# abstract-liu/LORB_SLAM

Measured on AMD Instinct MI355X. Metric: ORB matches/sec + local-BA iterations/sec (50 KF, 10k pts) at 1/2/4/8 MI355X, higher is better.
Workload: dtype f64+u8; 1 GPU; c4_local_mapping_step_chained; windows_per_gpu=1, kf=50, fixed_kf=5, points=10679, observations=75130, new_kf_keypoints=2000, match=2000x~10679 bf crossCheck, parallelism=independent windows x1

## Files before the change

### lorb_slam_amd/csrc/lorb_ba.hip

```cpp
#ifndef LORB_NO_CONTRACT
#pragma clang fp contract(fast)
#endif
#include "lorb_ba_math.h"
#include "lorb_internal.h"
#include "lorb_ba_dev.h"
#include "lorb_ba_plan.h"

#include <algorithm>
#include <cmath>
#include <type_traits>

namespace {

using namespace lorb::ba;
using lorb::residual;
using lorb::residual_jac;
using lorb::residual_jac_s;
using lorb::residual_s;

__device__ __forceinline__ void init_run(const BaDev& d, int W, int ctot, int n_pt, int nf, const LMOpt& o, const int i,
                                         const int stride) {
  if (i < W) {
    WinState s;
    s.radius = o.init_radius; s.decrease_factor = 2.0; s.cost = 0.0; s.x_norm = 0.0; s.gmax = 0.0;
    s.initial_cost = 0.0; s.iter = 0; s.n_success = 0; s.n_invalid = 0;
    s.done = d.win[i].n_obs_all == 0 ? 1 : 0;
    s.relin = 1; s.cur = 0; s.last_successful = 1; s.term = 0; s.chol_fail = 0; s.pad = 0;
    d.st[i] = s;
    d.ls_fail[i] = 0;
    if (d.sharded) d.wfail_part[i] = 0.0;
  }
  if (i < ctot) {
    double x[6];
#pragma unroll
    for (int k = 0; k < 6; ++k) { x[k] = d.x_init_pose[6 * i + k]; d.x_pose[0][6 * i + k] = x[k]; }
    d.rot_lin[i] = lorb::rot_jet(x);
  }
  if (i < nf) {
    double x[6];
#pragma unroll
    for (int k = 0; k < 6; ++k) x[k] = d.fixed_pose[6 * i + k];
    d.rot_fix[i] = lorb::rot_jet(x);
    d.rotv_fix[i] = lorb::rot_val(x);
  }
  for (int k = i; k < 3 * n_pt; k += stride) d.x_pt[0][k] = d.x_init_pt[k];
}
__global__ __launch_bounds__(256) void k_ba_init(BaDev d, int W, int ctot, int n_pt, int nf, LMOpt o) {
  init_run(d, W, ctot, n_pt, nf, o, blockIdx.x * blockDim.x + threadIdx.x, gridDim.x * blockDim.x);
}


constexpr int kGW = kGB / 64;
static_assert(kGW >= 1 && kGW <= 16 && kGB % 64 == 0, "point groups of 64..1024 observations, whole waves");
template <bool M1>
__device__ __forceinline__ void block_red3(double& a, double& b, double& c, double (*red)[kGW]) {
  a = wave_sum(a); b = M1 ? wave_max(b) : wave_sum(b); c = wave_sum(c);
  if (kGW == 1) return;
  __syncthreads();
  if ((threadIdx.x & 63) == 0) {
    const int w = threadIdx.x >> 6;
    red[0][w] = a; red[1][w] = b; red[2][w] = c;
  }
  __syncthreads();
  a = red[0][0]; b = red[1][0]; c = red[2][0];
#pragma unroll
  for (int k = 1; k < kGW; ++k) { a += red[0][k]; b = M1 ? fmax(b, red[1][k]) : b + red[1][k]; c += red[2][k]; }
}

__device__ __forceinline__ bool prep_point(const double (&Eu)[6], const double (&bu)[3], const double (&sp)[3],
                                           double rad, const LMOpt& o, double (&Ei)[6], double (&b)[3]) {
  double E[6];
#pragma unroll
  for (int k = 0; k < 3; ++k) b[k] = bu[k] * sp[k];
  E[0] = Eu[0] * sp[0] * sp[0]; E[1] = Eu[1] * sp[0] * sp[1]; E[2] = Eu[2] * sp[0] * sp[2];
  E[3] = Eu[3] * sp[1] * sp[1]; E[4] = Eu[4] * sp[1] * sp[2]; E[5] = Eu[5] * sp[2] * sp[2];
  E[0] += fmin(fmax(E[0], o.min_diag), o.max_diag) / rad;
  E[3] += fmin(fmax(E[3], o.min_diag), o.max_diag) / rad;
  E[5] += fmin(fmax(E[5], o.min_diag), o.max_diag) / rad;
  if (!inv3(E, Ei)) {
#pragma unroll
    for (int k = 0; k < 6; ++k) Ei[k] = 0.0;
    return false;
  }
  return true;
}
__device__ __forceinline__ void prep_fail(const BaDev& d, int win, int fold) {
  if (fold) d.ls_fail[win] = 1;
  else if (d.sharded) d.wfail_part[win] = 1.0;
  else d.st[win].chol_fail = 1;
}

template <int PH>
__global__ __launch_bounds__(64) void k_ba_win_reduce(BaDev d) {
  const int w = blockIdx.x;
  if (d.st[w].done) return;
  const BaWin& W = d.win[w];
  const int lane = threadIdx.x;
  double a = 0.0, b = 0.0, c = 0.0;
  if (PH == 0) group_partials<0, 1, 2, true>(d.part, W.pblk_base, W.n_pblk, lane, a, c, b);
  else group_partials<3, 4, 5, false>(d.part, W.pblk_base, W.n_pblk, lane, a, b, c);
  a = wave_sum(a); b = wave_sum(b);
  c = PH == 0 ? wave_max(c) : wave_sum(c);
  if (lane == 0) {
    if (PH == 0) { d.wlin_part[2 * w] = a; d.wlin_part[2 * w + 1] = b; d.wmax_part[w] = c; }
    else { d.wstep_part[3 * w] = a; d.wstep_part[3 * w + 1] = b; d.wstep_part[3 * w + 2] = c; }
  }
}

template <bool SH>
__device__ __forceinline__ void lm_begin_run(const BaDev& d, const LMOpt& o, const int w) {
  const WinState* Sp = d.st + w;
  const WinState S = *Sp;
  const BaWin W = d.win[w];
  if (S.done) return;
  (void)lm_head<SH>(d, o, w, threadIdx.x, S, W);
}
template <bool SH>
__global__ __launch_bounds__(64) void k_ba_lm_begin(BaDev d, LMOpt o) {
  lm_begin_run<SH>(d, o, blockIdx.x);
}

__device__ __forceinline__ lorb_lm_iteration lm_rec(const WinState& S, int outcome, double mcc, double ncost,
                                                    double step_norm) {
  lorb_lm_iteration r;
  r.iteration = S.iter; r.outcome = outcome;
  r.cost = S.cost; r.model_cost_change = mcc; r.new_cost = ncost; r.radius = S.radius; r.step_norm = step_norm;
  return r;
}
__device__ __forceinline__ void lm_record(const BaDev& d, int w, const lorb_lm_iteration& r) {
  if (r.iteration < 1 || r.iteration > LORB_LM_TRACE_CAP) return;
  d.trace[(size_t)w * LORB_LM_TRACE_CAP + r.iteration - 1] = r;
}

__device__ __forceinline__ WinState state_copy(const WinState& s) {
  WinState r;
  r.radius = s.radius; r.decrease_factor = s.decrease_factor; r.cost = s.cost; r.x_norm = s.x_norm; r.gmax = s.gmax;
  r.initial_cost = s.initial_cost; r.iter = s.iter; r.n_success = s.n_success; r.n_invalid = s.n_invalid;
  r.done = s.done; r.relin = s.relin; r.cur = s.cur; r.last_successful = s.last_successful; r.term = s.term;
  r.chol_fail = s.chol_fail; r.pad = s.pad;
  return r;
}

__device__ __forceinline__ int lm_decide(const LMOpt& o, WinState& S, bool valid, double mccs, double ncost,
                                         double sn2, lorb_lm_iteration& rec) {
  const double model_cost_change = -mccs;
  valid = valid && isfinite(model_cost_change) && isfinite(sn2) && model_cost_change > 0.0;
  if (!valid) {
    rec = lm_rec(S, LORB_LM_STEP_INVALID, model_cost_change, ncost, sqrt(sn2));
    if (++S.n_invalid >= o.max_invalid) {
      S.done = 1; S.term = LORB_TERM_FAILURE;
    } else {
      S.radius = S.radius / S.decrease_factor;
      S.decrease_factor *= 2.0;
      S.last_successful = 0;
      if (S.iter >= o.max_iter) { S.done = 1; S.term = LORB_TERM_NO_CONVERGENCE; }
    }
    return 0;
  }
  S.n_invalid = 0;
  const double new_cost = isfinite(ncost) ? ncost : 1.7976931348623157e308;
  const double step_norm = sqrt(sn2);
  if (step_norm <= o.ptol * (S.x_norm + o.ptol)) {
    rec = lm_rec(S, LORB_LM_STEP_PARAM_TOL, model_cost_change, new_cost, step_norm);
    S.done = 1; S.term = LORB_TERM_PARAMETER_TOL; return 0;
  }
  const double cost_change = S.cost - new_cost;
  if (fabs(cost_change) <= o.ftol * S.cost) {
    rec = lm_rec(S, LORB_LM_STEP_FUNC_TOL, model_cost_change, new_cost, step_norm);
    S.done = 1; S.term = LORB_TERM_FUNCTION_TOL; return 0;
  }
  const double rel = cost_change / model_cost_change;
  rec = lm_rec(S, rel > o.min_rel ? LORB_LM_STEP_ACCEPTED : LORB_LM_STEP_REJECTED, model_cost_change, new_cost,
               step_norm);
  if (rel > o.min_rel) {
    S.cur ^= 1;
    S.relin = 1;
    S.cost = new_cost;
    S.n_success++;
    const double tt = 2.0 * rel - 1.0;
    S.radius = S.radius / fmax(1.0 / 3.0, 1.0 - tt * tt * tt);
    S.radius = fmin(o.max_radius, S.radius);
    S.decrease_factor = 2.0;
  } else {
    S.last_successful = 0;
    S.radius = S.radius / S.decrease_factor;
    S.decrease_factor *= 2.0;
  }
  if (S.iter >= o.max_iter) { S.done = 1; S.term = LORB_TERM_NO_CONVERGENCE; }
  return rel > o.min_rel;
}

template <bool SH>
__device__ __forceinline__ void lm_end_eval(const BaDev& d, const LMOpt& o, int w, int lane, WinState& S,
                                            const BaWin& W, lorb_lm_iteration& rec) {
  bool valid = !S.chol_fail;
  double mccs = 0.0, ncost = 0.0, sn2 = 0.0;
  if (valid) {
    const int cur = S.cur;
    const int c0 = W.pose_base + lane;
    const bool has0 = lane < W.n_poses;
// ... 935 lines not shown
      df = 2.0;
    } else {
      last_successful = 0;
      radius /= df;
      df *= 2.0;
    }
  }
#pragma unroll
  for (int k = 0; k < 6; ++k)
    if (t == k) pose_out[k] = xs[k];
  if (t == 0) {
    lorb_ba_summary sm;
    sm.iterations = iter; sm.successful_steps = n_success; sm.termination = term; sm.pad_ = 0;
    sm.initial_cost = initial_cost; sm.final_cost = cost;
    *sum = sm;
  }
}
__global__ __launch_bounds__(kPoThreads) void k_ba_pose_only(PoOff aoff, const int32_t* __restrict__ res_off,
                                                             const float* __restrict__ intr,
                                                             const float* __restrict__ pose_init,
                                                             const float* __restrict__ pts3d,
                                                             const float* __restrict__ obs2d, LMOpt o,
                                                             double* __restrict__ pose_out,
                                                             lorb_ba_summary* __restrict__ sums) {
  const int f = blockIdx.x;
  const int r0 = aoff.n ? aoff.off[f] : res_off[f], r1 = aoff.n ? aoff.off[f + 1] : res_off[f + 1];
  const float* P = pts3d + 3 * (size_t)r0;
  const float* U = obs2d + 2 * (size_t)r0;
  po_run(r1 - r0, intr[4 * f], intr[4 * f + 1], intr[4 * f + 2], intr[4 * f + 3], pose_init + 6 * f, o,
         [&](int r, double (&X)[3], double (&uv)[2]) {
#pragma unroll
           for (int k = 0; k < 3; ++k) X[k] = P[3 * r + k];
           uv[0] = U[2 * r]; uv[1] = U[2 * r + 1];
         },
         pose_out + 6 * f, sums + f);
}

struct TailSlots {
  int nk;
  const int* code;
  bool keep;
  const uint8_t* slot_state;
  const float *slot_pos, *pt_pos, *x, *y;
  float* list;
  int* copy_to;
  int* assign_out;
};
__device__ __forceinline__ void tail_run(const TailSlots& s, bool solve, double fx, double fyv, double cx, double cy,
                                         const float* pose_init, const LMOpt& o, int* __restrict__ n_res,
                                         double* __restrict__ pose_out, lorb_ba_summary* __restrict__ sum) {
  __shared__ int s_slot[kPoRegRes];
  __shared__ int wsum[kPoW];
  const int t = threadIdx.x;
  int nres = 0;
  for (int c0 = 0; c0 < s.nk; c0 += kPoThreads) {
    const int j = c0 + t;
    int cd = LORB_ASSIGN_NULL;
    bool has = false;
    if (j < s.nk) {
      cd = s.code[j];
      has = cd >= 0 || (s.keep && cd == LORB_ASSIGN_UNCHANGED && s.slot_state && s.slot_state[j] != LORB_SLOT_EMPTY);
      if (s.copy_to) s.copy_to[j] = cd;
      if (s.assign_out) s.assign_out[j] = cd;
    }
    int tot;
    const int r = nres + lorb::block_excl_scan<kPoThreads>(has ? 1 : 0, wsum, &tot);
    if (has) {
      if (r < kPoRegRes) {
        s_slot[r] = j;
      } else {
        const float* X = cd >= 0 ? s.pt_pos + 3 * (size_t)cd : s.slot_pos + 3 * (size_t)j;
        float* L = s.list + 5 * (size_t)r;
        L[0] = X[0]; L[1] = X[1]; L[2] = X[2]; L[3] = s.x[j]; L[4] = s.y[j];
      }
    }
    nres += tot;
  }
  __syncthreads();
  if (t == 0) *n_res = nres;
  po_run(solve ? nres : 0, fx, fyv, cx, cy, pose_init, o,
         [&](int r, double (&X)[3], double (&uv)[2]) {
           if (r < kPoRegRes) {
             const int j = s_slot[r], cd = s.code[j];
             const float* Xp = cd >= 0 ? s.pt_pos + 3 * (size_t)cd : s.slot_pos + 3 * (size_t)j;
#pragma unroll
             for (int k = 0; k < 3; ++k) X[k] = Xp[k];
             uv[0] = s.x[j]; uv[1] = s.y[j];
           } else {
             const float* L = s.list + 5 * (size_t)r;
#pragma unroll
             for (int k = 0; k < 3; ++k) X[k] = L[k];
             uv[0] = L[3]; uv[1] = L[4];
           }
         },
         pose_out, sum);
}

__global__ __launch_bounds__(kPoThreads) void k_track_tail(lorb::TrackTail a, LMOpt o) {
  const int nm1 = *a.nm1;
  const bool retry = nm1 <= a.min_matches;
  const int nm2 = retry ? *a.nm2 : -1;
  const int pass = !retry ? 1 : (nm2 > a.min_matches ? 2 : 0);
  if (threadIdx.x == 0) { a.rec->pass = pass; a.rec->nmatches_first = nm1; a.rec->nmatches_retry = nm2; }
  const TailSlots s = {a.nk, retry ? a.assign2 : a.assign, !retry, a.slot_state, a.slot_pos, a.last_pos, a.x, a.y,
                       a.list, retry ? a.assign : nullptr, a.assign_out};
  tail_run(s, pass != 0, a.fx, a.fy_eff, a.cx, a.cy, a.pose_init, o, &a.rec->n_residuals, a.rec->pose, &a.rec->summary);
}

__global__ __launch_bounds__(kPoThreads) void k_local_tail(lorb::LocalTail a, LMOpt o) {
  __shared__ int wcnt[kPoW];
  const int nm = *a.nm;
  int c = 0;
  for (int m = threadIdx.x; m < a.np; m += kPoThreads) c += a.in_view[m] != 0;
  int n_in_view;
  lorb::block_excl_scan<kPoThreads>(c, wcnt, &n_in_view);
  const bool ok = nm > a.min_matches;
  if (threadIdx.x == 0) { a.rec->ok = ok; a.rec->nmatches = nm; a.rec->n_in_view = n_in_view; }
  const TailSlots s = {a.nk, a.assign, true, a.slot_state, a.slot_pos, a.pt_pos, a.x, a.y, a.list, nullptr, a.assign_out};
  tail_run(s, ok, a.fx, a.fy_eff, a.cx, a.cy, a.pose_init, o, &a.rec->n_residuals, a.rec->pose, &a.rec->summary);
}

LMOpt to_dev_opt(const lorb_lm_options* o) {
  LMOpt d;
  d.max_iter = o->max_num_iterations; d.max_invalid = o->max_num_consecutive_invalid_steps;
  d.jacobi = o->jacobi_scaling; d.ftol = o->function_tolerance; d.gtol = o->gradient_tolerance;
  d.ptol = o->parameter_tolerance; d.init_radius = o->initial_trust_region_radius;
  d.max_radius = o->max_trust_region_radius; d.min_radius = o->min_trust_region_radius;
  d.min_rel = o->min_relative_decrease; d.min_diag = o->min_lm_diagonal; d.max_diag = o->max_lm_diagonal;
  return d;
}
bool same_opt(const LMOpt& a, const LMOpt& b) {
  return a.max_iter == b.max_iter && a.max_invalid == b.max_invalid && a.jacobi == b.jacobi && a.ftol == b.ftol &&
         a.gtol == b.gtol && a.ptol == b.ptol && a.init_radius == b.init_radius && a.max_radius == b.max_radius &&
         a.min_radius == b.min_radius && a.min_rel == b.min_rel && a.min_diag == b.min_diag && a.max_diag == b.max_diag;
}

bool no_graph() { static const bool v = env_flag("LORB_NO_GRAPH"); return v; }
bool no_fuse() { static const bool v = env_flag("LORB_NO_FUSE"); return v; }

int chol_kind_of(const lorb_ba_plan* P) {
  static const bool force_old = [] { const char* e = getenv("LORB_CHOL"); return e && e[0] == 'o'; }();
  static const bool no_2s = [] { const char* e = getenv("LORB_CHOL"); return e && e[0] == 'w'; }();
  if (!P->Ctot) return -1;
  const bool chol_w = !force_old && P->max_bw <= 48 && sizeof(double) * (size_t)P->max_env_w <= (size_t)kLdsBudget;
  const bool chol_2s = chol_w && !no_2s && P->min_n16 >= 128 && P->min_bw >= 15;
  return chol_2s ? 2 : chol_w ? 1 : 0;
}

size_t x2_count(const lorb_ba_plan* P) {
  return P->devb ? P->x2_off + (size_t)P->env_total : (size_t)P->env_total + P->n_total + P->W;
}

int red_threads(const lorb_ba_plan* P) {
  const double W = std::max(P->W, 1), cams = std::max((double)P->Ctot / W, 1.0);
  const double cand = (double)P->n_pblk / W * ((P->max_bw + 1) / 6.0) / cams;
  if (P->grid_bp <= 256 || cand >= 128.0) return 1024;
  return P->grid_bp <= 1024 ? 512 : 256;
}
template <int MODE>
void launch_red(const lorb_ba_plan* P, hipStream_t s, const BaDev& d, const LMOpt& o) {
  const int rt = red_threads(P);
  if (rt == 1024) hipLaunchKernelGGL((k_ba_red<MODE, 1024>), dim3(P->grid_bp), dim3(1024), 0, s, d, o);
  else if (rt == 512) hipLaunchKernelGGL((k_ba_red<MODE, 512>), dim3(P->grid_bp), dim3(512), 0, s, d, o);
  else hipLaunchKernelGGL((k_ba_red<MODE, 256>), dim3(P->grid_bp), dim3(256), 0, s, d, o);
}

void launch_ls(const lorb_ba_plan* P, hipStream_t s, const BaDev& d, const LMOpt& o) {
  lorb::KernelTimer kt(P->ctx, LORB_K_BA_LINEARIZE);
  if (P->has_super) {
    if (P->grid_sg) hipLaunchKernelGGL(k_ba_ls_sup, dim3(P->grid_sg), dim3(kLsThreads), 0, s, d, o);
  } else if (P->grid_pblk) {
    hipLaunchKernelGGL(k_ba_ls, dim3(P->grid_pblk), dim3(kLsThreads), 0, s, d, o);
  }
}

constexpr int kFoldMaxGroups = 512;
bool fold_of(const lorb_ba_plan* P) {
  if (env_flag("LORB_NO_FOLD") || no_fuse() || P->comm || P->has_super || chol_kind_of(P) != 2) return false;
  for (const BaWin& w : P->hwin)
    if (w.n_poses > 0 && w.n_pblk == 0) return false;
  return P->grid_pblk > 0 && P->grid_pblk <= kFoldMaxGroups;
}

lorb_ba_plan::GraphKey graph_key(const lorb_ba_plan* P) {
  lorb_ba_plan::GraphKey k;
  k.kind = chol_kind_of(P);
  k.lds = k.kind >= 1 ? P->max_env_w : P->max_env + 1000000 * P->max_bw;
  k.memset_env = sizeof(double) * (size_t)P->max_env > (size_t)kLdsBudget;
  k.env_total = k.memset_env ? P->env_total : 0;
  k.grid_pblk = P->grid_pblk; k.grid_bp = P->grid_bp; k.pt_launch = P->pt_launch;
  k.x2_n = P->comm ? (int)x2_count(P) : 0;
  k.red_wide = red_threads(P);
  k.sup = P->has_super ? 1 : 0;
  k.grid_sg = P->grid_sg;
  k.fold = P->fold ? 1 : 0;
  return k;
}

int enqueue_linearize(lorb_ba_plan* P, const LMOpt& o) {
  hipStream_t s = P->ctx->stream;
  const BaDev& d = P->dev;
  launch_ls(P, s, d, o);
  if (P->grid_bp) {
    lorb::KernelTimer kt(P->ctx, LORB_K_BA_SCHUR);
    launch_red<0>(P, s, d, o);
  }
  if (P->comm) {
    hipLaunchKernelGGL(k_ba_win_reduce<0>, dim3(P->W), dim3(64), 0, s, d);
    {
      lorb::KernelTimer kt(P->ctx, LORB_K_ALLREDUCE);
      LORB_TRY(lorb::comm_allreduce(P->comm, d.U_part, d.U, (size_t)P->Ctot * 27 + 2 * P->W, LORB_OP_SUM));
      LORB_TRY(lorb::comm_allreduce(P->comm, d.wmax_part, d.wmax, (size_t)P->W, LORB_OP_MAX));
    }
    hipLaunchKernelGGL(k_ba_lm_begin<true>, dim3(P->W), dim3(64), 0, s, d, o);
  } else {
    hipLaunchKernelGGL(k_ba_lm_begin<false>, dim3(P->W), dim3(64), 0, s, d, o);
  }
  return LORB_OK;
}

int enqueue_iteration(lorb_ba_plan* P, const LMOpt& o, bool first, bool last) {
  lorb_ctx* ctx = P->ctx;
  hipStream_t s = ctx->stream;
  const bool fused = !first && chol_kind_of(P) == 2 && !no_fuse();
  const bool fold_in = P->fold && fused, fold_out = P->fold && !last;
  BaDev d = P->dev;
  d.fold = fold_in ? (P->W == 1 ? 2 : 1) : 0;
  if (fused) {
    launch_ls(P, s, d, o);
  } else {
    LORB_TRY(enqueue_linearize(P, o));
  }
  const bool chol_in_lds = sizeof(double) * (size_t)P->max_env <= (size_t)kLdsBudget;
  if (P->env_total && !chol_in_lds && !P->comm) LORB_HIP(ctx, hipMemsetAsync(d.env, 0, sizeof(double) * P->env_total, s));
  if (P->grid_bp) {
    lorb::KernelTimer kt(ctx, LORB_K_BA_SCHUR);
    if (fused) launch_red<2>(P, s, d, o);
    else launch_red<1>(P, s, d, o);
  }
  if (P->comm && fused) {
    hipLaunchKernelGGL(k_ba_win_reduce<0>, dim3(P->W), dim3(64), 0, s, d);
    lorb::KernelTimer kt(ctx, LORB_K_ALLREDUCE);
    LORB_TRY(lorb::comm_allreduce(P->comm, d.U_part, d.U, P->fx_n, LORB_OP_SUM));
    LORB_TRY(lorb::comm_allreduce(P->comm, d.wmax_part, d.wmax, (size_t)P->W, LORB_OP_MAX));
  } else if (P->comm) {
    lorb::KernelTimer kt(ctx, LORB_K_ALLREDUCE);
    LORB_TRY(lorb::comm_allreduce(P->comm, P->x2_send, P->x2_recv, x2_count(P), LORB_OP_SUM));
  }
  const int kind = chol_kind_of(P);
  P->chol_kind = kind;
  if (kind >= 0) {
    lorb::KernelTimer kt(ctx, LORB_K_BA_CHOLESKY);
    launch_chol(kind, CholShape{P->W, P->max_env, P->max_env_w, P->max_bw}, s, d, o, fused);
  }
  if (P->grid_pblk) hipLaunchKernelGGL(k_ba_bs2, dim3(P->grid_pblk), dim3(kGB), 0, s, d);
  if (P->comm) {
    hipLaunchKernelGGL(k_ba_win_reduce<1>, dim3(P->W), dim3(64), 0, s, d);
    {
      lorb::KernelTimer kt(ctx, LORB_K_ALLREDUCE);
      LORB_TRY(lorb::comm_allreduce(P->comm, d.wstep_part, d.wstep, 3 * (size_t)P->W, LORB_OP_SUM));
    }
    hipLaunchKernelGGL(k_ba_lm_end<true>, dim3(P->W), dim3(64), 0, s, d, o);
  } else if (!fold_out) {
    hipLaunchKernelGGL(k_ba_lm_end<false>, dim3(P->W), dim3(64), 0, s, d, o);
  }
  LORB_CHECK_LAUNCH(ctx);
  return LORB_OK;
}

int enqueue_solve(lorb_ba_plan* P, const LMOpt& o) {
  lorb_ctx* ctx = P->ctx;
  {
    const int n = std::max(std::max(std::max(P->W, P->Ctot), P->NF), std::min(3 * P->pt_launch, 256 * 1024));
    hipLaunchKernelGGL(k_ba_init, dim3(lorb::ceil_div(std::max(n, 1), 256)), dim3(256), 0, ctx->stream, P->dev, P->W,
                       P->Ctot, P->pt_launch, P->NF, o);
  }
  LORB_CHECK_LAUNCH(ctx);
  if (o.max_iter <= 0) return enqueue_linearize(P, o);
  for (int it = 0; it < o.max_iter; ++it) LORB_TRY(enqueue_iteration(P, o, it == 0, it + 1 == o.max_iter));
  return LORB_OK;
}

int plan_solve(lorb_ba_plan* P, const lorb_lm_options* opt) {
  lorb_ctx* ctx = P->ctx;
  LMOpt o = to_dev_opt(opt);
  P->fold = fold_of(P);
  const bool timing = ctx->ktime || no_graph() || (P->comm && !P->comm->rccl);
  if (timing) return enqueue_solve(P, o);
  const lorb_ba_plan::GraphKey key = graph_key(P);
  const bool same = key == P->gkey && same_opt(P->graph_opt, o);
  return P->cache.replay_or_capture(ctx, same, [&] { return enqueue_solve(P, o); },
                                    [&] { P->gkey = key; P->graph_opt = o; });
}

int plan_read(lorb_ba_plan* P, double* const* pose_out, double* const* point_out,
              lorb_ba_summary* sums) {
  lorb_ctx* ctx = P->ctx;
  std::vector<WinState> st(P->W);
  std::vector<std::vector<double>> hp(P->W);
  LORB_HIP(ctx, hipMemcpyAsync(st.data(), P->d_state, sizeof(WinState) * P->W, hipMemcpyDeviceToHost, ctx->stream));
  LORB_HIP(ctx, hipStreamSynchronize(ctx->stream));
  for (int w = 0; w < P->W; ++w) {
    const BaWin& bw = P->hwin[w];
    const int cur = st[w].cur;
    if (pose_out && pose_out[w] && bw.n_poses) {
      hp[w].resize(6 * (size_t)bw.n_poses);
      LORB_HIP(ctx, hipMemcpyAsync(hp[w].data(), P->dev.x_pose[cur] + 6 * bw.pose_base, sizeof(double) * 6 * bw.n_poses, hipMemcpyDeviceToHost, ctx->stream));
    }
    if (point_out && point_out[w] && bw.n_points)
      LORB_HIP(ctx, hipMemcpyAsync(point_out[w], P->dev.x_pt[cur] + 3 * bw.point_base, sizeof(double) * 3 * bw.n_points, hipMemcpyDeviceToHost, ctx->stream));
    if (sums) {
      lorb_ba_summary s{};
      s.iterations = st[w].iter; s.successful_steps = st[w].n_success; s.termination = st[w].term;
      s.initial_cost = st[w].initial_cost; s.final_cost = st[w].cost;
      if (bw.n_obs_all == 0) { s.iterations = 0; s.termination = LORB_TERM_FUNCTION_TOL; }
      sums[w] = s;
    }
  }
  LORB_HIP(ctx, hipStreamSynchronize(ctx->stream));
  for (int w = 0; w < P->W; ++w) {
    if (hp[w].empty()) continue;
    const std::vector<int>& map = P->cam_map[w];
    for (int c = 0; c < P->hwin[w].n_poses; ++c)
      for (int q = 0; q < 6; ++q)
        pose_out[w][6 * (size_t)c + q] = hp[w][6 * (size_t)(map.empty() ? c : map[c]) + q];
  }
  return LORB_OK;
}

}

struct lorb_ba_group {
  lorb_ctx* ctx = nullptr;
  std::vector<lorb_ba_plan*> plans;
  GraphCache cache{"group graph"};
  LMOpt graph_opt{};
  std::vector<unsigned> gens;
  std::vector<lorb_ba_plan::GraphKey> keys;
  int n_fused = 0;
};

namespace {

bool group_fused(const lorb_ba_group* G) {
  if (no_fuse() || G->plans.size() > (size_t)kGrpMax) return false;
  for (const lorb_ba_plan* P : G->plans)
    if (P->W == 0 || P->comm || P->has_super || chol_kind_of(P) != 2) return false;
  return true;
}

template <typename F>
GrpGrid grp_grid(const lorb_ba_group* G, F f) {
  GrpGrid g{};
  for (size_t k = 0; k < G->plans.size(); ++k) g.pre[k + 1] = g.pre[k] + f(G->plans[k]);
  for (size_t k = G->plans.size() + 1; k <= (size_t)kGrpMax; ++k) g.pre[k] = g.pre[G->plans.size()];
  return g;
}

template <int MODE>
void launch_red_g(const lorb_ba_group* G, hipStream_t s, const BaGrp& bg, const LMOpt& o) {
  const GrpGrid gg = grp_grid(G, [](const lorb_ba_plan* P) { return P->grid_bp; });
  const int n = (int)G->plans.size(), nb = gg.pre[n];
  if (nb == 0) return;
  bool wide = nb <= 256;
  for (const lorb_ba_plan* P : G->plans) wide = wide || (red_threads(P) == 1024 && P->grid_bp > 256);
  const int rt = wide ? 1024 : nb <= 1024 ? 512 : 256;
  if (rt == 1024) hipLaunchKernelGGL((k_ba_red_g<MODE, 1024>), dim3(nb), dim3(1024), 0, s, bg, gg, o);
  else if (rt == 512) hipLaunchKernelGGL((k_ba_red_g<MODE, 512>), dim3(nb), dim3(512), 0, s, bg, gg, o);
  else hipLaunchKernelGGL((k_ba_red_g<MODE, 256>), dim3(nb), dim3(256), 0, s, bg, gg, o);
}

int enqueue_group_solve(lorb_ba_group* G, const LMOpt& o) {
  lorb_ctx* ctx = G->ctx;
  hipStream_t s = ctx->stream;
  const int n = (int)G->plans.size();
  BaGrp bg{};
  bg.n = n;
  for (int k = 0; k < n; ++k) bg.d[k] = G->plans[k]->dev;
  {
    GrpInit a{};
    for (int k = 0; k < n; ++k) {
      const lorb_ba_plan* P = G->plans[k];
      a.W[k] = P->W; a.ctot[k] = P->Ctot; a.n_pt[k] = P->pt_launch; a.nf[k] = P->NF;
    }
    const GrpGrid gg = grp_grid(G, [](const lorb_ba_plan* P) {
      const int m = std::max(std::max(std::max(P->W, P->Ctot), P->NF), std::min(3 * P->pt_launch, 256 * 1024));
      return lorb::ceil_div(std::max(m, 1), 256);
    });
    hipLaunchKernelGGL(k_ba_init_g, dim3(gg.pre[n]), dim3(256), 0, s, bg, gg, a, o);
  }
  const GrpGrid g_pb = grp_grid(G, [](const lorb_ba_plan* P) { return P->grid_pblk; });
  const GrpGrid g_w = grp_grid(G, [](const lorb_ba_plan* P) { return P->W; });
  size_t lds = 0;
  for (const lorb_ba_plan* P : G->plans) lds = std::max(lds, sizeof(double) * (size_t)P->max_env_w);
  const bool fold = G->plans[0]->fold;
  bool one_win = true;
  for (const lorb_ba_plan* P : G->plans) one_win = one_win && P->W == 1;
  BaGrp bgf = bg;
  for (int k = 0; k < n; ++k) bgf.d[k].fold = one_win ? 2 : 1;
  auto linearise = [&](bool fold_in) {
    lorb::KernelTimer kt(ctx, LORB_K_BA_LINEARIZE);
    if (g_pb.pre[n]) hipLaunchKernelGGL(k_ba_ls_g, dim3(g_pb.pre[n]), dim3(kLsThreads), 0, s, fold_in ? bgf : bg, g_pb, o);
  };
  if (o.max_iter <= 0) {
    linearise(false);
    launch_red_g<0>(G, s, bg, o);
    hipLaunchKernelGGL(k_ba_lm_begin_g, dim3(g_w.pre[n]), dim3(64), 0, s, bg, g_w, o);
    LORB_CHECK_LAUNCH(ctx);
    return LORB_OK;
  }
  for (int it = 0; it < o.max_iter; ++it) {
    const bool first = it == 0;
    const bool fold_in = fold && !first, fold_out = fold && it + 1 < o.max_iter;
    const BaGrp& bi = fold_in ? bgf : bg;
    linearise(fold_in);
    if (first) {
      {
        lorb::KernelTimer kt(ctx, LORB_K_BA_SCHUR);
        launch_red_g<0>(G, s, bg, o);
      }
      hipLaunchKernelGGL(k_ba_lm_begin_g, dim3(g_w.pre[n]), dim3(64), 0, s, bg, g_w, o);
    }
    for (const lorb_ba_plan* P : G->plans)
      if (P->env_total && sizeof(double) * (size_t)P->max_env > (size_t)kLdsBudget)
        LORB_HIP(ctx, hipMemsetAsync(P->dev.env, 0, sizeof(double) * P->env_total, s));
    {
      lorb::KernelTimer kt(ctx, LORB_K_BA_SCHUR);
      if (first) launch_red_g<1>(G, s, bg, o);
      else launch_red_g<2>(G, s, bi, o);
    }
    {
      lorb::KernelTimer kt(ctx, LORB_K_BA_CHOLESKY);
      launch_chol_2s_g(s, bi, g_w, o, !first, lds);
    }
    if (g_pb.pre[n]) hipLaunchKernelGGL(k_ba_bs2_g, dim3(g_pb.pre[n]), dim3(kGB), 0, s, bg, g_pb);
    if (!fold_out) hipLaunchKernelGGL(k_ba_lm_end_g, dim3(g_w.pre[n]), dim3(64), 0, s, bg, g_w, o);
  }
  for (lorb_ba_plan* P : G->plans) P->chol_kind = 2;
  LORB_CHECK_LAUNCH(ctx);
  return LORB_OK;
}

int group_solve(lorb_ba_group* G, const lorb_lm_options* opt) {
  lorb_ctx* ctx = G->ctx;
  if (!group_fused(G)) {
    for (lorb_ba_plan* P : G->plans)
      if (P->W > 0) LORB_TRY(plan_solve(P, opt));
    return LORB_OK;
  }
  const LMOpt o = to_dev_opt(opt);
  bool fold = true;
  int groups = 0;
  for (const lorb_ba_plan* P : G->plans) { fold = fold && fold_of(P); groups += P->grid_pblk; }
  fold = fold && groups <= kFoldMaxGroups;
  for (lorb_ba_plan* P : G->plans) P->fold = fold;
  if (no_graph() || ctx->ktime) {
    LORB_TRY(enqueue_group_solve(G, o));
    G->n_fused++;
    return LORB_OK;
  }
  bool same = same_opt(G->graph_opt, o) && G->gens.size() == G->plans.size();
  for (size_t k = 0; k < G->plans.size() && same; ++k)
    same = G->gens[k] == G->plans[k]->gen && G->keys[k] == graph_key(G->plans[k]);
  LORB_TRY(G->cache.replay_or_capture(ctx, same, [&] { return enqueue_group_solve(G, o); }, [&] {
    G->graph_opt = o;
    G->gens.clear(); G->keys.clear();
    for (const lorb_ba_plan* P : G->plans) { G->gens.push_back(P->gen); G->keys.push_back(graph_key(P)); }
  }));
  G->n_fused++;
  return LORB_OK;
}

}

namespace lorb {
int launch_local_tail(lorb_ctx* ctx, const LocalTail& t, const lorb_lm_options* opt) {
  hipLaunchKernelGGL(k_local_tail, dim3(1), dim3(kPoThreads), 0, ctx->stream, t, to_dev_opt(opt));
  LORB_CHECK_LAUNCH(ctx);
  return LORB_OK;
}
int launch_track_tail(lorb_ctx* ctx, const TrackTail& t, const lorb_lm_options* opt) {
  hipLaunchKernelGGL(k_track_tail, dim3(1), dim3(kPoThreads), 0, ctx->stream, t, to_dev_opt(opt));
// ... 187 lines not shown
```

### lorb_slam_amd/csrc/lorb_ba_build.hip

```cpp
#ifndef LORB_NO_CONTRACT
#pragma clang fp contract(fast)
#endif
#include "lorb_ba_math.h"
#include "lorb_internal.h"
#include "lorb_ba_dev.h"
#include "lorb_ba_plan.h"

#include <algorithm>
#include <chrono>
#include <cmath>
#include <map>

struct lorb_ba_devbuild {
  int K_cap = 0, P_cap = 0, C = 0, F = 0, Wd = 0;
  int* key_out = nullptr; int* val_out = nullptr;
  int* scr = nullptr; size_t scr_bytes = 0;
  int* pt_cnt = nullptr;
  int* hdr = nullptr;
  int* cov = nullptr;
  int* cam_cnt = nullptr;
  unsigned long long* bits = nullptr;
  int* perm = nullptr;
  int pblk_cap = 0, part_cap = 0, gspan_cap = 0, sgrp_cap = 0;
  size_t gpart_cap = 0;
  int* pinned = nullptr; size_t pinned_n = 0;
  bool dirty = true;
  bool sorted_hint = false;
  std::vector<double> h_red;
  unsigned char* up_dev = nullptr; unsigned char* up_host = nullptr; int up_bp_cap = 0;
  const unsigned char* up_host_dev = nullptr;
  size_t off_live = 0, off_perm = 0, off_gcam = 0, off_bp = 0, up_bytes = 0;
  std::vector<char> last_adj;
  std::vector<int> h_copy;
  std::vector<int> last_map;
  hipEvent_t rb_ev = nullptr;
  bool rb_pending = false, rb_sorted = false, rb_fuse = false;
  ~lorb_ba_devbuild() {
    if (rb_ev) (void)hipEventDestroy(rb_ev);
    if (pinned) (void)hipHostFree(pinned);
    if (up_host) (void)hipHostFree(up_host);
  }
};

namespace {

using namespace lorb::ba;

void print_diagnostics(const lorb_ba_plan& p) {
  if (p.hp_n)
    fprintf(stderr, "lorb_ba_plan: host phase %.2f us per device build (%d builds): checks %.2f order %.2f blocks %.2f "
            "buffers %.2f staging %.2f launch %.2f\n", p.hp_us / p.hp_n, p.hp_n, p.hp_sec[0] / p.hp_n, p.hp_sec[1] / p.hp_n,
            p.hp_sec[2] / p.hp_n, p.hp_sec[3] / p.hp_n, p.hp_sec[4] / p.hp_n, p.hp_sec[5] / p.hp_n);
  if (p.dev.gspan && p.n_pblk > 0 && getenv("LORB_PM_SPANS")) {
    std::vector<int2> gs(p.n_pblk);
    if (hipStreamSynchronize(p.ctx->stream) == hipSuccess &&
        hipMemcpy(gs.data(), p.dev.gspan, sizeof(int2) * p.n_pblk, hipMemcpyDeviceToHost) == hipSuccess) {
      std::vector<int> sp;
      for (const int2& g : gs) if (g.y > 0) sp.push_back(g.y);
      std::sort(sp.begin(), sp.end());
      if (!sp.empty())
        fprintf(stderr, "lorb_ba_plan: %d point groups (%zu live), %d observations; camera span p50 %d p90 %d max %d\n",
                p.n_pblk, sp.size(), p.K, sp[sp.size() / 2], sp[sp.size() * 9 / 10], sp.back());
    }
  }
#ifdef LORB_LS_STAMPS
  if (p.dev.dbg && p.n_pblk > 0 && getenv("LORB_LS_PRINT")) {
    std::vector<unsigned long long> st((size_t)p.n_pblk * 8);
    if (hipStreamSynchronize(p.ctx->stream) == hipSuccess &&
        hipMemcpy(st.data(), p.dev.dbg, sizeof(unsigned long long) * st.size(), hipMemcpyDeviceToHost) == hipSuccess) {
      fprintf(stderr, "lorb_ba_plan: k_ba_ls phase cycles (median, p90):");
      for (int k = 0; k < 5; ++k) {
        std::vector<long long> v;
        for (int g = 0; g < p.n_pblk; ++g)
          if (st[8 * g]) v.push_back((long long)(st[8 * g + k + 1] - st[8 * g + k]));
        std::sort(v.begin(), v.end());
        if (!v.empty()) fprintf(stderr, " %c %lld %lld", "ABCDE"[k], v[v.size() / 2], v[v.size() * 9 / 10]);
      }
      fprintf(stderr, "\n");
      std::map<unsigned long long, std::vector<int>> by_cu;
      unsigned long long r0 = ~0ull, r1 = 0;
      std::vector<long long> dur;
      for (int g = 0; g < p.n_pblk; ++g) {
        if (!st[8 * g]) continue;
        const unsigned long long a = st[8 * g + 7] >> 20, b = a + (st[8 * g + 7] & 0xfffff);
        r0 = std::min(r0, a); r1 = std::max(r1, b);
        dur.push_back((long long)(b - a));
        by_cu[st[8 * g + 6] & 0xff00ffull].push_back(g);
      }
      std::sort(dur.begin(), dur.end());
      int shared = 0;
      long long pair_max = 0;
      for (auto& c : by_cu) {
        if (c.second.size() < 2) continue;
        ++shared;
        unsigned long long a = ~0ull, b = 0;
        for (int g : c.second) { a = std::min(a, st[8 * g + 7] >> 20); b = std::max(b, (st[8 * g + 7] >> 20) + (st[8 * g + 7] & 0xfffff)); }
        pair_max = std::max(pair_max, (long long)(b - a));
      }
      if (!dur.empty())
        fprintf(stderr, "lorb_ba_plan: k_ba_ls real time (us): first start -> last end %.2f; group p50 %.2f p90 %.2f max %.2f; "
                "%zu CUs, %d with > 1 group (their span max %.2f)\n", (r1 - r0) * 0.01, dur[dur.size() / 2] * 0.01,
                dur[dur.size() * 9 / 10] * 0.01, dur.back() * 0.01, by_cu.size(), shared, pair_max * 0.01);
      std::vector<PBlk> pb(p.n_pblk);
      std::vector<int2> gs(p.n_pblk);
      if (hipMemcpy(pb.data(), p.dev.pblk, sizeof(PBlk) * p.n_pblk, hipMemcpyDeviceToHost) == hipSuccess &&
          hipMemcpy(gs.data(), p.dev.gspan, sizeof(int2) * p.n_pblk, hipMemcpyDeviceToHost) == hipSuccess) {
        std::vector<int> ord;
        for (int g = 0; g < p.n_pblk; ++g) if (st[8 * g]) ord.push_back(g);
        std::sort(ord.begin(), ord.end(), [&](int a, int b) { return (st[8 * a + 7] & 0xfffff) > (st[8 * b + 7] & 0xfffff); });
        for (size_t i = 0; i < ord.size() && i < 6; ++i) {
          const int g = ord[i];
          fprintf(stderr, "  group %d: %.2f us, points %d obs %d span %d, phases", g, (st[8 * g + 7] & 0xfffff) * 0.01,
                  pb[g].cnt, pb[g].no, gs[g].y);
          for (int k = 0; k < 5; ++k) fprintf(stderr, " %lld", (long long)(st[8 * g + k + 1] - st[8 * g + k]));
          fprintf(stderr, "\n");
        }
      }
    }
  }
#endif
}

template <typename T>
int dalloc(lorb_ba_plan* P, size_t n, T** out) {
  void* p = nullptr;
  LORB_HIP(P->ctx, hipMalloc(&p, std::max<size_t>(n, 1) * sizeof(T)));
  P->allocs.push_back(p);
  *out = static_cast<T*>(p);
  return LORB_OK;
}
template <typename T>
int dupload(lorb_ba_plan* P, const std::vector<T>& v, T** out) {
  LORB_TRY(dalloc(P, v.size(), out));
  if (!v.empty())
    LORB_HIP(P->ctx, hipMemcpyAsync(*out, v.data(), v.size() * sizeof(T), hipMemcpyHostToDevice, P->ctx->stream));
  return LORB_OK;
}
template <typename T>
int dalloc(lorb_ba_plan* P, size_t n, const T** out) { return dalloc(P, n, const_cast<T**>(out)); }
template <typename T>
int dupload(lorb_ba_plan* P, const std::vector<T>& v, const T** out) { return dupload(P, v, const_cast<T**>(out)); }
int dfree(lorb_ba_plan* P, const void* ptr) {
  LORB_HIP(P->ctx, hipStreamSynchronize(P->ctx->stream));
  LORB_HIP(P->ctx, hipFree(const_cast<void*>(ptr)));
  auto it = std::find(P->allocs.begin(), P->allocs.end(), ptr);
  if (it != P->allocs.end()) P->allocs.erase(it);
  return LORB_OK;
}

int camera_band(int C, const std::vector<char>& adj, const std::vector<int>& pos) {
  int b = 0;
  for (int c = 0; c < C; ++c) {
    int lo = pos[c];
    for (int n = 0; n < C; ++n)
      if (adj[(size_t)c * C + n]) lo = std::min(lo, pos[n]);
    b = std::max(b, pos[c] - lo);
  }
  return b;
}

std::vector<int> camera_order(int C, const std::vector<char>& adj) {
  std::vector<int> id(C), deg(C, 0);
  for (int c = 0; c < C; ++c) {
    id[c] = c;
    for (int n = 0; n < C; ++n) deg[c] += (n != c) && adj[(size_t)c * C + n];
  }
  static const bool off = env_flag("LORB_NO_RCM");
  if (off || C < 3) return id;
  std::vector<int> order;
  std::vector<char> seen(C, 0);
  order.reserve(C);
  while ((int)order.size() < C) {
    int s = -1;
    for (int c = 0; c < C; ++c)
      if (!seen[c] && (s < 0 || deg[c] < deg[s])) s = c;
    size_t head = order.size();
    order.push_back(s);
    seen[s] = 1;
    while (head < order.size()) {
      const int u = order[head++];
      std::vector<int> nb;
      for (int n = 0; n < C; ++n)
        if (n != u && adj[(size_t)u * C + n] && !seen[n]) nb.push_back(n);
      std::sort(nb.begin(), nb.end(), [&](int a, int b) { return deg[a] != deg[b] ? deg[a] < deg[b] : a < b; });
      for (int n : nb) { seen[n] = 1; order.push_back(n); }
    }
  }
  std::reverse(order.begin(), order.end());
  std::vector<int> pos(C);
  for (int i = 0; i < C; ++i) pos[order[i]] = i;
  return camera_band(C, adj, pos) < camera_band(C, adj, id) ? pos : id;
}

constexpr int kPmSpan = 128;
constexpr size_t kPartBudgetBytes = (size_t)16 << 30;
void pm_layout(BaWin& bw, int span_max, long long& total) {
  bw.bwc = bw.n > 0 ? std::max(bw.bw - 5, 0) / 6 : 0;
  span_max = std::max(std::min(span_max, bw.n_poses), 0);
  bw.part_cam = 36 * pm_nslots(span_max, bw.bwc);
  bw.part_stride = bw.part_cam + 18 * span_max;
  bw.part_base = total;
  total += (long long)bw.n_sg * bw.part_stride;
}
int sg_factor(int n_pblk) {
  const char* e = getenv("LORB_SG_F");
  if (e && atoi(e) >= 1) return n_pblk > 1 ? atoi(e) : 1;
  return n_pblk > 512 ? (n_pblk + 479) / 480 : 1;
}
int part_budget_check(lorb_ctx* ctx, long long total) {
  if ((size_t)std::max(total, 1ll) * sizeof(double) > kPartBudgetBytes)
    return lorb::set_error(ctx, LORB_E_NOMEM, "point-group partials need %.1f GB (> %.0f GB budget)",
                           (double)total * sizeof(double) / 1e9, (double)kPartBudgetBytes / 1e9);
  return LORB_OK;
}

int band_of(const std::vector<int>& fc) {
  int bw = 0;
  for (int c = 0; c < (int)fc.size(); ++c) bw = std::max(bw, 6 * c + 5 - 6 * fc[c]);
  return bw;
}

int alloc_exchange(lorb_ba_plan* P, size_t C, size_t W, size_t solve_n, double** sol, double** sol_part) {
  BaDev& d = P->dev;
  const lorb_comm* comm = P->comm;
  const size_t lin_pad = (C * 27 + 2 * W + 31) & ~(size_t)31;
  P->fx_n = lin_pad + solve_n;
  double *lin, *mx, *stp;
  LORB_TRY(dalloc(P, P->fx_n, &lin)); LORB_TRY(dalloc(P, W, &mx)); LORB_TRY(dalloc(P, 3 * W, &stp));
  double *linp = lin, *mxp = mx, *stpp = stp;
  if (comm && comm->nranks > 1) {
    LORB_TRY(dalloc(P, P->fx_n, &linp)); LORB_TRY(dalloc(P, W, &mxp)); LORB_TRY(dalloc(P, 3 * W, &stpp));
    LORB_HIP(P->ctx, hipMemsetAsync(linp, 0, sizeof(double) * P->fx_n, P->ctx->stream));
  }
  d.U = lin; d.V = lin + C * 21; d.wlin = lin + C * 27; d.wmax = mx; d.wstep = stp;
  d.U_part = linp; d.V_part = linp + C * 21; d.wlin_part = linp + C * 27; d.wmax_part = mxp; d.wstep_part = stpp;
  *sol = lin + lin_pad; *sol_part = linp + lin_pad;
  P->x2_send = *sol_part; P->x2_recv = *sol;
  d.sharded = comm ? 1 : 0;
  d.rank0 = comm ? (comm->rank == 0) : 1;
  return LORB_OK;
}

std::vector<std::vector<int>> point_cameras(const lorb_ba_window& in) {
  std::vector<std::vector<int>> pf(std::max(in.n_points, 0));
  for (int k = 0; k < in.n_obs; ++k) {
    const int p = in.obs_point[k], f = in.obs_frame[k];
    if (p >= 0 && p < in.n_points && f >= 0 && f < in.n_poses) pf[p].push_back(f);
  }
  return pf;
}

int build_plan(lorb_ctx* ctx, int nw, const lorb_ba_window* win_in, lorb_ba_plan* P) {
  P->cam_map.assign(nw, {});
  std::vector<lorb_ba_window> wins(win_in, win_in + nw);
  std::vector<std::vector<int>> frame_buf(nw);
  std::vector<std::vector<float>> pose_buf(nw);
  for (int w = 0; w < nw; ++w) {
    const lorb_ba_window& in = win_in[w];
    const int C = std::max(in.n_poses, 0);
    std::vector<char> adj((size_t)C * C, 0);
    for (auto& v : point_cameras(in))
      for (int a : v)
        for (int b : v) adj[(size_t)a * C + b] = 1;
    if (P->comm && C > 0) {
      std::vector<double> h(adj.begin(), adj.end());
      LORB_TRY(lorb::comm_allreduce_host(P->comm, h.data(), h.size(), LORB_OP_MAX));
      for (size_t i = 0; i < h.size(); ++i) adj[i] = h[i] > 0.0;
    }
    std::vector<int> map = camera_order(C, adj);
    bool ident = true;
    for (int c = 0; c < C; ++c) ident &= map[c] == c;
    P->cam_map[w] = map;
    if (ident) continue;
    frame_buf[w].assign(in.obs_frame, in.obs_frame + std::max(in.n_obs, 0));
    for (int& f : frame_buf[w])
      if (f >= 0 && f < C) f = map[f];
    pose_buf[w].resize(6 * (size_t)C);
    for (int c = 0; c < C; ++c)
      for (int q = 0; q < 6; ++q) pose_buf[w][6 * (size_t)map[c] + q] = in.pose_init[6 * (size_t)c + q];
    wins[w].obs_frame = frame_buf[w].data();
    wins[w].pose_init = pose_buf[w].data();
  }
  const lorb_ba_window* win = wins.data();
  P->ctx = ctx;
  P->W = nw;
  lorb_comm* comm = P->comm;
  std::vector<std::vector<int>> g_fc(nw);
  std::vector<std::vector<int>> g_cam_obs(nw);
  std::vector<int> g_obs(nw, 0);
  if (comm) {
    size_t nfc = 0;
    for (int w = 0; w < nw; ++w) nfc += (size_t)std::max(win[w].n_poses, 0);
    std::vector<double> hmin(nfc), hsum(nfc + nw);
    size_t o = 0;
    for (int w = 0; w < nw; ++w) {
      const lorb_ba_window& in = win[w];
      std::vector<int> fc(std::max(in.n_poses, 0)), cobs(std::max(in.n_poses, 0), 0);
      for (int c = 0; c < in.n_poses; ++c) fc[c] = c;
      for (auto& v : point_cameras(in))
        for (int a : v) {
          cobs[a]++;
          for (int b : v) fc[a] = std::min(fc[a], b);
        }
      for (int c = 0; c < in.n_poses; ++c) { hmin[o + c] = fc[c]; hsum[o + c] = cobs[c]; }
      hsum[nfc + w] = in.n_obs;
      o += in.n_poses;
    }
    LORB_TRY(lorb::comm_allreduce_host(comm, hmin.data(), hmin.size(), LORB_OP_MIN));
    LORB_TRY(lorb::comm_allreduce_host(comm, hsum.data(), hsum.size(), LORB_OP_SUM));
    o = 0;
    for (int w = 0; w < nw; ++w) {
      g_fc[w].resize(win[w].n_poses); g_cam_obs[w].resize(win[w].n_poses);
      for (int c = 0; c < win[w].n_poses; ++c) { g_fc[w][c] = (int)hmin[o + c]; g_cam_obs[w][c] = (int)hsum[o + c]; }
      g_obs[w] = (int)hsum[nfc + w];
      o += win[w].n_poses;
    }
  }
  std::vector<int> cam_active;
  std::vector<int> pt_obs_off(1, 0), obs_cam, obs_fix, obs_pt;
  std::vector<double2> obs_uv;
  std::vector<double> fixed, xpose, xpt;
  std::vector<PBlk> pblk;
  std::vector<int2> gcam;
  std::vector<int4> sgrp;
  std::vector<BlockPair> bps;
  int pose_base = 0, point_base = 0, fix_base = 0, env_base = 0, row_base = 0, n_pairs = 0;
  long long part_total = 0;
  for (int w = 0; w < nw; ++w) {
    const lorb_ba_window& in = win[w];
    if (in.n_poses < 0 || in.n_points < 0 || in.n_obs < 0 || in.n_fixed < 0)
      return lorb::set_error(ctx, LORB_E_INVALID, "window %d: negative sizes", w);
    BaWin bw{};
    bw.pose_base = pose_base; bw.n_poses = in.n_poses;
    bw.point_base = point_base; bw.n_points = in.n_points;
    bw.fx = in.fx; bw.fy = in.fy; bw.cx = in.cx; bw.cy = in.cy;
    bw.obs_base = (int)obs_cam.size(); bw.n_obs = in.n_obs;
    bw.n_obs_all = comm ? g_obs[w] : in.n_obs;
    std::vector<int> cnt(in.n_points + 1, 0);
    for (int k = 0; k < in.n_obs; ++k) {
      const int p = in.obs_point[k], f = in.obs_frame[k];
      if (p < 0 || p >= in.n_points) return lorb::set_error(ctx, LORB_E_INVALID, "window %d obs %d: bad point %d", w, k, p);
      if (f >= in.n_poses || f < -in.n_fixed) return lorb::set_error(ctx, LORB_E_INVALID, "window %d obs %d: bad frame %d", w, k, f);
      cnt[p + 1]++;
    }
    for (int p = 0; p < in.n_points; ++p) cnt[p + 1] += cnt[p];
    std::vector<int> order(in.n_obs), fill(in.n_points, 0);
    for (int k = 0; k < in.n_obs; ++k) { const int p = in.obs_point[k]; order[cnt[p] + fill[p]++] = k; }
    const int ob0 = (int)obs_cam.size();
    for (int p = 0; p < in.n_points; ++p) pt_obs_off.push_back(ob0 + cnt[p + 1]);
    for (int e = 0; e < in.n_obs; ++e) {
      const int k = order[e], f = in.obs_frame[k];
      obs_cam.push_back(f >= 0 ? pose_base + f : -1);
      obs_pt.push_back(point_base + in.obs_point[k]);
      obs_fix.push_back(f >= 0 ? -1 : fix_base + (-1 - f));
      obs_uv.push_back(make_double2(in.obs_uv[2 * k], in.obs_uv[2 * k + 1]));
    }
    for (int i = 0; i < 6 * in.n_fixed; ++i) fixed.push_back(in.fixed_pose[i]);
    for (int i = 0; i < 6 * in.n_poses; ++i) xpose.push_back(in.pose_init[i]);
    for (int i = 0; i < 3 * in.n_points; ++i) xpt.push_back(in.point_init[i]);
    {
      std::vector<int> n_cam(in.n_poses, 0);
// ... 234 lines not shown
        constexpr int kR = 16;
        int fr[kR];
#pragma unroll
        for (int k = 0; k < kR; ++k) fr[k] = k < cnt ? of[i + k] : -1 - k;
#pragma unroll
        for (int a = 1; a < kR; ++a)
#pragma unroll
          for (int b = 0; b < a; ++b)
            if (fr[a] >= 0 && fr[a] == fr[b]) err |= 4;
        for (int a = kR; a < cnt; ++a) {
          const int fa = of[i + a];
          if (fa < 0) continue;
          for (int b = 0; b < a; ++b)
            if (of[i + b] == fa) err |= 4;
        }
        if (FUSE && q >= 0 && q < n_pt) {
#pragma unroll
          for (int a = 0; a < kR; ++a) {
            if (fr[a] < 0 || fr[a] >= C) continue;
            atomicAdd(&s_cam[fr[a]], 1);
#pragma unroll
            for (int b = 0; b < a; ++b)
              if (fr[b] >= 0 && fr[b] < C && fr[b] != fr[a])
                atomicAdd(&s_cov[max(fr[a], fr[b]) * C + min(fr[a], fr[b])], 1);
          }
          for (int a = kR; a < cnt; ++a) {
            const int fa = of[i + a];
            if (fa < 0 || fa >= C) continue;
            atomicAdd(&s_cam[fa], 1);
            for (int b = 0; b < a; ++b) {
              const int fb = of[i + b];
              if (fb >= 0 && fb < C && fb != fa) atomicAdd(&s_cov[max(fa, fb) * C + min(fa, fb)], 1);
            }
          }
        }
      }
    }
  }
#pragma unroll
  for (int o = 32; o > 0; o >>= 1) cnt = max(cnt, __shfl_xor(cnt, o, 64));
  if (lane == 0 && cnt) atomicMax(&s_cnt, cnt);
  if (err) atomicOr(&s_err, err);
  __syncthreads();
  for (int k = t; k < C * kDbWords; k += 256) {
    const unsigned long long v = s_bits[k];
    const int wd = w0 + k % kDbWords;
    if (v && wd < Wd)
      __hip_atomic_fetch_or(&bits[(size_t)(k / kDbWords) * Wd + wd], v, __ATOMIC_RELAXED, __HIP_MEMORY_SCOPE_AGENT);
  }
  if (FUSE) {
    for (int k = t; k < C * C + C; k += 256) {
      const int v = s_cov[k];
      if (v) __hip_atomic_fetch_add(k < C * C ? &cov[k] : &cam_cnt[k - C * C], v, __ATOMIC_RELAXED, __HIP_MEMORY_SCOPE_AGENT);
    }
  }
  if (t == 0) {
    if (s_cnt > __hip_atomic_load(&hdr[1], __ATOMIC_RELAXED, __HIP_MEMORY_SCOPE_AGENT)) atomicMax(&hdr[1], s_cnt);
    if (s_err) atomicOr(&hdr[2], s_err);
  }
}

__global__ __launch_bounds__(1024) void k_db_scan1(const int* __restrict__ in, int* __restrict__ out, int n,
                                                   const int* __restrict__ n_dev, int* __restrict__ hdr) {
  __shared__ int wsum[16];
  __shared__ int s_tile[lorb::kScanTileLds];
  if (n_dev) n = min(n, *n_dev + 1);
  int mx = 0;
  const int tot = lorb::wg_excl_scan(in, out, n, s_tile, wsum, &mx);
  if (hdr) {
#pragma unroll
    for (int o = 32; o > 0; o >>= 1) mx = max(mx, __shfl_xor(mx, o, 64));
    if ((threadIdx.x & 63) == 0 && mx) atomicMax(&hdr[1], mx);
    if (threadIdx.x == 0) hdr[0] = tot;
  }
}

__global__ __launch_bounds__(256) void k_db_scatter(lorb_ba_window_dev w, int C, int F,
                                                    const int* __restrict__ pt_off, int* __restrict__ pt_cnt,
                                                    int* __restrict__ val) {
  const int k = blockIdx.x * 256 + threadIdx.x;
  const int n_obs = min(*w.d_n_obs, w.max_obs), n_pt = min(*w.d_n_points, w.max_points);
  if (k >= n_obs) return;
  const int q = w.d_obs_point[k], f = w.d_obs_frame[k];
  if (f < -F || f >= C || q < 0 || q >= n_pt) return;
  val[pt_off[q] + atomicSub(&pt_cnt[q], 1) - 1] = k;
}

__global__ __launch_bounds__(256) void k_db_segsort(lorb_ba_window_dev w, const int* __restrict__ pt_off,
                                                    int* __restrict__ val, int* __restrict__ key) {
  const int p = blockIdx.x * 256 + threadIdx.x;
  if (p >= min(*w.d_n_points, w.max_points)) return;
  const int a0 = pt_off[p], a1 = pt_off[p + 1], m = a1 - a0;
  if (m <= 16) {
    int v[16];
#pragma unroll
    for (int i = 0; i < 16; ++i) v[i] = i < m ? val[a0 + i] : 0x7fffffff;
#pragma unroll
    for (int r = 0; r < 16; ++r)
#pragma unroll
      for (int i = r & 1; i + 1 < 16; i += 2) {
        const int lo = min(v[i], v[i + 1]), hi = max(v[i], v[i + 1]);
        v[i] = lo; v[i + 1] = hi;
      }
#pragma unroll
    for (int i = 0; i < 16; ++i)
      if (i < m) { val[a0 + i] = v[i]; key[a0 + i] = p; }
  } else {
    for (int i = a0 + 1; i < a1; ++i) {
      const int x = val[i];
      int j = i - 1;
      while (j >= a0 && val[j] > x) { val[j + 1] = val[j]; --j; }
      val[j + 1] = x;
    }
    for (int i = a0; i < a1; ++i) key[i] = p;
  }
}

__global__ __launch_bounds__(256) void k_db_cov(int C, int Wd, const unsigned long long* __restrict__ bits,
                                                int* __restrict__ cov, int* __restrict__ cam_cnt) {
  const int pr = blockIdx.x * 4 + (threadIdx.x >> 6), lane = threadIdx.x & 63;
  if (pr >= C * (C + 1) / 2) return;
  int a = 0, r = pr;
  while (r >= C - a) { r -= C - a; ++a; }
  const int b = a + r;
  const unsigned long long* x = bits + (size_t)a * Wd;
  const unsigned long long* y = bits + (size_t)b * Wd;
  int c = 0;
  for (int i = lane; i < Wd; i += 64) c += __popcll(x[i] & y[i]);
#pragma unroll
  for (int o = 32; o > 0; o >>= 1) c += __shfl_xor(c, o, 64);
  if (lane == 0) {
    if (a == b) {
      cam_cnt[a] = c;
      cov[a * C + a] = 0;
    } else {
      cov[a * C + b] = c;
      cov[b * C + a] = c;
    }
  }
}

struct DbFused {
  int C, F, P, G, S, env_n, bits_n;
  int sorted;
  unsigned long long* bits;
  int* hdr;
  int* cov;
  int cov_n;
  const int* up_src;
  int* up_dst;
  int up_words;
  int sgf = 1, nsg = 0;
  int4* sgrp = nullptr;
};
struct DbCams {
  int perm[kPmSpan], gcam[kPmSpan];
};
__device__ __forceinline__ void group_bounds(const int* __restrict__ off, int P, long long b0, long long b1, int lane,
                                             int& s0, int& s1) {
  const int half = lane >> 5, j = lane & 31;
  const long long bound = half ? b1 : b0;
  int lo = 0, hi = P;
  while (__ballot(hi > lo)) {
    const int n = hi - lo;
    bool pr = false;
    if (n > 0) {
      const int q = lo + (int)(((long long)n * (j + 1)) / 33);
      pr = (long long)off[q] + q >= bound;
    }
    const unsigned long long bal = __ballot(pr);
    const unsigned msk = half ? (unsigned)(bal >> 32) : (unsigned)bal;
    if (n > 0) {
      if (msk) {
        const int f = __builtin_ctz(msk);
        hi = lo + (int)(((long long)n * (f + 1)) / 33);
        if (f > 0) lo = lo + (int)(((long long)n * f) / 33) + 1;
      } else {
        lo = lo + (int)(((long long)n * 32) / 33) + 1;
      }
    }
  }
  s0 = __shfl(lo, 0, 64);
  s1 = __shfl(lo, 32, 64);
}
__global__ __launch_bounds__(256) void k_db_gather(lorb_ba_window_dev w, BaDev d, int K, const int* __restrict__ key,
                                                   const int* __restrict__ val, DbFused f, DbCams cams) {
  const int gt = blockIdx.x * 256 + threadIdx.x, gs = gridDim.x * 256;
  for (int i = gt; i < f.up_words; i += gs) f.up_dst[i] = f.up_src[i];
  const int* __restrict__ perm = cams.perm;
  const int* __restrict__ gcam = cams.gcam;
  {
    const int m = max(max(6 * f.C, 6 * f.F), 3 * f.P);
    for (int i = gt; i < m; i += gs) {
      if (i < 6 * f.C) {
        const int c = i / 6, q = i - 6 * c;
        d.x_init_pose[6 * perm[c] + q] = (double)w.d_pose_init[i];
        if (q == 0) const_cast<int*>(d.cam_active)[perm[c]] = gcam[c] > 0;
      }
      if (i < 6 * f.F) const_cast<double*>(d.fixed_pose)[i] = (double)w.d_fixed_pose[i];
      if (i < 3 * f.P) d.x_init_pt[i] = (double)w.d_point_init[i];
    }
  }
  for (int g = gt >> 6; g < f.G; g += gs >> 6) {
    int s0, s1;
    group_bounds(d.pt_obs_off, f.P, (long long)g * f.S, (long long)(g + 1) * f.S, threadIdx.x & 63, s0, s1);
    if ((threadIdx.x & 63) == 0) {
      PBlk b;
      b.win = 0; b.p0 = s0; b.cnt = s1 - s0; b.o0 = d.pt_obs_off[s0]; b.no = d.pt_obs_off[s1] - d.pt_obs_off[s0];
      const_cast<PBlk*>(d.pblk)[g] = b;
    }
  }
  for (int i = gt; i < f.nsg; i += gs) f.sgrp[i] = make_int4(0, i * f.sgf, min(f.sgf, f.G - i * f.sgf), 0);
  for (int i = gt; i < f.env_n; i += gs) d.env_part[i] = 0.0;
  for (int i = gt; i < f.bits_n; i += gs) f.bits[i] = 0ull;
  for (int i = gt; i < f.cov_n; i += gs) f.cov[i] = 0;
  if (gt == 0) { f.hdr[1] = 0; f.hdr[2] = 0; }
  for (int e = gt; e < K; e += gs) {
    const int k = f.sorted ? e : val[e];
    const int fr = w.d_obs_frame[k];
    const_cast<int*>(d.obs_pt)[e] = f.sorted ? w.d_obs_point[e] : key[e];
    const_cast<int*>(d.obs_cam)[e] = fr >= 0 ? perm[fr] : -1;
    const_cast<int*>(d.obs_fix)[e] = fr >= 0 ? -1 : -1 - fr;
    const_cast<double2*>(d.obs_uv)[e] = make_double2(w.d_obs_uv[2 * k], w.d_obs_uv[2 * k + 1]);
  }
}

__global__ __launch_bounds__(256) void k_db_result(BaDev d, int C, int P, const int* __restrict__ perm,
                                                   float* __restrict__ pose_out, float* __restrict__ pt_out,
                                                   float* __restrict__ ring, int R, int t0) {
  const int i = blockIdx.x * 256 + threadIdx.x;
  const int cur = d.st[0].cur;
  if ((pose_out || ring) && i < 6 * C) {
    const int c = i / 6, q = i - 6 * c;
    const float v = (float)d.x_pose[cur][6 * perm[c] + q];
    if (pose_out) pose_out[i] = v;
    if (ring) {
      const int r = (t0 + c) % R;
      ring[6 * (r < 0 ? r + R : r) + q] = v;
    }
  }
  if (pt_out)
    for (int k = i; k < 3 * P; k += gridDim.x * 256) pt_out[k] = (float)d.x_pt[cur][k];
}

__global__ __launch_bounds__(256) void k_db_result64(BaDev d, int C, int P, const int* __restrict__ perm,
                                                     double* __restrict__ out) {
  const int i = blockIdx.x * 256 + threadIdx.x;
  const WinState& st = d.st[0];
  const int cur = st.cur;
  if (i < 6 * C) {
    const int c = i / 6, q = i - 6 * c;
    out[i] = d.x_pose[cur][6 * perm[c] + q];
  }
  for (int k = i; k < 3 * P; k += gridDim.x * 256) out[6 * C + k] = d.x_pt[cur][k];
  if (i == 0) {
    double* s = out + 6 * C + 3 * P;
    s[0] = st.iter; s[1] = st.n_success; s[2] = st.term; s[3] = st.initial_cost; s[4] = st.cost;
  }
}

template <typename T, typename Cap>
int grow(lorb_ba_plan* P, T** ptr, Cap* cap, size_t need) {
  if (*ptr && (size_t)*cap >= need) return LORB_OK;
  if (*ptr) LORB_TRY(dfree(P, *ptr));
  const size_t n = std::max<size_t>(need + need / 4, 16);
  LORB_TRY(dalloc(P, n, ptr));
  *cap = (Cap)n;
  P->cache.invalidate();
  P->gen++;
  return LORB_OK;
}

int dev_alloc(lorb_ctx* ctx, const lorb_ba_window_dev* w, lorb_ba_plan* P) {
  lorb_ba_devbuild& b = *P->devb;
  b.K_cap = w->max_obs; b.P_cap = w->max_points; b.C = w->n_poses; b.F = w->n_fixed;
  b.Wd = (std::max(b.P_cap, 1) + 63) / 64;
  const size_t K = (size_t)std::max(b.K_cap, 1), Pn = (size_t)std::max(b.P_cap, 1), C = (size_t)std::max(b.C, 1);
  BaDev& d = P->dev;
  if (b.C > kPmSpan)
    return lorb::set_error(ctx, LORB_E_UNSUPPORTED, "device-built plans hold windows of <= %d cameras (%d)", kPmSpan, b.C);
  LORB_TRY(dalloc(P, K, &b.key_out)); LORB_TRY(dalloc(P, K, &b.val_out));
  {
    const size_t ints = ((Pn + 1 + 8 + C * C + C) + 1) & ~(size_t)1;
    b.scr_bytes = sizeof(int) * ints + sizeof(unsigned long long) * C * (size_t)b.Wd;
    unsigned char* m;
    LORB_TRY(dalloc(P, b.scr_bytes, &m));
    b.scr = reinterpret_cast<int*>(m);
    b.pt_cnt = b.scr; b.hdr = b.pt_cnt + Pn + 1; b.cov = b.hdr + 8; b.cam_cnt = b.cov + C * C;
    b.bits = reinterpret_cast<unsigned long long*>(b.scr + ints);
  }
  LORB_TRY(dalloc(P, K, &d.obs_pt)); LORB_TRY(dalloc(P, K, &d.obs_cam)); LORB_TRY(dalloc(P, K, &d.obs_fix));
  LORB_TRY(dalloc(P, K, &d.obs_uv)); LORB_TRY(dalloc(P, C, &d.cam_active));
  LORB_TRY(dalloc(P, Pn + 1, &d.pt_obs_off)); LORB_TRY(dalloc(P, (size_t)std::max(b.F, 1) * 6, &d.fixed_pose));
  LORB_TRY(dalloc(P, C * 6, &d.x_init_pose)); LORB_TRY(dalloc(P, Pn * 3, &d.x_init_pt));
  LORB_TRY(dalloc(P, C * 6, &d.x_pose[0])); LORB_TRY(dalloc(P, C * 6, &d.x_pose[1]));
  LORB_TRY(dalloc(P, Pn * 3, &d.x_pt[0])); LORB_TRY(dalloc(P, Pn * 3, &d.x_pt[1]));
  LORB_TRY(dalloc(P, C * 6, &d.scale_pose)); LORB_TRY(dalloc(P, Pn * 3, &d.scale_pt));
  LORB_TRY(dalloc(P, Pn * 3, &d.etb)); LORB_TRY(dalloc(P, Pn * 6, &d.pinv));
  const size_t n = 6 * C;
  P->x2_off = (n + 1 + 31) & ~(size_t)31;
  double *sol, *solp;
  LORB_TRY(alloc_exchange(P, C, 1, P->x2_off + n * n, &sol, &solp));
  d.rhs = sol; d.wfail = sol + n; d.env = sol + P->x2_off;
  d.rhs_part = solp; d.wfail_part = solp + n; d.env_part = solp + P->x2_off;
  LORB_TRY(dalloc(P, 2 * C, &d.rot_lin)); d.rot_stride = (int)C; LORB_TRY(dalloc(P, C, &d.rot_cand));
  LORB_TRY(dalloc(P, (size_t)std::max(b.F, 1), &d.rot_fix)); LORB_TRY(dalloc(P, (size_t)std::max(b.F, 1), &d.rotv_fix));
  LORB_TRY(dalloc(P, n, &d.ycam));
  LORB_TRY(dalloc(P, dbg_words(1, K + Pn + 1), &d.dbg));
  LORB_TRY(dalloc(P, ((size_t)n / 16 + 2) * 1024, &d.kco));
  LORB_TRY(dalloc(P, (size_t)1, &P->d_state)); d.st = P->d_state;
  LORB_TRY(dalloc(P, (size_t)1, &d.st2)); LORB_TRY(dalloc(P, (size_t)1, &d.ls_fail));
  LORB_TRY(dalloc(P, (size_t)LORB_LM_TRACE_CAP, &d.trace));
  P->W = 1;
  P->hwin.assign(1, BaWin{});
  P->pt_launch = b.P_cap;
  return LORB_OK;
}

int up_alloc(lorb_ba_plan* P, int bp_need) {
  lorb_ba_devbuild& b = *P->devb;
  if (b.up_dev && b.up_bp_cap >= bp_need) return LORB_OK;
  lorb_ctx* ctx = P->ctx;
  const int cap = std::max(bp_need + bp_need / 4, 16);
  auto al = [](size_t x) { return (x + 255) & ~(size_t)255; };
  const size_t C = (size_t)std::max(b.C, 1);
  b.off_live = al(sizeof(BaWin));
  b.off_perm = b.off_live + 256;
  b.off_gcam = b.off_perm + al(4 * C);
  b.off_bp = b.off_gcam + al(4 * C);
  b.up_bytes = b.off_bp + sizeof(BlockPair) * (size_t)cap;
  if (b.up_dev) {
    LORB_TRY(dfree(P, b.up_dev));
    (void)hipHostFree(b.up_host);
    b.up_host = nullptr;
  }
  LORB_TRY(dalloc(P, b.up_bytes, &b.up_dev));
  LORB_HIP(ctx, hipHostMalloc(reinterpret_cast<void**>(&b.up_host), b.up_bytes));
  LORB_HIP(ctx, hipHostGetDevicePointer((void**)&b.up_host_dev, b.up_host, 0));
  b.up_bp_cap = cap;
  BaDev& d = P->dev;
  d.win = reinterpret_cast<const BaWin*>(b.up_dev);
  d.live = reinterpret_cast<const int*>(b.up_dev + b.off_live);
  b.perm = reinterpret_cast<int*>(b.up_dev + b.off_perm);
  d.bp = reinterpret_cast<const BlockPair*>(b.up_dev + b.off_bp);
  P->grid_bp = cap;
  P->cache.invalidate();
  P->gen++;
  return LORB_OK;
}

int db_phase1_issue(lorb_ctx* ctx, const lorb_ba_window_dev* w, lorb_ba_plan* P, bool sorted) {
  lorb_ba_devbuild& b = *P->devb;
  hipStream_t s = ctx->stream;
  BaDev& d = P->dev;
  const int C = b.C, F = b.F, Kc = w->max_obs;
  const size_t nrb = 8 + (size_t)C + (size_t)C * C;
  const int nb_obs = lorb::ceil_div(std::max(Kc, 1), 256), nb_pt = lorb::ceil_div(std::max(b.P_cap, 1), 256);
  if (b.pinned_n < nrb) {
    if (b.pinned) (void)hipHostFree(b.pinned);
    b.pinned = nullptr; b.pinned_n = 0;
    LORB_HIP(ctx, hipHostMalloc(reinterpret_cast<void**>(&b.pinned), sizeof(int) * nrb));
    b.pinned_n = nrb;
  }
  if (!b.rb_ev) LORB_HIP(ctx, hipEventCreateWithFlags(&b.rb_ev, hipEventDisableTiming));
  if (b.dirty) LORB_HIP(ctx, hipMemsetAsync(b.scr, 0, b.scr_bytes, s));
  b.dirty = true;
  const bool fuse = sorted && C > 0 && sizeof(int) * ((size_t)C * C + C) <= (size_t)kDbFuseLds;
  if (sorted) {
    const size_t lds = sizeof(unsigned long long) * kDbWords * std::max(C, 1) +
                       (fuse ? sizeof(int) * ((size_t)C * C + C) : 0);
    hipLaunchKernelGGL(fuse ? k_db_sorted<true> : k_db_sorted<false>, dim3(lorb::ceil_div(Kc + 1, 256)), dim3(256), lds, s,
                       *w, C, F, b.Wd, const_cast<int*>(d.pt_obs_off), b.hdr, b.bits, b.cov, b.cam_cnt);
  } else {
    hipLaunchKernelGGL(k_db_keys, dim3(nb_obs), dim3(256), 0, s, *w, C, F, b.Wd, b.pt_cnt, b.hdr, b.bits);
    hipLaunchKernelGGL(k_db_scan1, dim3(1), dim3(1024), 0, s, b.pt_cnt, const_cast<int*>(d.pt_obs_off), b.P_cap + 1,
                       w->d_n_points, b.hdr);
    if (Kc > 0) {
      hipLaunchKernelGGL(k_db_scatter, dim3(nb_obs), dim3(256), 0, s, *w, C, F, d.pt_obs_off, b.pt_cnt, b.val_out);
      hipLaunchKernelGGL(k_db_segsort, dim3(nb_pt), dim3(256), 0, s, *w, d.pt_obs_off, b.val_out, b.key_out);
    }
  }
  if (C > 0 && !fuse)
    hipLaunchKernelGGL(k_db_cov, dim3(lorb::ceil_div(C * (C + 1) / 2, 4)), dim3(256), 0, s, C, b.Wd, b.bits, b.cov,
                       b.cam_cnt);
  LORB_CHECK_LAUNCH(ctx);
  LORB_HIP(ctx, hipMemcpyAsync(b.pinned, b.hdr, sizeof(int) * nrb, hipMemcpyDeviceToHost, s));
  LORB_HIP(ctx, hipEventRecord(b.rb_ev, s));
  b.rb_sorted = sorted;
  b.rb_fuse = fuse;
  b.rb_pending = true;
  return LORB_OK;
}

int db_phase1_wait(lorb_ctx* ctx, const lorb_ba_window_dev* w, lorb_ba_plan* P) {
  lorb_ba_devbuild& b = *P->devb;
  for (;;) {
    b.rb_pending = false;
    LORB_HIP(ctx, lorb::spin_wait(b.rb_ev));
    if (!(b.rb_sorted && (b.pinned[2] & 16))) return LORB_OK;
    b.sorted_hint = false;
    LORB_TRY(db_phase1_issue(ctx, w, P, false));
  }
}

int dev_build_issue(lorb_ctx* ctx, const lorb_ba_window_dev* w, lorb_ba_plan* P, int* lerr_out) {
  lorb_ba_devbuild& b = *P->devb;
  const bool shape_ok = w->n_poses == b.C && w->n_fixed == b.F && w->max_obs <= b.K_cap && w->max_points <= b.P_cap;
  *lerr_out = shape_ok ? 0 : 32;
  if (!shape_ok && !P->comm)
    return lorb::set_error(ctx, LORB_E_INVALID, "window shape differs from the plan's (cameras %d/%d, fixed %d/%d)",
                           w->n_poses, b.C, w->n_fixed, b.F);
  if (!shape_ok) return LORB_OK;
  const int rc = db_phase1_issue(ctx, w, P, b.sorted_hint);
  if (rc != LORB_OK && P->comm) { *lerr_out |= 64; return LORB_OK; }
  return rc;
}

struct HostPhase {
  using Clock = std::chrono::steady_clock;
  lorb_ba_plan* P;
  const bool on;
  const Clock::time_point t0 = Clock::now();
  Clock::time_point last = t0;
  void mark(int k) {
    if (!on) return;
    const auto now = Clock::now();
    P->hp_sec[k] += std::chrono::duration<double, std::micro>(now - last).count();
    if (k == 5) { P->hp_us += std::chrono::duration<double, std::micro>(now - t0).count(); P->hp_n++; }
    last = now;
  }
};

struct DbBuild {
  int K, maxk, Pn, K_all;
  const int *cov, *cam_cnt;
  const int *gcov, *gcam;
  std::vector<int> g_int;
  std::vector<BlockPair> bps;
  int n_pairs = 0, bw = 0;
  int S, G, SF, NSG;
  long long part_total;
};

int db_land(lorb_ctx* ctx, const lorb_ba_window_dev* w, lorb_ba_plan* P, int lerr, int phase_rc, DbBuild& r) {
  lorb_ba_devbuild& b = *P->devb;
  const bool shape_ok = !(lerr & 32), fuse = b.rb_fuse;
  const int C = b.C;
  const size_t nrb = 8 + (size_t)C + (size_t)C * C;
  if (phase_rc != LORB_OK) {
    if (!P->comm) return phase_rc;
    lerr |= 64;
  }
  b.h_copy.resize(nrb);
  if (lerr) std::fill(b.h_copy.begin(), b.h_copy.end(), 0);
  else std::memcpy(b.h_copy.data(), b.pinned, sizeof(int) * nrb);
  int* H = b.h_copy.data();
  if (fuse)
    for (int i = 0; i < C; ++i)
      for (int j = i + 1; j < C; ++j) H[8 + (size_t)i * C + j] = H[8 + (size_t)j * C + i];
  r.K = r.K_all = H[0]; r.maxk = H[1]; r.Pn = H[3];
  r.cov = r.gcov = H + 8;
  r.cam_cnt = r.gcam = r.cov + (size_t)C * C;
  const int err = H[2], Pn = r.Pn;
  int gerr = err, gmaxk = r.maxk;
  if (P->comm) {
    const size_t m = (size_t)C * C + C;
    b.h_red.assign(m + 9, 0.0);
    for (size_t i = 0; i < m; ++i) b.h_red[i] = (double)r.cov[i];
    b.h_red[m] = r.K;
    b.h_red[m + 1] = (Pn < 0 || Pn > b.P_cap) ? 1.0 : 0.0;
    for (int q = 0; q < 7; ++q) b.h_red[m + 2 + q] = ((err | lerr) >> q) & 1;
    LORB_TRY(lorb::comm_allreduce_host(P->comm, b.h_red.data(), b.h_red.size(), LORB_OP_SUM));
    double mk = r.maxk;
    LORB_TRY(lorb::comm_allreduce_host(P->comm, &mk, 1, LORB_OP_MAX));
    r.g_int.resize(m);
    for (size_t i = 0; i < m; ++i) r.g_int[i] = (int)b.h_red[i];
    r.gcov = r.g_int.data();
    r.gcam = r.g_int.data() + (size_t)C * C;
    r.K_all = (int)b.h_red[m];
    gerr = b.h_red[m + 1] > 0.0 ? 16 : 0;
    for (int q = 0; q < 7; ++q) gerr |= b.h_red[m + 2 + q] > 0.0 ? 1 << q : 0;
    gmaxk = (int)mk;
  }
  if (gerr & 32)
    return lorb::set_error(ctx, LORB_E_INVALID, "window shape differs from the plan's on %s (cameras %d/%d, fixed %d/%d)",
                           shape_ok ? "another rank" : "this rank", w->n_poses, b.C, w->n_fixed, b.F);
  if (gerr & 64)
    return phase_rc != LORB_OK ? phase_rc
                               : lorb::set_error(ctx, LORB_E_DEVICE, "device plan build failed on another rank");
  if (gerr & 8) return lorb::set_error(ctx, LORB_E_INVALID, "live point / observation count outside [0, capacity] (%d / %d)",
                                       b.P_cap, b.K_cap);
  if (gerr & 1) return lorb::set_error(ctx, LORB_E_INVALID, "observation with a point index outside [0, n_points)");
  if (gerr & 2) return lorb::set_error(ctx, LORB_E_INVALID, "observation with a frame index >= n_poses");
  if (gerr & 4) return lorb::set_error(ctx, LORB_E_INVALID, "a point observed twice by one camera");
  if ((gerr & 16) || Pn < 0 || Pn > b.P_cap) return lorb::set_error(ctx, LORB_E_INVALID, "n_points %d outside [0, %d]", Pn, b.P_cap);
  if (kGB - gmaxk < 1)
    return lorb::set_error(ctx, LORB_E_UNSUPPORTED, "a point with %d observations (device plans hold <= %d)", gmaxk, kGB - 1);
  return LORB_OK;
}

void db_camera_order(lorb_ba_devbuild& b, const DbBuild& r) {
  const int C = b.C;
  bool same_adj = b.last_adj.size() == (size_t)C * C;
  for (int i = 0; i < C && same_adj; ++i) {
    const int* row = r.gcov + (size_t)i * C;
    const char* last = b.last_adj.data() + (size_t)i * C;
    for (int j = 0; j < C; ++j)
      if (last[j] != (char)((i == j && r.gcam[i] > 0) || row[j] > 0)) { same_adj = false; break; }
  }
  if (!same_adj) {
    std::vector<char> adj((size_t)C * C, 0);
    for (int i = 0; i < C; ++i)
      for (int j = 0; j < C; ++j) adj[(size_t)i * C + j] = (i == j && r.gcam[i] > 0) || r.gcov[(size_t)i * C + j] > 0;
    b.last_map = camera_order(C, adj);
    b.last_adj.swap(adj);
  }
}

void db_blocks(const lorb_ba_devbuild& b, DbBuild& r) {
  const int C = b.C;
  std::vector<int> inv(C), fc(C);
  for (int c = 0; c < C; ++c) inv[b.last_map[c]] = c;
  for (int ch = 0; ch < C; ++ch) {
    fc[ch] = ch;
    for (int cl = 0; cl <= ch; ++cl) {
      const int cnt = ch == cl ? r.cam_cnt[inv[ch]] : r.cov[(size_t)inv[ch] * C + inv[cl]];
      if (ch != cl && r.gcov[(size_t)inv[ch] * C + inv[cl]] > 0) fc[ch] = std::min(fc[ch], cl);
      if (ch != cl && cnt == 0) continue;
      r.bps.push_back(BlockPair{0, ch, cl, r.n_pairs, cnt});
      r.n_pairs += cnt;
    }
  }
  r.bw = band_of(fc);
}

int db_layout(lorb_ctx* ctx, const lorb_ba_window_dev* w, lorb_ba_plan* P, DbBuild& r) {
  const int C = P->devb->C, n = 6 * C, K = r.K, Pn = r.Pn, bwid = r.bw;
  const int S = r.S = kGB - (r.maxk + 1) + 1;
  const int G = r.G = Pn > 0 ? (K + Pn - 1) / S + 1 : 0;
  BaWin bw{};
  bw.pose_base = 0; bw.n_poses = C; bw.point_base = 0; bw.n_points = Pn; bw.pblk_base = 0; bw.n_pblk = G;
  bw.env_base = 0; bw.env_size = n * (bwid + 1); bw.n = n; bw.row_base = 0; bw.bw = bwid;
  bw.obs_base = 0; bw.n_obs = K; bw.n_obs_all = r.K_all;
  bw.fx = w->fx; bw.fy = w->fy; bw.cx = w->cx; bw.cy = w->cy;
  const int SF = r.SF = sg_factor(G), NSG = r.NSG = G > 0 ? (G + SF - 1) / SF : 0;
  bw.sg_base = 0; bw.n_sg = NSG;
  r.part_total = 0;
  pm_layout(bw, C, r.part_total);
  LORB_TRY(part_budget_check(ctx, r.part_total));
  P->hwin[0] = bw;
  P->Ctot = C; P->Ptot = Pn; P->K = K; P->NF = P->devb->F; P->n_pblk = G; P->n_bp = (int)r.bps.size(); P->n_pairs = r.n_pairs;
  P->env_total = bw.env_size; P->n_total = n;
  P->max_env = bw.env_size + 2 * n; P->max_bw = bwid;
  P->min_bw = n > 0 ? bwid : (1 << 30);
  const int n16 = (n + 15) & ~15;
  P->max_env_w = chol_lds_words(n16, bwid);
  if (bwid <= 48 && sizeof(double) * (size_t)chol_lds_words(n16, 48) <= (size_t)kLdsBudget)
    P->max_env_w = chol_lds_words(n16, 48);
  P->min_n16 = n16 > 0 ? n16 : (1 << 30);
  return LORB_OK;
}

int db_buffers(lorb_ba_plan* P, const DbBuild& r) {
  lorb_ba_devbuild& b = *P->devb;
  BaDev& d = P->dev;
  LORB_TRY(grow(P, &d.pblk, &b.pblk_cap, (size_t)std::max(r.G, 1)));
  LORB_TRY(grow(P, &d.part, &b.part_cap, (size_t)b.pblk_cap * 8));
  P->grid_pblk = b.pblk_cap;
  LORB_TRY(grow(P, &d.gpart, &b.gpart_cap, (size_t)std::max(r.part_total, 1ll)));
  LORB_TRY(grow(P, &d.gspan, &b.gspan_cap, (size_t)b.pblk_cap));
  LORB_TRY(grow(P, &d.sgrp, &b.sgrp_cap, (size_t)b.pblk_cap));
  P->has_super = r.SF > 1;
  P->grid_sg = b.pblk_cap;
  return up_alloc(P, (int)r.bps.size());
}

void db_stage_and_gather(lorb_ctx* ctx, const lorb_ba_window_dev* w, lorb_ba_plan* P, const DbBuild& r, HostPhase& hp) {
  lorb_ba_devbuild& b = *P->devb;
  const std::vector<int>& map = b.last_map;
  const std::vector<BlockPair>& bps = r.bps;
  const int C = b.C;
  unsigned char* h = b.up_host;
  memcpy(h, &P->hwin[0], sizeof(BaWin));
  const int live[3] = {r.G, (int)bps.size(), r.NSG};
  memcpy(h + b.off_live, live, sizeof(live));
  memcpy(h + b.off_perm, map.data(), sizeof(int) * C);
  memcpy(h + b.off_gcam, r.gcam, sizeof(int) * C);
  if (!bps.empty()) memcpy(h + b.off_bp, bps.data(), sizeof(BlockPair) * bps.size());
  const int up_words = (int)((b.off_bp + sizeof(BlockPair) * bps.size() + 3) / 4);
  hp.mark(4);
  DbFused f{C, b.F, r.Pn, r.G, r.S, P->env_total, C * b.Wd, b.rb_sorted ? 1 : 0, b.bits, b.hdr, b.cov, C * C + C,
            reinterpret_cast<const int*>(b.up_host_dev), reinterpret_cast<int*>(b.up_dev), up_words};
  f.sgf = r.SF; f.nsg = r.NSG; f.sgrp = const_cast<int4*>(P->dev.sgrp);
  DbCams cams;
  for (int c = 0; c < C; ++c) { cams.perm[c] = map[c]; cams.gcam[c] = r.gcam[c]; }
  const int NB = lorb::ceil_div(r.K, 256);
  hipLaunchKernelGGL(k_db_gather, dim3(std::max(NB, 1)), dim3(256), 0, ctx->stream, *w, P->dev, r.K, b.key_out, b.val_out,
                     f, cams);
  b.dirty = false;
  hp.mark(5);
}

int dev_build_finish(lorb_ctx* ctx, const lorb_ba_window_dev* w, lorb_ba_plan* P, int lerr) {
  lorb_ba_devbuild& b = *P->devb;
  const int phase_rc = (lerr || !b.rb_pending) ? LORB_OK : db_phase1_wait(ctx, w, P);
  static const bool hp_log = env_flag("LORB_HOST_PHASE");
  HostPhase hp{P, hp_log};
  DbBuild r;
  LORB_TRY(db_land(ctx, w, P, lerr, phase_rc, r));
  hp.mark(0);
  db_camera_order(b, r);
  hp.mark(1);
  P->cam_map.assign(1, b.last_map);
  db_blocks(b, r);
  LORB_TRY(db_layout(ctx, w, P, r));
  hp.mark(2);
  LORB_TRY(db_buffers(P, r));
  hp.mark(3);
  db_stage_and_gather(ctx, w, P, r, hp);
  LORB_CHECK_LAUNCH(ctx);
  return LORB_OK;
}

int dev_build(lorb_ctx* ctx, const lorb_ba_window_dev* w, lorb_ba_plan* P) {
  int lerr = 0;
  LORB_TRY(dev_build_issue(ctx, w, P, &lerr));
  return dev_build_finish(ctx, w, P, lerr);
}

int create_host_plan(lorb_ctx* ctx, lorb_comm* comm, int32_t n_windows, const lorb_ba_window* windows, lorb_ba_plan** out) {
  if (!ctx || !out || n_windows < 0 || (n_windows > 0 && !windows)) return LORB_E_INVALID;
  if (comm && comm->ctx != ctx) return lorb::set_error(ctx, LORB_E_INVALID, "communicator belongs to another context");
  *out = nullptr;
  lorb_ba_plan* P = new (std::nothrow) lorb_ba_plan();
  if (!P) return LORB_E_NOMEM;
  P->comm = comm;
  const int rc = build_plan(ctx, n_windows, windows, P);
  if (rc != LORB_OK) { delete P; return rc; }
  *out = P;
  return LORB_OK;
}
bool window_dev_ok(const lorb_ba_window_dev* w) {
  return w->n_poses >= 0 && w->n_fixed >= 0 && w->max_points >= 0 && w->max_obs >= 0 && w->d_n_points && w->d_n_obs &&
         (w->n_poses == 0 || w->d_pose_init) && (w->n_fixed == 0 || w->d_fixed_pose) &&
         (w->max_points == 0 || w->d_point_init) &&
         (w->max_obs == 0 || (w->d_obs_point && w->d_obs_frame && w->d_obs_uv));
}
int create_dev_plan(lorb_ctx* ctx, lorb_comm* comm, const lorb_ba_window_dev* win, lorb_ba_plan** out) {
  if (!ctx || !win || !out) return LORB_E_INVALID;
  if (comm && comm->ctx != ctx) return lorb::set_error(ctx, LORB_E_INVALID, "communicator belongs to another context");
  if (!window_dev_ok(win)) return LORB_E_INVALID;
  *out = nullptr;
  lorb_ba_plan* P = new (std::nothrow) lorb_ba_plan();
  if (!P) return LORB_E_NOMEM;
  P->ctx = ctx;
  P->comm = comm;
  P->devb = new (std::nothrow) lorb_ba_devbuild();
  if (P->devb) P->devb->sorted_hint = true;
  int rc = P->devb ? dev_alloc(ctx, win, P) : LORB_E_NOMEM;
  if (rc == LORB_OK) rc = dev_build(ctx, win, P);
  if (rc != LORB_OK) { delete P; return rc; }
  *out = P;
  return LORB_OK;
}

}

lorb_ba_plan::~lorb_ba_plan() {
  print_diagnostics(*this);
  delete devb;
  for (void* p : allocs) (void)hipFree(p);
}

namespace lorb {
int ba_plan_update_dev_issue(lorb_ba_plan* P, const lorb_ba_window_dev* w) {
  if (!P || !w || !P->devb || P->comm) return LORB_E_INVALID;
  int lerr = 0;
  return dev_build_issue(P->ctx, w, P, &lerr);
}
int ba_plan_update_dev_finish(lorb_ba_plan* P, const lorb_ba_window_dev* w) {
  if (!P || !w || !P->devb || P->comm) return LORB_E_INVALID;
  return dev_build_finish(P->ctx, w, P, 0);
}
void ba_plan_sorted_hint(lorb_ba_plan* P, bool sorted) {
  if (P && P->devb) P->devb->sorted_hint = sorted;
}
const int* ba_plan_point_offsets(const lorb_ba_plan* P) { return P && P->devb ? P->dev.pt_obs_off : nullptr; }
void ba_plan_window_counts(const lorb_ba_plan* P, int* n_points, int* n_obs) {
  *n_points = P->Ptot;
  *n_obs = P->K;
}

static dim3 result_grid(const lorb_ba_plan* P) {
  return dim3(lorb::ceil_div(std::max(std::max(6 * P->Ctot, 1), std::min(3 * P->Ptot, 256 * 1024)), 256));
}
int ba_plan_result_ring_dev(lorb_ba_plan* P, float* ring, int R, int t0, float* d_point_out) {
  if (!P || !P->devb || !ring || R < 1) return LORB_E_INVALID;
  hipLaunchKernelGGL(k_db_result, result_grid(P), dim3(256), 0, P->ctx->stream, P->dev, P->Ctot, P->Ptot,
                     P->devb->perm, (float*)nullptr, d_point_out, ring, R, t0);
  LORB_CHECK_LAUNCH(P->ctx);
  return LORB_OK;
}

int ba_plan_result64_dev(lorb_ba_plan* P, double* d_out) {
  if (!P || !P->devb || !d_out) return LORB_E_INVALID;
  hipLaunchKernelGGL(k_db_result64, result_grid(P), dim3(256), 0, P->ctx->stream, P->dev, P->Ctot, P->Ptot, P->devb->perm,
                     d_out);
  LORB_CHECK_LAUNCH(P->ctx);
  return LORB_OK;
}

}

extern "C" {

int lorb_ba_plan_create(lorb_ctx* ctx, int32_t n_windows, const lorb_ba_window* windows, lorb_ba_plan** out) {
  return create_host_plan(ctx, nullptr, n_windows, windows, out);
}

int lorb_ba_plan_create_sharded(lorb_ctx* ctx, lorb_comm* comm, int32_t n_windows, const lorb_ba_window* shards,
                                lorb_ba_plan** out) {
  if (!comm) return LORB_E_INVALID;
  return create_host_plan(ctx, comm, n_windows, shards, out);
}

int lorb_ba_plan_create_dev(lorb_ctx* ctx, const lorb_ba_window_dev* win, lorb_ba_plan** out) {
  return create_dev_plan(ctx, nullptr, win, out);
}

int lorb_ba_plan_create_sharded_dev(lorb_ctx* ctx, lorb_comm* comm, const lorb_ba_window_dev* shard,
                                    lorb_ba_plan** out) {
  if (!comm) return LORB_E_INVALID;
  return create_dev_plan(ctx, comm, shard, out);
}

int lorb_ba_plan_update_dev(lorb_ba_plan* plan, const lorb_ba_window_dev* win) {
  if (!plan || !win) return LORB_E_INVALID;
  if (!plan->devb) return lorb::set_error(plan->ctx, LORB_E_INVALID, "not a device-built plan");
  return dev_build(plan->ctx, win, plan);
}

int lorb_ba_plan_result_dev(lorb_ba_plan* plan, float* d_pose_out, float* d_point_out) {
  if (!plan) return LORB_E_INVALID;
  if (!plan->devb) return lorb::set_error(plan->ctx, LORB_E_INVALID, "not a device-built plan");
  const int C = plan->Ctot, Pn = plan->Ptot;
  const int m = std::max(6 * C, std::min(3 * Pn, 256 * 1024));
  if (m > 0)
    hipLaunchKernelGGL(k_db_result, dim3(lorb::ceil_div(m, 256)), dim3(256), 0, plan->ctx->stream, plan->dev, C, Pn,
                       plan->devb->perm, d_pose_out, d_point_out, (float*)nullptr, 1, 0);
  LORB_CHECK_LAUNCH(plan->ctx);
  return LORB_OK;
}

int lorb_ba_plan_destroy(lorb_ba_plan* plan) {
  if (!plan) return LORB_OK;
  if (plan->ctx) (void)hipStreamSynchronize(plan->ctx->stream);
  delete plan;
  return LORB_OK;
}

}
```

### lorb_slam_amd/csrc/lorb_ba_dev.h

```cpp
#pragma once
#include "lorb_ba_math.h"
#include "lorb_internal.h"

namespace lorb {
namespace ba {

constexpr int kGB = 256;

struct BaWin {
  int pose_base, n_poses, point_base, n_points;
  int pblk_base, n_pblk;
  int env_base, env_size, n, row_base, bw;
  int obs_base, n_obs;
  int n_obs_all;
  int part_stride, part_cam, bwc, pad_;
  int sg_base, n_sg;
  long long part_base;
  double fx, fy, cx, cy;
};
struct PBlk { int win, p0, cnt, o0, no; };
struct BlockPair { int win, ch, cl, off, cnt; };
struct WinState {
  double radius, decrease_factor, cost, x_norm, gmax, initial_cost;
  int iter, n_success, n_invalid, done, relin, cur, last_successful, term, chol_fail, pad;
// ... 154 lines not shown
  double* x_pt[2];
  double* scale_pose;
  double* scale_pt;
  double* etb;
  double* pinv;
  double* U;
  double* V;
  double* env;
  double* rhs;
  double *U_part, *V_part, *wlin, *wlin_part, *wmax, *wmax_part;
  double *env_part, *rhs_part, *wfail, *wfail_part, *wstep, *wstep_part;
  const int* cam_active;
  int sharded, rank0;
  double* ycam;
  double* part;
  unsigned long long* dbg;
  double* kco;
  WinState* st;
  WinState* st2;
  int* ls_fail;
  int fold;
  int rot_stride;
  double* gpart;
  int2* gspan;
  const int4* sgrp;
  lorb_lm_iteration* trace;
  const int* live;
};

__device__ __forceinline__ int u21(int a, int b) {
  if (a > b) { const int t = a; a = b; b = t; }
  return a * 6 - (a * (a - 1)) / 2 + (b - a);
}

__device__ __forceinline__ int rot_off(const BaDev& d, int k) { return k ? d.rot_stride : 0; }

__device__ __forceinline__ double readlane_d(double v, int l) {
  const unsigned long long u = __double_as_longlong(v);
  const int lo = __builtin_amdgcn_readlane((int)(u & 0xffffffffu), l);
  const int hi = __builtin_amdgcn_readlane((int)(u >> 32), l);
  return __longlong_as_double(((unsigned long long)(unsigned)hi << 32) | (unsigned)lo);
}

__device__ __forceinline__ double& band(double* A, int bw, int i, int j) {
  return A[(size_t)i * (bw + 1) + (j - i + bw)];
}
__host__ __device__ __forceinline__ int pm_slot(int a, int dd, int bwc) {
  return a <= bwc ? a * (a + 1) / 2 + dd : (bwc + 1) * (bwc + 2) / 2 + (a - bwc - 1) * (bwc + 1) + dd;
}
__host__ __device__ __forceinline__ int pm_nslots(int span, int bwc) {
  return span <= 0 ? 0 : pm_slot(span - 1, span - 1 < bwc ? span - 1 : bwc, bwc) + 1;
}

#ifndef LORB_RSQ_STEPS
#define LORB_RSQ_STEPS 2
#endif
__device__ __forceinline__ double rsqrt_refined(double a) {
  double y = __builtin_amdgcn_rsq(a);
#pragma unroll
  for (int s = 0; s < LORB_RSQ_STEPS; ++s) {
    const double e = fma(-a * y, y, 1.0);
    y = fma(0.5 * y, e, y);
  }
  return y;
}

template <int F0, int F1, int F2, bool M1>
__device__ __forceinline__ void group_partials(const double* __restrict__ part, int base, int n, int lane,
                                               double& a, double& b, double& c) {
  constexpr int kPU = 8;
  for (int b0 = lane; b0 < n; b0 += 64 * kPU) {
    double v0[kPU], v1[kPU], v2[kPU];
#pragma unroll
    for (int u = 0; u < kPU; ++u) {
      const int g = b0 + 64 * u;
      const double* P = part + 8 * (base + (g < n ? g : 0));
      v0[u] = P[F0]; v1[u] = P[F1]; v2[u] = P[F2];
    }
#pragma unroll
    for (int u = 0; u < kPU; ++u)
      if (b0 + 64 * u < n) {
        a += v0[u];
        b = M1 ? fmax(b, v1[u]) : b + v1[u];
        c += v2[u];
      }
  }
}

template <bool SH>
__device__ __forceinline__ WinState lm_head(const BaDev& d, const LMOpt& o, int w, int lane, WinState S, const BaWin& W) {
  if (S.relin) {
    double cost = 0.0, gm = 0.0, xn2 = 0.0;
    if (!SH) group_partials<0, 1, 2, true>(d.part, W.pblk_base, W.n_pblk, lane, cost, gm, xn2);
    const int cur = S.cur;
    for (int c = W.pose_base + lane; c < W.pose_base + W.n_poses; c += 64) {
      if (S.iter == 0) {
        const int dg[6] = {0, 6, 11, 15, 18, 20};
        for (int k = 0; k < 6; ++k) d.scale_pose[6 * c + k] = 1.0 / (1.0 + sqrt(d.U[21 * c + dg[k]]));
      }
      if (!d.cam_active[c]) continue;
      for (int k = 0; k < 6; ++k) {
        const double x = d.x_pose[cur][6 * c + k];
        gm = fmax(gm, fabs(x - (x + -d.V[6 * c + k])));
        xn2 += x * x;
      }
    }
    cost = wave_sum(cost); gm = wave_max(gm); xn2 = wave_sum(xn2);
    if (SH) { cost += d.wlin[2 * w]; xn2 += d.wlin[2 * w + 1]; gm = fmax(gm, d.wmax[w]); }
    S.cost = cost;
    S.gmax = gm;
    S.x_norm = sqrt(xn2);
    if (S.iter == 0) S.initial_cost = cost;
    S.last_successful = 1;
    S.relin = 0;
  }
  if (lane == 0) {
    if (S.iter >= o.max_iter) { S.done = 1; S.term = LORB_TERM_NO_CONVERGENCE; }
    else if (S.last_successful && S.gmax <= o.gtol) { S.done = 1; S.term = LORB_TERM_GRADIENT_TOL; }
    else if (S.radius <= o.min_radius) { S.done = 1; S.term = LORB_TERM_MIN_RADIUS; }
    else S.iter++;
    d.st[w] = S;
  }
  return S;
}

__host__ __device__ constexpr int chol2s_words(int n16, int bw) {
  return n16 * (bw + 1) + (n16 + 48) + 2 * 64 * 18 + 48 + 2 * 64 * 17 + 2;
}
constexpr int chol_lds_words(int n16, int bw) {
  const int w1 = n16 * (bw + 1) + 2 * n16 + 64 * 18, w2 = (n16 + 48) * (bw + 2) + 2 * 64 * 18 + 48;
  const int w3 = chol2s_words(n16, bw);
  return w1 > w2 ? (w1 > w3 ? w1 : w3) : (w2 > w3 ? w2 : w3);
}

constexpr int kGrpMax = 4;
struct BaGrp {
  BaDev d[kGrpMax];
  int n;
};
struct GrpGrid {
  int pre[kGrpMax + 1];
};
struct GrpInit {
  int W[kGrpMax], ctot[kGrpMax], n_pt[kGrpMax], nf[kGrpMax];
};
__device__ __forceinline__ int grp_member(const GrpGrid& G, int n, unsigned b, unsigned& lb) {
  int k = 0;
#pragma unroll
  for (int i = 1; i < kGrpMax; ++i) k += (i < n && (int)b >= G.pre[i]) ? 1 : 0;
  lb = b - (unsigned)G.pre[k];
  return k;
}


constexpr int kLdsBudget = 160 * 1024 - 2048;
struct CholShape { int W, max_env, max_env_w, max_bw; };
void launch_chol(int kind, const CholShape& sh, hipStream_t s, const BaDev& d, const LMOpt& o, bool head);
void launch_chol_2s_g(hipStream_t s, const BaGrp& g, const GrpGrid& G, const LMOpt& o, bool head, size_t lds);

}
}
```

### lorb_slam_amd/csrc/lorb_ba_plan.h

```cpp
#pragma once
#include "lorb_ba_dev.h"

#include <algorithm>
#include <cstring>
#include <vector>

namespace lorb::ba {

inline bool env_flag(const char* name) { const char* e = getenv(name); return e && e[0] == '1'; }

inline size_t dbg_words(size_t windows, size_t stamp_slots) {
#ifdef LORB_CHOL_TRACE
  return windows * 512;
#elif defined(LORB_LS_STAMPS)
  return stamp_slots * 8;
#else
  return windows * 8;
#endif
}

struct GraphCache {
  const char* what;
  hipGraph_t graph = nullptr;
  hipGraphExec_t exec = nullptr;
  bool valid = false;
  int captures = 0;
  int kernel_nodes = 0;
  explicit GraphCache(const char* what_) : what(what_) {}
  GraphCache(const GraphCache&) = delete;
  GraphCache& operator=(const GraphCache&) = delete;
  ~GraphCache() { destroy(); }
  void invalidate() { valid = false; }
  template <typename F, typename R>
  int replay_or_capture(lorb_ctx* ctx, bool same, F enqueue, R remember) {
    if (!valid || !same) {
      destroy();
      LORB_HIP(ctx, hipStreamBeginCapture(ctx->stream, hipStreamCaptureModeThreadLocal));
      const int rc = enqueue();
      hipGraph_t g = nullptr;
      const hipError_t e = hipStreamEndCapture(ctx->stream, &g);
      if (rc != LORB_OK) { if (g) (void)hipGraphDestroy(g); return rc; }
      if (e != hipSuccess) return lorb::set_error(ctx, LORB_E_DEVICE, "%s capture failed: %s", what, hipGetErrorString(e));
      graph = g;
      LORB_HIP(ctx, hipGraphInstantiate(&exec, graph, nullptr, nullptr, 0));
      {
        size_t nn = 0;
        LORB_HIP(ctx, hipGraphGetNodes(graph, nullptr, &nn));
        std::vector<hipGraphNode_t> nodes(nn);
        if (nn) LORB_HIP(ctx, hipGraphGetNodes(graph, nodes.data(), &nn));
        kernel_nodes = 0;
        for (size_t i = 0; i < nn; ++i) {
          hipGraphNodeType ty;
          LORB_HIP(ctx, hipGraphNodeGetType(nodes[i], &ty));
          kernel_nodes += ty == hipGraphNodeTypeKernel;
        }
      }
      remember();
      valid = true;
      captures++;
    }
    LORB_HIP(ctx, hipGraphLaunch(exec, ctx->stream));
    return LORB_OK;
  }

 private:
  void destroy() {
    if (exec) { (void)hipGraphExecDestroy(exec); exec = nullptr; }
    if (graph) { (void)hipGraphDestroy(graph); graph = nullptr; }
    valid = false;
  }
};

}

struct lorb_ba_devbuild;

struct lorb_ba_plan {
  lorb_ctx* ctx = nullptr;
  int W = 0, Ctot = 0, Ptot = 0, K = 0, NF = 0, n_pblk = 0, n_bp = 0, n_pairs = 0;
  int env_total = 0, n_total = 0, max_env = 0, max_bw = 0, max_env_w = 0, min_n16 = 1 << 30;
  int min_bw = 1 << 30;
  double hp_us = 0.0, hp_sec[6] = {};
  int hp_n = 0;
  std::vector<lorb::ba::BaWin> hwin;
  std::vector<void*> allocs;
  lorb::ba::BaDev dev{};
  lorb::ba::WinState* d_state = nullptr;
  lorb::ba::GraphCache cache{"graph"};
  lorb::ba::LMOpt graph_opt{};
  unsigned gen = 0;
  struct GraphKey {
    int kind = -1, lds = 0, memset_env = 0, env_total = 0, grid_pblk = 0, grid_bp = 0, pt_launch = 0, x2_n = 0;
    int red_wide = 0, sup = 0, grid_sg = 0;
    int fold = 0;
    bool operator==(const GraphKey& o) const { return memcmp(this, &o, sizeof(GraphKey)) == 0; }
  } gkey;
  int grid_pblk = 0, grid_bp = 0;
  int grid_sg = 0;
  bool has_super = false;
  bool fold = false;
  int pt_launch = 0;
  int* live = nullptr;
  lorb_comm* comm = nullptr;
  double *x2_send = nullptr, *x2_recv = nullptr;
  size_t fx_n = 0;
  size_t x2_off = 0;
  std::vector<std::vector<int>> cam_map;
  int chol_kind = -1;
  lorb_ba_devbuild* devb = nullptr;
  ~lorb_ba_plan();
};
```

### lorb_slam_amd/csrc/lorb_internal.h

```cpp
#pragma once

#include <hip/hip_runtime.h>

#include <cstdarg>
#include <cstdint>
#include <cstdio>
#include <cstring>
#include <new>
#include <string>
#include <vector>

#include "../../include/lorb_c.h"

struct lorb_ctx {
  int device = 0;
  hipStream_t stream = nullptr;
  std::string err;
  hipEvent_t ev[64] = {};
  static constexpr int kScratch = 128;
  void* scratch[kScratch] = {};
  size_t scratch_sz[kScratch] = {};
  std::vector<unsigned char> up_mirror[kScratch];
  bool ktime = false;
  std::vector<hipEvent_t> kev_pool;
  std::vector<std::pair<hipEvent_t, hipEvent_t>> kev[LORB_K_COUNT];
  size_t tkey_ready = 0;
  void* tkey_buf = nullptr;
  void* done_buf = nullptr;
  void* pinned = nullptr;
  size_t pinned_sz = 0;
  hipEvent_t spin_ev = nullptr;
  lorb_ba_solver* solver = nullptr;
  void* io_in = nullptr;
  void* io_in_dev = nullptr;
  size_t io_in_sz = 0;
  void* io_out = nullptr;
  void* io_out_dev = nullptr;
  size_t io_out_sz = 0;
  bool io_pending = false;
  void* zero_ss = nullptr;
  size_t zero_ss_sz = 0;
};

namespace lorb {
inline hipError_t spin_wait(hipEvent_t ev) {
  hipError_t e;
  while ((e = hipEventQuery(ev)) == hipErrorNotReady) {
  }
  return e;
}
inline hipError_t spin_sync(lorb_ctx* ctx) {
  hipError_t e = hipEventRecord(ctx->spin_ev, ctx->stream);
  if (e != hipSuccess) return e;
  return spin_wait(ctx->spin_ev);
}
}

struct lorb_comm {
  lorb_ctx* ctx = nullptr;
  int nranks = 1, rank = 0;
  bool rccl = false;
  void* nccl = nullptr;
  lorb_host_allreduce_fn fn = nullptr;
  void* user = nullptr;
  double* pinned = nullptr;
  size_t pinned_n = 0;
  double* dbuf = nullptr;
  size_t dbuf_n = 0;
};

namespace lorb {

int set_error(lorb_ctx* ctx, int code, const char* fmt, ...);
int comm_allreduce(lorb_comm* comm, const double* d_send, double* d_recv, size_t n, int op);
int comm_allreduce_host(lorb_comm* comm, double* h_buf, size_t n, int op);

#define LORB_HIP(ctx, call)                                                              \
  do {                                                                                   \
    hipError_t e_ = (call);                                                              \
    if (e_ != hipSuccess)                                                                \
      return ::lorb::set_error((ctx), LORB_E_DEVICE, "%s failed: %s (%s:%d)", #call,    \
                               hipGetErrorString(e_), __FILE__, __LINE__);               \
  } while (0)

#define LORB_CHECK_LAUNCH(ctx) LORB_HIP(ctx, hipGetLastError())

#define LORB_TRY(expr)          \
  do {                          \
    int rc_ = (expr);           \
    if (rc_ != LORB_OK) return rc_; \
  } while (0)

int ba_plan_result64_dev(lorb_ba_plan* P, double* d_out);
int ba_plan_result_ring_dev(lorb_ba_plan* P, float* ring, int R, int t0, float* d_point_out);
void ba_plan_sorted_hint(lorb_ba_plan* P, bool sorted);
int ba_plan_update_dev_issue(lorb_ba_plan* P, const lorb_ba_window_dev* w);
int ba_plan_update_dev_finish(lorb_ba_plan* P, const lorb_ba_window_dev* w);
void ba_plan_window_counts(const lorb_ba_plan* P, int* n_points, int* n_obs);
const int* ba_plan_point_offsets(const lorb_ba_plan* P);

int match1_keys_dev(lorb_ctx* ctx, const uint8_t* d_q, int nq, const uint8_t* d_t, int nt,
                    unsigned long long** qkey_out, hipStream_t stream = nullptr);
int match1_keys_into(lorb_ctx* ctx, const uint8_t* d_q, int nq, const uint8_t* d_t, int nt,
                     unsigned long long* qkey, uint32_t* tkey, hipStream_t st);

int scratch(lorb_ctx* ctx, int slot, size_t bytes, void** out);
template <typename T>
int scratch_t(lorb_ctx* ctx, int slot, size_t count, T** out) {
  void* p = nullptr;
  int rc = scratch(ctx, slot, count * sizeof(T) + 16, &p);
  *out = static_cast<T*>(p);
  return rc;
}

int upload(lorb_ctx* ctx, int slot, const void* host, size_t bytes, void** dev);
template <typename T>
int upload_t(lorb_ctx* ctx, int slot, const T* host, size_t count, T** dev) {
  void* p = nullptr;
  if (host == nullptr || count == 0) { *dev = nullptr; return scratch(ctx, slot, 16, &p) == LORB_OK ? (*dev = nullptr, LORB_OK) : LORB_E_DEVICE; }
  int rc = upload(ctx, slot, host, count * sizeof(T), &p);
  *dev = static_cast<T*>(p);
  return rc;
}

class InPack {
 public:
  explicit InPack(lorb_ctx* c) : ctx(c) {}
  int add(const void* host, size_t bytes) {
    parts.push_back({host, bytes, total});
    total += (bytes + 255) & ~size_t(255);
    return (int)parts.size() - 1;
  }
  template <typename T>
  int add_t(const T* host, size_t count) { return add(host, host ? count * sizeof(T) : 0); }
  int commit(bool mapped = false);
  template <typename T>
  T* dev(int i) const { return parts[i].bytes ? reinterpret_cast<T*>(static_cast<unsigned char*>(base) + parts[i].off) : nullptr; }

 private:
  struct Part { const void* host; size_t bytes, off; };
  lorb_ctx* ctx;
  std::vector<Part> parts;
  size_t total = 0;
  void* base = nullptr;
};
class OutPack {
 public:
  explicit OutPack(lorb_ctx* c) : ctx(c) {}
  int add(size_t bytes) {
    parts.push_back({bytes, total});
    total += (bytes + 255) & ~size_t(255);
    return (int)parts.size() - 1;
  }
  int alloc(bool direct = false);
  int fetch();
  template <typename T>
  T* dev(int i) const { return reinterpret_cast<T*>(static_cast<unsigned char*>(dbase) + parts[i].off); }
  template <typename T>
  const T* host(int i) const { return reinterpret_cast<const T*>(static_cast<const unsigned char*>(hbase) + parts[i].off); }

 private:
  struct Part { size_t bytes, off; };
  lorb_ctx* ctx;
  std::vector<Part> parts;
  size_t total = 0;
  void* dbase = nullptr;
  void* hbase = nullptr;
  bool direct = false;
};

struct KernelTimer {
  lorb_ctx* ctx; int k; hipEvent_t b = nullptr, e = nullptr;
  KernelTimer(lorb_ctx* c, int kid);
  ~KernelTimer();
};

inline unsigned ceil_div(size_t a, size_t b) { return static_cast<unsigned>((a + b - 1) / b); }

__device__ __forceinline__ int block_excl_scan_1024(int v, int* wsum, int* total) {
  const int lane = threadIdx.x & 63, wv = threadIdx.x >> 6;
  int incl = v;
#pragma unroll
  for (int o = 1; o < 64; o <<= 1) {
    const int u = __shfl_up(incl, o, 64);
    if (lane >= o) incl += u;
  }
  if (lane == 63) wsum[wv] = incl;
  __syncthreads();
  int pre = 0, tot = 0;
#pragma unroll
  for (int w = 0; w < 16; ++w) {
    const int s = wsum[w];
    pre += w < wv ? s : 0;
    tot += s;
  }
  __syncthreads();
  *total = tot;
  return pre + incl - v;
}

template <int NT>
__device__ __forceinline__ int block_excl_scan(int v, int* wsum, int* total) {
  const int lane = threadIdx.x & 63, wv = threadIdx.x >> 6;
  int incl = v;
#pragma unroll
  for (int o = 1; o < 64; o <<= 1) {
    const int u = __shfl_up(incl, o, 64);
    if (lane >= o) incl += u;
  }
  if (lane == 63) wsum[wv] = incl;
  __syncthreads();
  int pre = 0, tot = 0;
#pragma unroll
  for (int w = 0; w < NT / 64; ++w) {
    const int s = wsum[w];
    pre += w < wv ? s : 0;
    tot += s;
  }
  __syncthreads();
  *total = tot;
  return pre + incl - v;
}

constexpr int kScanTile = 16384, kScanTileLds = kScanTile + kScanTile / 16;
__device__ __forceinline__ int wg_scan_tile(const int* __restrict__ in, int* __restrict__ out, int n, int carry,
                                            int* s_tile, int* wsum, int* mx = nullptr) {
  const int t = threadIdx.x;
  auto pad = [](int i) { return i + (i >> 4); };
#pragma unroll
  for (int u = 0; u < 4; ++u) {
    const int i = 4 * (t + 1024 * u);
    int4 v = make_int4(0, 0, 0, 0);
    if (i + 3 < n && ((reinterpret_cast<size_t>(in) & 15) == 0)) {
      v = *reinterpret_cast<const int4*>(in + i);
    } else {
      v.x = i < n ? in[i] : 0; v.y = i + 1 < n ? in[i + 1] : 0;
      v.z = i + 2 < n ? in[i + 2] : 0; v.w = i + 3 < n ? in[i + 3] : 0;
    }
    s_tile[pad(i)] = v.x; s_tile[pad(i + 1)] = v.y; s_tile[pad(i + 2)] = v.z; s_tile[pad(i + 3)] = v.w;
  }
  __syncthreads();
  int v[16], loc = 0, m = 0;
#pragma unroll
  for (int u = 0; u < 16; ++u) {
    v[u] = s_tile[17 * t + u];
    m = max(m, v[u]);
    loc += v[u];
// ... 236 lines not shown
```

### lorb_slam_amd/csrc/lorb_map.hip

```cpp
#include <algorithm>
#include <chrono>
#include <cstdlib>

#include "lorb_internal.h"

namespace {

struct MapDev {
  float* pos; uint8_t* desc; int* obs_pt; int* obs_kf; float* obs_uv;
  float* pos2; uint8_t* desc2; int* obs_pt2; int* obs_kf2; float* obs_uv2;
  int* obs_frame;
  int* cnt;
  int* flag_pt; int* newid; int* flag_obs; int* newpos;
  int* flag_new; int* newnew;
  int* tile_tot;
  float* ring;
  float* pose_init; float* fixed;
  int P_cap, K_cap, W, F, R;
};

struct Pose6 { float v[6]; };

__device__ __forceinline__ int ring_slot(int kf, int R) { const int r = kf % R; return r < 0 ? r + R : r; }

// ... 101 lines not shown
    if (nw) {
      p = pn++;
      float X[3];
      lorb::unproject_point(fx, fy, cx, cy, Twc, xq, yq, z, X);
      m.pos[3 * p + 0] = X[0]; m.pos[3 * p + 1] = X[1]; m.pos[3 * p + 2] = X[2];
      uint4* dd = reinterpret_cast<uint4*>(m.desc + 32 * (size_t)p);
      if constexpr (RM > 0) { dd[0] = d0[u]; dd[1] = d1[u]; }
      else {
        const uint4* sd = reinterpret_cast<const uint4*>(kdesc + 32 * (size_t)q);
        dd[0] = sd[0]; dd[1] = sd[1];
      }
    }
    const int k = ko++;
    m.obs_pt[k] = p;
    m.flag_new[p] = 1;
    m.obs_kf[k] = kf;
    m.obs_uv[2 * k + 0] = xq;
    m.obs_uv[2 * k + 1] = yq;
  }
  if (t == 0) {
    m.cnt[0] = P0 + tot.v[1]; m.cnt[1] = K0 + tot.v[0];
    m.cnt[3] = tot.v[1]; m.cnt[4] = tot.v[0]; m.cnt[5] = tot.v[2];
  }
}

__global__ __launch_bounds__(256) void k_map_cull(MapDev m, int Kb, int K0, int t0) {
  const int k = blockIdx.x * 256 + threadIdx.x, lane = threadIdx.x & 63;
  const int kc = min(m.cnt[1], Kb), k0 = min(K0, kc);
  const bool old = k < k0;
  int p = -1, kfv = 0, pprev = -1;
  if (k < kc) { p = m.obs_pt[k]; kfv = m.obs_kf[k]; }
  if (old && k > 0) pprev = m.obs_pt[k - 1];
  const bool start = old && (k == 0 || pprev != p);
  const unsigned long long B = __ballot(start || !old), Wb = __ballot(old && kfv >= t0);
  if (k > Kb) return;
  if (k >= kc) { m.flag_obs[k] = 0; return; }
  if (!old) {
    m.flag_obs[k] = kfv >= t0 - m.F;
    if (kfv >= t0) m.flag_pt[p] = 1;
    return;
  }
  const unsigned long long upto = lane == 63 ? ~0ull : (2ull << lane) - 1;
  const unsigned long long below = B & upto, above = B & ~upto;
  const int s0 = below ? 63 - __builtin_clzll(below) : 0;
  const int e0 = above ? __builtin_ctzll(above) : 64;
  const unsigned long long run = (e0 == 64 ? ~0ull : (1ull << e0) - 1) & ~((1ull << s0) - 1);
  bool keep = (Wb & run) != 0 || m.flag_new[p] != 0;
  const int wbase = k - lane;
  if (!below)
    for (int j = wbase - 1; !keep && j >= 0 && m.obs_pt[j] == p; --j) keep = m.obs_kf[j] >= t0;
  if (!above)
    for (int j = wbase + 64; !keep && j < k0 && m.obs_pt[j] == p; ++j) keep = m.obs_kf[j] >= t0;
  m.flag_obs[k] = keep && kfv >= t0 - m.F;
  if (start && keep) m.flag_pt[p] = 1;
}

__device__ __forceinline__ int tile_base(const int* tot, int tile) {
  int s = 0;
  for (int k = 0; k < tile; ++k) s += tot[k];
  return s;
}
__device__ __forceinline__ int new_id(const MapDev& m, int i) {
  return m.newid[i] + tile_base(m.tile_tot, i / lorb::kScanTile);
}
__device__ __forceinline__ int new_pos(const MapDev& m, int ntP, int i) {
  return m.newpos[i] + tile_base(m.tile_tot + 2 * ntP, i / lorb::kScanTile);
}
__device__ __forceinline__ int new_before(const MapDev& m, int ntP, int p) {
  return m.newnew[p] + tile_base(m.tile_tot + ntP, p / lorb::kScanTile);
}

__global__ __launch_bounds__(256) void k_map_compact(MapDev m, int Pb, int Kb, int K0, int P0, int t0, int ntP,
                                                     const int* __restrict__ pt_off) {
  const int i = blockIdx.x * 256 + threadIdx.x;
  if (blockIdx.x == 0) {
    if (i == 0) { m.cnt[0] = new_id(m, Pb); m.cnt[1] = new_pos(m, ntP, Kb); }
    for (int j = i; j < 6 * m.W; j += 256) m.pose_init[j] = m.ring[6 * ring_slot(t0 + j / 6, m.R) + j % 6];
    for (int j = i; j < 6 * m.F; j += 256) m.fixed[j] = m.ring[6 * ring_slot(t0 - 1 - j / 6, m.R) + j % 6];
  }
  const int fp = i < Pb ? m.flag_pt[i] : 0;
  if (i < Pb && m.flag_new[i]) m.flag_new[i] = 0;
  if (fp) {
    m.flag_pt[i] = 0;
    const int d = new_id(m, i);
    m.pos2[3 * d + 0] = m.pos[3 * i + 0];
    m.pos2[3 * d + 1] = m.pos[3 * i + 1];
    m.pos2[3 * d + 2] = m.pos[3 * i + 2];
    const uint4* s = reinterpret_cast<const uint4*>(m.desc + 32 * (size_t)i);
    uint4* o = reinterpret_cast<uint4*>(m.desc2 + 32 * (size_t)d);
    o[0] = s[0]; o[1] = s[1];
  }
  if (i < Kb && m.flag_obs[i]) {
    const int p = m.obs_pt[i], kf = m.obs_kf[i];
    int d;
    if (i < K0) {
      d = new_pos(m, ntP, i) + new_before(m, ntP, p);
    } else {
      int lo = 0, hi = K0;
      if (pt_off) {
        lo = pt_off[min(p + 1, P0)];
      } else {
        while (lo < hi) {
          const int mid = (lo + hi) >> 1;
          if (m.obs_pt[mid] <= p) lo = mid + 1; else hi = mid;
        }
      }
      d = new_pos(m, ntP, lo) + new_before(m, ntP, p);
    }
    m.obs_pt2[d] = new_id(m, p);
    m.obs_kf2[d] = kf;
    m.obs_uv2[2 * d + 0] = m.obs_uv[2 * i + 0];
    m.obs_uv2[2 * d + 1] = m.obs_uv[2 * i + 1];
    m.obs_frame[d] = kf >= t0 ? kf - t0 : -1 - (t0 - 1 - kf);
  }
}

__global__ __launch_bounds__(1024) void k_map_scans(MapDev m, int Pb, int Kb, int ntP) {
  __shared__ int wsum[16];
  __shared__ int s_tile[lorb::kScanTileLds];
  const int seg = (int)blockIdx.x < ntP ? 0 : (int)blockIdx.x < 2 * ntP ? 1 : 2;
  const int tile = blockIdx.x - seg * ntP;
  const int n = seg < 2 ? Pb + 1 : Kb + 1, base = tile * lorb::kScanTile;
  const int* in = seg == 0 ? m.flag_pt : seg == 1 ? m.flag_new : m.flag_obs;
  int* out = seg == 0 ? m.newid : seg == 1 ? m.newnew : m.newpos;
  const int tot = lorb::wg_scan_tile(in + base, out + base, min(n - base, lorb::kScanTile), 0, s_tile, wsum);
  if (threadIdx.x == 0) m.tile_tot[blockIdx.x] = tot;
}

}

struct lorb_map {
  lorb_ctx* ctx = nullptr;
  MapDev m{};
  int t0 = 0;
  int h_P = 0, h_K = 0;
  int n_cap = 0, last_n = 0;
  float fx = 0, fy = 0, cx = 0, cy = 0;
  bool prof = false;
  double prof_ms[8] = {};
  int prof_n = 0;
  std::chrono::steady_clock::time_point prof_clk{};
  int* mt = nullptr;
  unsigned long long* qkey = nullptr;
  uint32_t* tkey = nullptr;
  int* pinned = nullptr;
  lorb_ba_plan* plan = nullptr;
  bool plan_ok = false;
  bool broken = false;
  bool overlap = false;
  hipStream_t side = nullptr;
  hipEvent_t ev_built = nullptr, ev_app = nullptr;
  bool built = false;
  int n_overlapped = 0;
  std::vector<void*> allocs;
  ~lorb_map() {
    if (prof && prof_n)
      fprintf(stderr, "lorb_map profile over %d steps (ms/step): match %.3f unproject %.3f append %.3f slide %.3f "
              "plan %.3f solve %.3f writeback %.3f\n", prof_n, prof_ms[0] / prof_n, prof_ms[1] / prof_n,
              prof_ms[2] / prof_n, prof_ms[3] / prof_n, prof_ms[4] / prof_n, prof_ms[5] / prof_n, prof_ms[6] / prof_n);
    if (side) (void)hipStreamSynchronize(side);
    if (plan) (void)lorb_ba_plan_destroy(plan);
    if (pinned) (void)hipHostFree(pinned);
    if (ev_built) (void)hipEventDestroy(ev_built);
    if (ev_app) (void)hipEventDestroy(ev_app);
    if (side) (void)hipStreamDestroy(side);
    for (void* p : allocs) (void)hipFree(p);
  }
};

namespace {

template <typename T>
int malloc_n(lorb_map* M, size_t n, T** out) {
  void* p = nullptr;
  LORB_HIP(M->ctx, hipMalloc(&p, std::max<size_t>(n, 1) * sizeof(T)));
  M->allocs.push_back(p);
  *out = static_cast<T*>(p);
  return LORB_OK;
}

int map_alloc(lorb_map* M, const lorb_map_init* in) {
  MapDev& m = M->m;
  m.P_cap = in->max_points; m.K_cap = in->max_obs; m.W = in->n_window; m.F = in->n_fixed;
  m.R = in->n_window + in->n_fixed + 1;
  const size_t P = (size_t)m.P_cap, K = (size_t)m.K_cap;
  LORB_TRY(malloc_n(M, 3 * P, &m.pos)); LORB_TRY(malloc_n(M, 3 * P, &m.pos2));
  LORB_TRY(malloc_n(M, 32 * P, &m.desc)); LORB_TRY(malloc_n(M, 32 * P, &m.desc2));
  LORB_TRY(malloc_n(M, K, &m.obs_pt)); LORB_TRY(malloc_n(M, K, &m.obs_pt2));
  LORB_TRY(malloc_n(M, K, &m.obs_kf)); LORB_TRY(malloc_n(M, K, &m.obs_kf2));
  LORB_TRY(malloc_n(M, 2 * K, &m.obs_uv)); LORB_TRY(malloc_n(M, 2 * K, &m.obs_uv2));
  LORB_TRY(malloc_n(M, K, &m.obs_frame));
  LORB_TRY(malloc_n(M, (size_t)8, &m.cnt));
  LORB_TRY(malloc_n(M, P + 1, &m.flag_pt)); LORB_TRY(malloc_n(M, P + 1, &m.newid));
  LORB_HIP(M->ctx, hipMemsetAsync(m.flag_pt, 0, sizeof(int) * ((size_t)P + 1), M->ctx->stream));
  LORB_TRY(malloc_n(M, P + 1, &m.flag_new)); LORB_TRY(malloc_n(M, P + 1, &m.newnew));
  LORB_HIP(M->ctx, hipMemsetAsync(m.flag_new, 0, sizeof(int) * ((size_t)P + 1), M->ctx->stream));
  LORB_TRY(malloc_n(M, K + 1, &m.flag_obs)); LORB_TRY(malloc_n(M, K + 1, &m.newpos));
  LORB_TRY(malloc_n(M, 2 * (P + 1) / lorb::kScanTile + (K + 1) / lorb::kScanTile + 4, &m.tile_tot));
  LORB_TRY(malloc_n(M, 6 * (size_t)m.R, &m.ring));
  LORB_TRY(malloc_n(M, 6 * (size_t)m.W, &m.pose_init));
  LORB_TRY(malloc_n(M, 6 * (size_t)std::max(m.F, 1), &m.fixed));
  const size_t n = (size_t)std::max(in->max_keypoints, 1);
  M->n_cap = (int)n;
  LORB_TRY(malloc_n(M, n, &M->mt));
  LORB_TRY(malloc_n(M, n, &M->qkey));
  LORB_TRY(malloc_n(M, P, &M->tkey));
  LORB_HIP(M->ctx, hipMemsetAsync(M->tkey, 0xff, sizeof(uint32_t) * std::max<size_t>(P, 1), M->ctx->stream));
  LORB_HIP(M->ctx, hipHostMalloc(reinterpret_cast<void**>(&M->pinned), sizeof(int) * 8));
  return LORB_OK;
}

lorb_ba_window_dev window_of(const lorb_map* M) {
  const MapDev& m = M->m;
  lorb_ba_window_dev w{};
  w.n_poses = m.W; w.n_fixed = m.F; w.max_points = m.P_cap; w.max_obs = m.K_cap;
  w.d_n_points = m.cnt; w.d_n_obs = m.cnt + 1;
  w.fx = M->fx; w.fy = M->fy; w.cx = M->cx; w.cy = M->cy;
  w.d_pose_init = m.pose_init; w.d_fixed_pose = m.fixed; w.d_point_init = m.pos;
  w.d_obs_point = m.obs_pt; w.d_obs_frame = m.obs_frame; w.d_obs_uv = m.obs_uv;
  return w;
}

int map_slide(lorb_map* M, int t0, int Pb, int Kb, int K0, int P0, const int* pt_off) {
  lorb_ctx* ctx = M->ctx;
  hipStream_t s = ctx->stream;
  MapDev& m = M->m;
  hipLaunchKernelGGL(k_map_cull, dim3(lorb::ceil_div(Kb + 1, 256)), dim3(256), 0, s, m, Kb, std::min(K0, Kb), t0);
  const int ntP = lorb::ceil_div(Pb + 1, lorb::kScanTile), ntK = lorb::ceil_div(Kb + 1, lorb::kScanTile);
  hipLaunchKernelGGL(k_map_scans, dim3(2 * ntP + ntK), dim3(1024), 0, s, m, Pb, Kb, ntP);
  const int nmax = std::max(std::max(Pb, Kb), 1);
  hipLaunchKernelGGL(k_map_compact, dim3(lorb::ceil_div(nmax, 256)), dim3(256), 0, s, m, Pb, Kb, std::min(K0, Kb), P0, t0,
                     ntP, pt_off);
  LORB_CHECK_LAUNCH(ctx);
  std::swap(m.pos, m.pos2); std::swap(m.desc, m.desc2); std::swap(m.obs_pt, m.obs_pt2);
  std::swap(m.obs_kf, m.obs_kf2); std::swap(m.obs_uv, m.obs_uv2);
  M->t0 = t0;
  return LORB_OK;
}

}

extern "C" {

int lorb_map_create(lorb_ctx* ctx, const lorb_map_init* in, lorb_map** out) {
  if (!ctx || !in || !out) return LORB_E_INVALID;
  *out = nullptr;
  if (in->n_window < 1 || in->n_fixed < 0 || in->n_points < 0 || in->n_obs < 0 || in->max_keypoints < 0 ||
      in->n_points > in->max_points || in->n_obs > in->max_obs || !in->pose ||
      (in->n_fixed > 0 && !in->fixed_pose) ||
      (in->n_points > 0 && (!in->point || !in->point_desc)) ||
      (in->n_obs > 0 && (!in->obs_point || !in->obs_kf || !in->obs_uv)))
    return lorb::set_error(ctx, LORB_E_INVALID, "lorb_map_create: bad sizes or missing arrays");
  const int W = in->n_window, F = in->n_fixed;
  for (int k = 0; k < in->n_obs; ++k) {
    if (in->obs_point[k] < 0 || in->obs_point[k] >= in->n_points)
      return lorb::set_error(ctx, LORB_E_INVALID, "observation %d: point %d outside [0, %d)", k, in->obs_point[k], in->n_points);
    if (in->obs_kf[k] < -F || in->obs_kf[k] >= W)
      return lorb::set_error(ctx, LORB_E_INVALID, "observation %d: keyframe %d outside [-%d, %d)", k, in->obs_kf[k], F, W);
  }
  lorb_map* M = new (std::nothrow) lorb_map();
  if (!M) return LORB_E_NOMEM;
  M->ctx = ctx;
  {
    const char* e = getenv("LORB_MAP_PROFILE");
    M->prof = e && e[0] == '1';
  }
  M->fx = in->fx; M->fy = in->fy; M->cx = in->cx; M->cy = in->cy;
  int rc = map_alloc(M, in);
  if (rc == LORB_OK) {
    hipStream_t s = ctx->stream;
    MapDev& m = M->m;
    std::vector<float> ring(6 * (size_t)m.R, 0.0f);
    for (int j = 0; j < W; ++j)
      for (int q = 0; q < 6; ++q) ring[6 * (size_t)(j % m.R) + q] = in->pose[6 * (size_t)j + q];
    for (int j = 0; j < F; ++j)
      for (int q = 0; q < 6; ++q) ring[6 * (size_t)(((-1 - j) % m.R + m.R) % m.R) + q] = in->fixed_pose[6 * (size_t)j + q];
    const int cnt[8] = {in->n_points, in->n_obs, 0, 0, 0, 0, 0, 0};
    auto up = [&](void* d, const void* h, size_t bytes) -> int {
      if (bytes) LORB_HIP(ctx, hipMemcpyAsync(d, h, bytes, hipMemcpyHostToDevice, s));
      return LORB_OK;
    };
    rc = up(m.ring, ring.data(), sizeof(float) * ring.size());
    if (rc == LORB_OK) rc = up(m.cnt, cnt, sizeof(cnt));
    if (rc == LORB_OK) rc = up(m.pos, in->point, sizeof(float) * 3 * (size_t)in->n_points);
    if (rc == LORB_OK) rc = up(m.desc, in->point_desc, 32 * (size_t)in->n_points);
    std::vector<int> ord(in->n_obs);
    for (int k = 0; k < in->n_obs; ++k) ord[k] = k;
    std::stable_sort(ord.begin(), ord.end(), [&](int a, int b) { return in->obs_point[a] < in->obs_point[b]; });
    std::vector<int> op(in->n_obs), ok(in->n_obs);
    std::vector<float> ouv(2 * (size_t)in->n_obs);
    for (int k = 0; k < in->n_obs; ++k) {
      op[k] = in->obs_point[ord[k]]; ok[k] = in->obs_kf[ord[k]];
      ouv[2 * k] = in->obs_uv[2 * ord[k]]; ouv[2 * k + 1] = in->obs_uv[2 * ord[k] + 1];
    }
    if (rc == LORB_OK) rc = up(m.obs_pt, op.data(), sizeof(int) * (size_t)in->n_obs);
    if (rc == LORB_OK) rc = up(m.obs_kf, ok.data(), sizeof(int) * (size_t)in->n_obs);
    if (rc == LORB_OK) rc = up(m.obs_uv, ouv.data(), sizeof(float) * 2 * (size_t)in->n_obs);
    if (rc == LORB_OK) {
      rc = map_slide(M, 0, in->n_points, in->n_obs, in->n_obs, in->n_points, nullptr);
      M->h_P = in->n_points; M->h_K = in->n_obs;
    }
    if (rc == LORB_OK) {
      const lorb_ba_window_dev w = window_of(M);
      rc = lorb_ba_plan_create_dev(ctx, &w, &M->plan);
      if (rc == LORB_OK) lorb::ba_plan_sorted_hint(M->plan, true);
      M->plan_ok = rc == LORB_OK;
    }
    if (rc == LORB_OK) {
      LORB_HIP(ctx, hipMemcpyAsync(M->pinned, m.cnt, sizeof(int) * 8, hipMemcpyDeviceToHost, s));
      LORB_HIP(ctx, hipStreamSynchronize(s));
      M->h_P = M->pinned[0]; M->h_K = M->pinned[1];
    }
  }
  if (rc != LORB_OK) { delete M; return rc; }
  *out = M;
  return LORB_OK;
}

}

namespace {

int map_mark(lorb_map* M, int i) {
  if (!M->prof) return LORB_OK;
  LORB_HIP(M->ctx, hipStreamSynchronize(M->ctx->stream));
  const auto now = std::chrono::steady_clock::now();
  M->prof_ms[i] += std::chrono::duration<double, std::milli>(now - M->prof_clk).count();
  M->prof_clk = now;
  return LORB_OK;
}

int map_build_fail(lorb_map* M, int rc) {
  M->built = false;
  hipStream_t s = M->ctx->stream;
  if (hipMemcpyAsync(M->pinned, M->m.cnt, sizeof(int) * 8, hipMemcpyDeviceToHost, s) == hipSuccess &&
      hipStreamSynchronize(s) == hipSuccess) {
    M->h_P = M->pinned[0]; M->h_K = M->pinned[1];
  } else {
    M->broken = true;
  }
  return rc;
}

int map_build_done(lorb_map* M) {
  lorb_ctx* ctx = M->ctx;
  M->plan_ok = true;
  if (!M->ev_built) LORB_HIP(ctx, hipEventCreateWithFlags(&M->ev_built, hipEventDisableTiming));
  LORB_HIP(ctx, hipEventRecord(M->ev_built, ctx->stream));
  M->built = true;
  LORB_TRY(map_mark(M, 4));
  lorb::ba_plan_window_counts(M->plan, &M->h_P, &M->h_K);
  return LORB_OK;
}

int map_prepare(lorb_map* M, const lorb_frame_params* frame, const float pose[6], const float Tcw[16], int32_t n,
                const uint8_t* d_desc, const float* d_x, const float* d_y, const float* d_depth, bool split = false) {
  if (!M || !frame || !pose || !Tcw || n < 0) return LORB_E_INVALID;
  lorb_ctx* ctx = M->ctx;
  if (n > M->n_cap) return lorb::set_error(ctx, LORB_E_INVALID, "%d keypoints > the map's max_keypoints %d", n, M->n_cap);
  if (n > 0 && (!d_desc || !d_x || !d_y || !d_depth)) return LORB_E_INVALID;
  if (M->broken) return lorb::set_error(ctx, LORB_E_DEVICE, "the map is unusable after an earlier failed step");
  hipStream_t s = ctx->stream;
  MapDev& m = M->m;
  const int kf = M->t0 + m.W;
  M->prof_clk = std::chrono::steady_clock::now();
  auto mark = [&](int i) { return map_mark(M, i); };
  LORB_TRY(mark(7));
  const bool ovl = M->overlap && M->built && !M->prof && !ctx->ktime;
  if (ovl && !M->side) {
    LORB_HIP(ctx, hipStreamCreateWithFlags(&M->side, hipStreamNonBlocking));
    LORB_HIP(ctx, hipEventCreateWithFlags(&M->ev_app, hipEventDisableTiming));
  }
  hipStream_t ms = ovl ? M->side : s;
  M->n_overlapped += ovl;
  if (ovl) LORB_HIP(ctx, hipStreamWaitEvent(ms, M->ev_built, 0));
  unsigned long long* qkey = nullptr;
  const bool has_t = M->h_P > 0;
  if (n > 0 && has_t) {
    if (const int rc = lorb::match1_keys_into(ctx, d_desc, n, m.desc, M->h_P, M->qkey, M->tkey, ms); rc != LORB_OK) {
      if (hipMemsetAsync(M->tkey, 0xff, sizeof(uint32_t) * std::max<size_t>(m.P_cap, 1), ms) != hipSuccess) M->broken = true;
      return rc;
    }
    qkey = M->qkey;
  }
  LORB_TRY(mark(0));
  LORB_TRY(mark(1));
  Pose6 p6;
  for (int q = 0; q < 6; ++q) p6.v[q] = pose[q];
  lorb::Mat4f Twc;
  lorb::inv4_lu32f(Tcw, Twc.v);
#define LORB_APPEND(RM)                                                                                       \
  hipLaunchKernelGGL(k_map_append<RM>, dim3(1), dim3(1024), 0, ms, m, n, kf, p6, (const unsigned long long*)qkey, \
                     (int)(has_t && qkey), M->mt, Twc, frame->fx, frame->fy, frame->cx, frame->cy, d_desc, d_x, d_y, \
                     d_depth)
  if (n <= 1024) LORB_APPEND(1);
  else if (n <= 2048) LORB_APPEND(2);
  else if (n <= 4096) LORB_APPEND(4);
  else LORB_APPEND(0);
#undef LORB_APPEND
  if (hipGetLastError() != hipSuccess) {
    M->broken = true;
    return lorb::set_error(ctx, LORB_E_DEVICE, "k_map_append launch failed; the map is unusable");
  }
  if (ovl) {
    LORB_HIP(ctx, hipEventRecord(M->ev_app, ms));
    LORB_HIP(ctx, hipStreamWaitEvent(s, M->ev_app, 0));
  }
  M->last_n = n;
  if (M->h_P + n > m.P_cap || M->h_K + n > m.K_cap) {
    LORB_HIP(ctx, hipMemcpyAsync(M->pinned, m.cnt, sizeof(int) * 8, hipMemcpyDeviceToHost, s));
    LORB_HIP(ctx, hipStreamSynchronize(s));
    if (M->pinned[2] & 1)
      return lorb::set_error(ctx, LORB_E_NOMEM, "map capacity exceeded (points %d + %d new / %d, observations %d + %d new / %d)",
                             M->h_P, n, m.P_cap, M->h_K, n, m.K_cap);
  }
  LORB_TRY(mark(2));
  LORB_TRY(map_slide(M, M->t0 + 1, std::min(M->h_P + n, m.P_cap), std::min(M->h_K + n, m.K_cap), M->h_K, M->h_P,
                      M->plan_ok ? lorb::ba_plan_point_offsets(M->plan) : nullptr));
  LORB_TRY(mark(3));
  const lorb_ba_window_dev w = window_of(M);
  M->plan_ok = false;
  if (split) {
    if (const int rc = lorb::ba_plan_update_dev_issue(M->plan, &w); rc != LORB_OK) return map_build_fail(M, rc);
    return LORB_OK;
  }
  if (const int rc = lorb_ba_plan_update_dev(M->plan, &w); rc != LORB_OK) return map_build_fail(M, rc);
  return map_build_done(M);
}

int map_build_finish(lorb_map* M) {
  const lorb_ba_window_dev w = window_of(M);
  if (const int rc = lorb::ba_plan_update_dev_finish(M->plan, &w); rc != LORB_OK) return map_build_fail(M, rc);
  return map_build_done(M);
}

int map_finish(lorb_map* M) {
  LORB_TRY(lorb::ba_plan_result_ring_dev(M->plan, M->m.ring, M->m.R, M->t0, M->m.pos));
  LORB_TRY(map_mark(M, 6));
  if (M->prof) M->prof_n++;
  return LORB_OK;
}

}

constexpr int kMapGrp = 4;
struct lorb_map_group {
  std::vector<lorb_map*> maps;
  std::vector<lorb_ba_group*> bag;
  int n_steps_fused = 0;
  ~lorb_map_group() {
    for (lorb_ba_group* g : bag) (void)lorb_ba_group_destroy(g);
  }
};

extern "C" {

int lorb_map_step_dev(lorb_map* M, const lorb_frame_params* frame, const float pose[6], const float Tcw[16], int32_t n,
                      const uint8_t* d_desc, const float* d_x, const float* d_y, const float* d_depth,
                      const lorb_lm_options* opt) {
  if (!M || !opt) return LORB_E_INVALID;
  LORB_TRY(map_prepare(M, frame, pose, Tcw, n, d_desc, d_x, d_y, d_depth));
  LORB_TRY(lorb_ba_plan_solve(M->plan, opt));
  LORB_TRY(map_mark(M, 5));
  return map_finish(M);
}

int lorb_map_set_overlap(lorb_map* M, int32_t enable) {
  if (!M || (enable != 0 && enable != 1)) return LORB_E_INVALID;
  M->overlap = enable == 1;
  if (!M->overlap && M->side) {
    LORB_HIP(M->ctx, hipStreamSynchronize(M->side));
  }
  return LORB_OK;
}

int lorb_map_counts(lorb_map* M, int32_t* out, int32_t n) {
  if (!M || !out || n < 0) return LORB_E_INVALID;
  lorb_ctx* ctx = M->ctx;
  LORB_HIP(ctx, hipMemcpyAsync(M->pinned, M->m.cnt, sizeof(int) * 8, hipMemcpyDeviceToHost, ctx->stream));
  LORB_HIP(ctx, hipStreamSynchronize(ctx->stream));
  const int32_t v[9] = {M->pinned[0], M->pinned[1], M->t0, M->last_n, M->pinned[3], M->pinned[4], M->pinned[5], M->m.W,
                        M->n_overlapped};
  for (int i = 0; i < n && i < 9; ++i) out[i] = v[i];
  return LORB_OK;
}

int lorb_map_read(lorb_map* M, const lorb_map_state* st) {
  if (!M || !st) return LORB_E_INVALID;
  lorb_ctx* ctx = M->ctx;
  hipStream_t s = ctx->stream;
  const MapDev& m = M->m;
  int32_t c[8];
  LORB_TRY(lorb_map_counts(M, c, 8));
  const size_t P = (size_t)c[0], K = (size_t)c[1];
  auto down = [&](void* h, const void* d, size_t bytes) -> int {
    if (h && bytes) LORB_HIP(ctx, hipMemcpyAsync(h, d, bytes, hipMemcpyDeviceToHost, s));
    return LORB_OK;
  };
  LORB_TRY(down(st->point, m.pos, sizeof(float) * 3 * P));
  LORB_TRY(down(st->point_desc, m.desc, 32 * P));
  LORB_TRY(down(st->obs_point, m.obs_pt, sizeof(int) * K));
  LORB_TRY(down(st->obs_kf, m.obs_kf, sizeof(int) * K));
  LORB_TRY(down(st->obs_uv, m.obs_uv, sizeof(float) * 2 * K));
  LORB_TRY(down(st->obs_frame, m.obs_frame, sizeof(int) * K));
  LORB_TRY(down(st->match_train, M->mt, sizeof(int) * (size_t)M->last_n));
  std::vector<float> ring(6 * (size_t)m.R);
  LORB_TRY(down(ring.data(), m.ring, sizeof(float) * ring.size()));
  LORB_HIP(ctx, hipStreamSynchronize(s));
  auto slot = [&](int kf) { return ((kf % m.R) + m.R) % m.R; };
  if (st->pose)
    for (int j = 0; j < m.W; ++j)
      for (int q = 0; q < 6; ++q) st->pose[6 * j + q] = ring[6 * (size_t)slot(M->t0 + j) + q];
  if (st->fixed_pose)
    for (int j = 0; j < m.F; ++j)
      for (int q = 0; q < 6; ++q) st->fixed_pose[6 * j + q] = ring[6 * (size_t)slot(M->t0 - 1 - j) + q];
  if (st->summary && M->plan) LORB_TRY(lorb_ba_plan_read(M->plan, nullptr, nullptr, st->summary));
  return LORB_OK;
}

int lorb_map_plan(lorb_map* M, lorb_ba_plan** out) {
  if (!M || !out) return LORB_E_INVALID;
  *out = M->plan;
  return LORB_OK;
}

int lorb_map_destroy(lorb_map* M) {
  if (!M) return LORB_E_INVALID;
  (void)hipStreamSynchronize(M->ctx->stream);
  delete M;
  return LORB_OK;
}

int lorb_map_group_create(int32_t n_maps, lorb_map* const* maps, lorb_map_group** out) {
  if (n_maps < 1 || !maps || !out || !maps[0]) return LORB_E_INVALID;
  *out = nullptr;
  lorb_ctx* ctx = maps[0]->ctx;
  for (int i = 0; i < n_maps; ++i) {
    if (!maps[i]) return lorb::set_error(ctx, LORB_E_INVALID, "lorb_map_group_create: map %d is null", i);
    if (maps[i]->ctx != ctx) return lorb::set_error(ctx, LORB_E_INVALID, "lorb_map_group_create: map %d is on another context", i);
    for (int j = 0; j < i; ++j)
      if (maps[j] == maps[i]) return lorb::set_error(ctx, LORB_E_INVALID, "lorb_map_group_create: map %d appears twice", i);
  }
  lorb_map_group* G = new (std::nothrow) lorb_map_group();
  if (!G) return LORB_E_NOMEM;
  G->maps.assign(maps, maps + n_maps);
  for (int i0 = 0; i0 < n_maps; i0 += kMapGrp) {
    std::vector<lorb_ba_plan*> plans;
    for (int i = i0; i < std::min(n_maps, i0 + kMapGrp); ++i) plans.push_back(maps[i]->plan);
    lorb_ba_group* g = nullptr;
    if (const int rc = lorb_ba_group_create(ctx, (int32_t)plans.size(), plans.data(), &g); rc != LORB_OK) {
      delete G;
      return rc;
    }
    G->bag.push_back(g);
  }
  *out = G;
  return LORB_OK;
}

int lorb_map_group_step_dev(lorb_map_group* G, const lorb_map_keyframe* kfs, const lorb_lm_options* opt) {
  if (!G || !kfs || !opt) return LORB_E_INVALID;
  const int n = (int)G->maps.size();
  int rc = LORB_OK, ready = n;
  for (int i = 0; i < n; ++i) {
    const lorb_map_keyframe& k = kfs[i];
    rc = map_prepare(G->maps[i], k.frame, k.pose, k.Tcw, k.n, k.d_desc, k.d_x, k.d_y, k.d_depth, true);
    if (rc != LORB_OK) { ready = i; break; }
  }
  std::vector<char> built(ready, 0);
  bool all = ready == n;
  for (int i = 0; i < ready; ++i) {
    const int r = map_build_finish(G->maps[i]);
    built[i] = r == LORB_OK;
    if (r != LORB_OK) {
      all = false;
      if (rc == LORB_OK) rc = r;
    }
  }
  if (all) {
    bool fused = true;
    for (lorb_ba_group* g : G->bag) {
      int32_t before[2], after[2];
      LORB_TRY(lorb_ba_group_info(g, before, 2));
      LORB_TRY(lorb_ba_group_solve(g, opt));
      LORB_TRY(lorb_ba_group_info(g, after, 2));
      fused = fused && after[1] > before[1];
    }
    G->n_steps_fused += fused;
  } else {
    for (int i = 0; i < ready; ++i)
      if (built[i]) LORB_TRY(lorb_ba_plan_solve(G->maps[i]->plan, opt));
  }
  for (int i = 0; i < ready; ++i)
    if (built[i]) LORB_TRY(map_finish(G->maps[i]));
  return rc;
}

int lorb_map_group_info(lorb_map_group* G, int32_t* info, int32_t n) {
  if (!G || !info || n < 0) return LORB_E_INVALID;
  int32_t caps = 0;
  for (lorb_ba_group* g : G->bag) {
    int32_t v[3];
    LORB_TRY(lorb_ba_group_info(g, v, 3));
    caps += v[2];
  }
  const int32_t v[4] = {(int32_t)G->maps.size(), (int32_t)G->bag.size(), G->n_steps_fused, caps};
  for (int i = 0; i < n && i < 4; ++i) info[i] = v[i];
  return LORB_OK;
}

int lorb_map_group_destroy(lorb_map_group* G) {
  if (!G) return LORB_E_INVALID;
  delete G;
  return LORB_OK;
}

}
```

### lorb_slam_amd/runtime.py

```python
import ctypes as C
import os

import numpy as np

from . import _abi as A

_HERE = os.path.dirname(os.path.abspath(__file__))
LIB_PATH = os.environ.get("LORB_LIB_PATH") or os.path.join(_HERE, "liblorb.so")
_lib = None


class LorbError(RuntimeError):
    pass


def lib():
    global _lib
    if _lib is None:
        if not os.path.exists(LIB_PATH):
            raise LorbError(f"{LIB_PATH} not built: run `make -C lorb_slam_amd/csrc` (hipcc, gfx950)")
        L = C.CDLL(LIB_PATH)
        L.lorb_last_error.restype = C.c_char_p
        L.lorb_last_error.argtypes = [C.c_void_p]
        for name in ("lorb_create", "lorb_destroy", "lorb_sync", "lorb_malloc", "lorb_free",
# ... 264 lines not shown
            ctx.check(lib().lorb_ba_plan_create_sharded(ctx.handle, comm.handle, C.c_int32(len(wins)), arr,
                                                        C.byref(self._p)), "lorb_ba_plan_create_sharded")

    def solve(self, opt=None):
        opt = opt or A.LMOptions.default()
        self.ctx.check(lib().lorb_ba_plan_solve(self._p, C.byref(opt)), "lorb_ba_plan_solve")

    def read(self):
        wins = self.wins
        poses = [np.zeros((len(w["pose_init"]), 6)) for w in wins]
        pts = [np.zeros((len(w["point_init"]), 3)) for w in wins]
        pp = (A.f64p * max(1, len(wins)))(*[A.ptr(p, C.c_double) for p in poses])
        qp = (A.f64p * max(1, len(wins)))(*[A.ptr(p, C.c_double) for p in pts])
        summ = (A.BASummary * max(1, len(wins)))()
        self.ctx.check(lib().lorb_ba_plan_read(self._p, pp, qp, summ), "lorb_ba_plan_read")
        return poses, pts, [summ[i].as_dict() for i in range(len(wins))]

    def trace(self, w=0):
        buf, n = (A.LMIteration * A.LM_TRACE_CAP)(), C.c_int32()
        self.ctx.check(lib().lorb_ba_plan_trace(self._p, C.c_int32(w), buf, C.c_int32(A.LM_TRACE_CAP), C.byref(n)),
                       "lorb_ba_plan_trace")
        return A.trace_list(buf, n.value)

    def info(self):
        v = (C.c_int32 * 11)()
        self.ctx.check(lib().lorb_ba_plan_info(self._p, v, C.c_int32(11)), "lorb_ba_plan_info")
        keys = ("band", "cholesky", "blocks", "point_groups", "observations", "points", "cameras", "reordered",
                "point_major", "red_threads", "partial_runs")
        return dict(zip(keys, [int(x) for x in v]))

    def close(self):
        if self._p:
            lib().lorb_ba_plan_destroy(self._p)
            self._p = C.c_void_p()

    def __del__(self):
        try:
            self.close()
        except Exception:
            pass


class BASolver:

    INFO_KEYS = ("resident_plans", "plan_creations", "host_plan_fallback", "band", "cholesky", "reordered")

    def __init__(self, ctx):
        self.ctx = ctx
        self._p = C.c_void_p()
        ctx.check(lib().lorb_ba_solver_create(ctx.handle, C.byref(self._p)), "lorb_ba_solver_create")

    def prepare(self, w):
        keep = A.KeepAlive()
        arr = A.make_windows([w], keep)
        pose = np.zeros((len(w["pose_init"]), 6))
        pts = np.zeros((len(w["point_init"]), 3))
        return (arr, keep, pose, pts, A.BASummary())

    def solve_prepared(self, prep, opt):
        arr, _, pose, pts, summ = prep
        self.ctx.check(lib().lorb_ba_solver_solve(self._p, arr, C.byref(opt), A.ptr(pose, C.c_double),
                                                  A.ptr(pts, C.c_double), C.byref(summ)), "lorb_ba_solver_solve")
        return pose, pts, summ.as_dict()

    def solve(self, w, opt=None):
        return self.solve_prepared(self.prepare(w), opt or A.LMOptions.default())

    def trace(self):
        buf, n = (A.LMIteration * A.LM_TRACE_CAP)(), C.c_int32()
        self.ctx.check(lib().lorb_ba_solver_trace(self._p, buf, C.c_int32(A.LM_TRACE_CAP), C.byref(n)),
                       "lorb_ba_solver_trace")
        return A.trace_list(buf, n.value)

    def info(self):
        v = (C.c_int32 * 6)()
        self.ctx.check(lib().lorb_ba_solver_info(self._p, v, C.c_int32(6)), "lorb_ba_solver_info")
        return dict(zip(self.INFO_KEYS, [int(x) for x in v]))

    def close(self):
        if self._p:
            lib().lorb_ba_solver_destroy(self._p)
            self._p = C.c_void_p()

    def __del__(self):
        try:
            self.close()
        except Exception:
            pass


class BAPlanDev(BAPlan):

    def __init__(self, ctx, arrays, n_poses, n_fixed, intr, comm=None):
        self.ctx, self.comm, self._keep = ctx, comm, A.KeepAlive()
        self._p = C.c_void_p()
        self.n_poses, self.n_fixed = n_poses, n_fixed
        self.win = self._window(arrays, intr)
        if comm is None:
            ctx.check(lib().lorb_ba_plan_create_dev(ctx.handle, C.byref(self.win), C.byref(self._p)),
                      "lorb_ba_plan_create_dev")
        else:
            ctx.check(lib().lorb_ba_plan_create_sharded_dev(ctx.handle, comm.handle, C.byref(self.win), C.byref(self._p)),
                      "lorb_ba_plan_create_sharded_dev")

    @staticmethod
    def upload(ctx, w, extra_points=0, extra_obs=0):
        P, K = len(w["point_init"]), len(w["obs_point"])

        def pad(a, n):
            a = np.asarray(a)
            return np.concatenate([a, np.zeros((n - len(a),) + a.shape[1:], a.dtype)])
        return dict(n_points=ctx.to_device(np.array([P], np.int32)), n_obs=ctx.to_device(np.array([K], np.int32)),
                    pose_init=ctx.to_device(A.f32(w["pose_init"]).reshape(-1, 6)),
                    fixed_pose=ctx.to_device(A.f32(w["fixed_pose"]).reshape(-1, 6)),
                    point_init=ctx.to_device(pad(A.f32(w["point_init"]).reshape(-1, 3), max(P + extra_points, 1))),
                    obs_point=ctx.to_device(pad(A.i32(w["obs_point"]), max(K + extra_obs, 1))),
                    obs_frame=ctx.to_device(pad(A.i32(w["obs_frame"]), max(K + extra_obs, 1))),
                    obs_uv=ctx.to_device(pad(A.f32(w["obs_uv"]).reshape(-1, 2), max(K + extra_obs, 1))))

    def _window(self, a, intr):
        self.arrays = a
        w = A.BAWindowDev()
        w.n_poses, w.n_fixed = self.n_poses, self.n_fixed
        w.max_points, w.max_obs = a["point_init"].shape[0], a["obs_point"].shape[0]
        w.d_n_points, w.d_n_obs = a["n_points"].ptr, a["n_obs"].ptr
        w.fx, w.fy, w.cx, w.cy = (float(v) for v in intr)
        for k in ("pose_init", "fixed_pose", "point_init", "obs_point", "obs_frame", "obs_uv"):
            setattr(w, "d_" + k, a[k].ptr)
        return w

    def update(self, arrays=None, intr=None):
        if arrays is not None:
            self.win = self._window(arrays, intr if intr is not None else (self.win.fx, self.win.fy, self.win.cx, self.win.cy))
        self.ctx.check(lib().lorb_ba_plan_update_dev(self._p, C.byref(self.win)), "lorb_ba_plan_update_dev")

    def read(self):
        info = self.info()
        poses = np.zeros((self.n_poses, 6)); pts = np.zeros((max(info["points"], 1), 3))
        pp = (A.f64p * 1)(A.ptr(poses, C.c_double))
        qp = (A.f64p * 1)(A.ptr(pts, C.c_double))
        summ = (A.BASummary * 1)()
        self.ctx.check(lib().lorb_ba_plan_read(self._p, pp, qp, summ), "lorb_ba_plan_read")
        return [poses], [pts[:info["points"]]], [summ[0].as_dict()]

    def result_dev(self, d_pose, d_points):
        self.ctx.check(lib().lorb_ba_plan_result_dev(self._p, d_pose.ptr if d_pose is not None else None,
                                                     d_points.ptr if d_points is not None else None),
                       "lorb_ba_plan_result_dev")


class LocalMap:

    COUNT_KEYS = ("points", "observations", "t0", "keypoints", "new_points", "new_observations", "matches", "window",
                  "overlapped_steps")

    def __init__(self, ctx, init, max_points=None, max_obs=None, max_keypoints=4096):
        self.ctx, self._keep = ctx, A.KeepAlive()
        k = self._keep.keep
        s = A.MapInit()
        s.n_window, s.n_fixed = len(init["pose_init"]), len(init["fixed_pose"])
        s.n_points, s.n_obs = len(init["point_init"]), len(init["obs_point"])
        s.max_points = int(max_points or 2 * s.n_points + 8 * max_keypoints)
        s.max_obs = int(max_obs or 2 * s.n_obs + 8 * max_keypoints)
        s.max_keypoints = int(max_keypoints)
        s.fx, s.fy, s.cx, s.cy = (float(v) for v in init["intr"])
        s.pose = A.ptr(k(A.f32(init["pose_init"])), C.c_float)
        s.fixed_pose = A.ptr(k(A.f32(init["fixed_pose"]).reshape(-1, 6)), C.c_float)
        s.point = A.ptr(k(A.f32(init["point_init"])), C.c_float)
        s.point_desc = A.ptr(k(A.u8(init["point_desc"])), C.c_uint8)
        s.obs_point = A.ptr(k(A.i32(init["obs_point"])), C.c_int32)
        s.obs_kf = A.ptr(k(A.i32(init["obs_kf"])), C.c_int32)
        s.obs_uv = A.ptr(k(A.f32(init["obs_uv"])), C.c_float)
        self.W, self.F, self.max_keypoints = s.n_window, s.n_fixed, s.max_keypoints
        self._p = C.c_void_p()
        ctx.check(lib().lorb_map_create(ctx.handle, C.byref(s), C.byref(self._p)), "lorb_map_create")
        self._keep.clear()

    def set_overlap(self, enable=True):
        self.ctx.check(lib().lorb_map_set_overlap(self._p, C.c_int32(1 if enable else 0)), "lorb_map_set_overlap")

    def step_dev(self, fp, pose, Tcw, n, d_desc, d_x, d_y, d_depth, opt=None):
        opt = opt or A.LMOptions.default()
        pose = A.f32(pose).reshape(6); T = A.f32(Tcw).reshape(16)
        self.ctx.check(lib().lorb_map_step_dev(self._p, C.byref(fp), A.ptr(pose, C.c_float), A.ptr(T, C.c_float),
                                               C.c_int32(n), d_desc.ptr, d_x.ptr, d_y.ptr, d_depth.ptr, C.byref(opt)),
                       "lorb_map_step_dev")

    def step(self, fp, kf, opt=None):
        fps = A.make_frame_params(fp) if isinstance(fp, dict) else fp
        arrs = [self.ctx.to_device(A.u8(kf["desc"])), self.ctx.to_device(A.f32(kf["x"])),
                self.ctx.to_device(A.f32(kf["y"])), self.ctx.to_device(A.f32(kf["depth"]))]
        try:
            self.step_dev(fps, kf["pose"], kf["Tcw"], len(kf["x"]), *arrs, opt=opt)
            self.ctx.sync()
        finally:
            for a in arrs:
                a.free()

    def counts(self):
        v = (C.c_int32 * 9)()
        self.ctx.check(lib().lorb_map_counts(self._p, v, C.c_int32(9)), "lorb_map_counts")
        return dict(zip(self.COUNT_KEYS, [int(x) for x in v]))

    def read(self):
        c = self.counts()
        P, K = c["points"], c["observations"]
        out = dict(point=np.zeros((max(P, 1), 3), np.float32), point_desc=np.zeros((max(P, 1), 32), np.uint8),
                   obs_point=np.zeros(max(K, 1), np.int32), obs_kf=np.zeros(max(K, 1), np.int32),
                   obs_uv=np.zeros((max(K, 1), 2), np.float32), obs_frame=np.zeros(max(K, 1), np.int32),
                   pose=np.zeros((self.W, 6), np.float32), fixed_pose=np.zeros((max(self.F, 1), 6), np.float32),
                   match_train=np.zeros(max(c["keypoints"], 1), np.int32))
        summ = A.BASummary()
        st = A.MapState()
        st.point = A.ptr(out["point"], C.c_float); st.point_desc = A.ptr(out["point_desc"], C.c_uint8)
        st.obs_point = A.ptr(out["obs_point"], C.c_int32); st.obs_kf = A.ptr(out["obs_kf"], C.c_int32)
        st.obs_uv = A.ptr(out["obs_uv"], C.c_float); st.obs_frame = A.ptr(out["obs_frame"], C.c_int32)
        st.pose = A.ptr(out["pose"], C.c_float); st.fixed_pose = A.ptr(out["fixed_pose"], C.c_float)
        st.match_train = A.ptr(out["match_train"], C.c_int32); st.summary = C.pointer(summ)
        self.ctx.check(lib().lorb_map_read(self._p, C.byref(st)), "lorb_map_read")
        for key, n in (("point", P), ("point_desc", P), ("obs_point", K), ("obs_kf", K), ("obs_uv", K),
                       ("obs_frame", K), ("fixed_pose", self.F), ("match_train", c["keypoints"])):
            out[key] = out[key][:n]
        out["summary"] = summ.as_dict()
        out.update(c)
        return out

    def trace(self):
        p = C.c_void_p()
        self.ctx.check(lib().lorb_map_plan(self._p, C.byref(p)), "lorb_map_plan")
        buf, n = (A.LMIteration * A.LM_TRACE_CAP)(), C.c_int32()
        self.ctx.check(lib().lorb_ba_plan_trace(p, C.c_int32(0), buf, C.c_int32(A.LM_TRACE_CAP), C.byref(n)),
                       "lorb_ba_plan_trace")
        return A.trace_list(buf, n.value)

    def plan_info(self):
        p = C.c_void_p()
        self.ctx.check(lib().lorb_map_plan(self._p, C.byref(p)), "lorb_map_plan")
        v = (C.c_int32 * 8)()
        self.ctx.check(lib().lorb_ba_plan_info(p, v, C.c_int32(8)), "lorb_ba_plan_info")
        keys = ("band", "cholesky", "blocks", "point_groups", "observations", "points", "cameras", "reordered")
        return dict(zip(keys, [int(x) for x in v]))

    def close(self):
        if self._p:
            lib().lorb_map_destroy(self._p)
            self._p = C.c_void_p()

    def __del__(self):
        try:
            self.close()
        except Exception:
            pass


class BAGroup:

    def __init__(self, ctx, plans):
        self.ctx, self.plans = ctx, list(plans)
        arr = (C.c_void_p * len(self.plans))(*[p._p for p in self.plans])
        self._p = C.c_void_p()
        ctx.check(lib().lorb_ba_group_create(ctx.handle, C.c_int32(len(self.plans)), arr, C.byref(self._p)),
                  "lorb_ba_group_create")

    def solve(self, opt=None):
        opt = opt or A.LMOptions.default()
        self.ctx.check(lib().lorb_ba_group_solve(self._p, C.byref(opt)), "lorb_ba_group_solve")

    def info(self):
        v = (C.c_int32 * 3)()
        self.ctx.check(lib().lorb_ba_group_info(self._p, v, C.c_int32(3)), "lorb_ba_group_info")
        return dict(zip(("plans", "fused_solves", "captures"), [int(x) for x in v]))

    def close(self):
        if self._p:
            lib().lorb_ba_group_destroy(self._p)
            self._p = C.c_void_p()

    def __del__(self):
        try:
            self.close()
        except Exception:
            pass


class MapGroup:

    def __init__(self, maps):
        self.maps = list(maps)
        self.ctx = self.maps[0].ctx
        arr = (C.c_void_p * len(self.maps))(*[m._p for m in self.maps])
        self._p = C.c_void_p()
        self.ctx.check(lib().lorb_map_group_create(C.c_int32(len(self.maps)), arr, C.byref(self._p)),
                       "lorb_map_group_create")

    def step_dev(self, fp, kfs, opt=None):
        opt = opt or A.LMOptions.default()
        arr = (A.MapKeyframe * len(self.maps))()
        keep = []
        for k, (pose, Tcw, n, dd, dx, dy, dz) in zip(arr, kfs):
            pose = A.f32(pose).reshape(6); T = A.f32(Tcw).reshape(16)
            keep += [pose, T]
            k.frame = C.pointer(fp); k.pose = A.ptr(pose, C.c_float); k.Tcw = A.ptr(T, C.c_float); k.n = int(n)
            k.d_desc, k.d_x, k.d_y, k.d_depth = dd.ptr, dx.ptr, dy.ptr, dz.ptr
        self.ctx.check(lib().lorb_map_group_step_dev(self._p, arr, C.byref(opt)), "lorb_map_group_step_dev")

    def info(self):
        v = (C.c_int32 * 4)()
        self.ctx.check(lib().lorb_map_group_info(self._p, v, C.c_int32(4)), "lorb_map_group_info")
        return dict(zip(("maps", "plan_groups", "fused_steps", "captures"), [int(x) for x in v]))

    def close(self):
        if self._p:
            lib().lorb_map_group_destroy(self._p)
            self._p = C.c_void_p()

    def __del__(self):
        try:
            self.close()
        except Exception:
            pass


Context.ba_pose_only = _ba_pose_only
Context.ba_local = _ba_local

from . import window as _window
```

Baseline: 11530 BA iterations/s.

## Speculatively chain device BA build and solve with on-device certification gate

Adds a speculative path to the local-mapping step. When the window structure is unchanged, a certify kernel checks the new build header against the previous plan's adjacency, group counts and reduction config on device, then gathers the data and runs the solver without a host readback in between. A device gate flag makes the init and result kernels skip work if certification fails, and the host checks the record afterward, rebuilding and re-solving on a miss. This removes the host synchronization between build and solve, at the cost of wasted GPU work and a second solve whenever certification fails.

```diff
diff --git a/lorb_slam_amd/csrc/lorb_ba.hip b/lorb_slam_amd/csrc/lorb_ba.hip
--- a/lorb_slam_amd/csrc/lorb_ba.hip
+++ b/lorb_slam_amd/csrc/lorb_ba.hip
@@ -45,7 +45,13 @@
   }
   for (int k = i; k < 3 * n_pt; k += stride) d.x_pt[0][k] = d.x_init_pt[k];
 }
-__global__ __launch_bounds__(256) void k_ba_init(BaDev d, int W, int ctot, int n_pt, int nf, LMOpt o) {
+__global__ __launch_bounds__(256) void k_ba_init(BaDev d, int W, int ctot, int n_pt, int nf, LMOpt o,
+                                                 const int* __restrict__ gate) {
+  if (gate && *gate) {
+    const int i = blockIdx.x * blockDim.x + threadIdx.x;
+    if (i < W) d.st[i].done = 1;
+    return;
+  }
   init_run(d, W, ctot, n_pt, nf, o, blockIdx.x * blockDim.x + threadIdx.x, gridDim.x * blockDim.x);
 }
 
@@ -1287,10 +1293,7 @@
 }
 
 int red_threads(const lorb_ba_plan* P) {
-  const double W = std::max(P->W, 1), cams = std::max((double)P->Ctot / W, 1.0);
-  const double cand = (double)P->n_pblk / W * ((P->max_bw + 1) / 6.0) / cams;
-  if (P->grid_bp <= 256 || cand >= 128.0) return 1024;
-  return P->grid_bp <= 1024 ? 512 : 256;
+  return red_threads_rule(P->W, P->Ctot, P->n_pblk, P->max_bw, P->grid_bp);
 }
 template <int MODE>
 void launch_red(const lorb_ba_plan* P, hipStream_t s, const BaDev& d, const LMOpt& o) {
@@ -1408,7 +1411,7 @@
   {
     const int n = std::max(std::max(std::max(P->W, P->Ctot), P->NF), std::min(3 * P->pt_launch, 256 * 1024));
     hipLaunchKernelGGL(k_ba_init, dim3(lorb::ceil_div(std::max(n, 1), 256)), dim3(256), 0, ctx->stream, P->dev, P->W,
-                       P->Ctot, P->pt_launch, P->NF, o);
+                       P->Ctot, P->pt_launch, P->NF, o, (const int*)P->gate);
   }
   LORB_CHECK_LAUNCH(ctx);
   if (o.max_iter <= 0) return enqueue_linearize(P, o);
@@ -1463,6 +1466,10 @@
   return LORB_OK;
 }
 
+}
+
+namespace lorb::ba {
+lorb_ba_plan::GraphKey plan_graph_key(const lorb_ba_plan* P) { return graph_key(P); }
 }
 
 struct lorb_ba_group {
diff --git a/lorb_slam_amd/csrc/lorb_ba_build.hip b/lorb_slam_amd/csrc/lorb_ba_build.hip
--- a/lorb_slam_amd/csrc/lorb_ba_build.hip
+++ b/lorb_slam_amd/csrc/lorb_ba_build.hip
@@ -35,6 +35,9 @@
   std::vector<int> last_map;
   hipEvent_t rb_ev = nullptr;
   bool rb_pending = false, rb_sorted = false, rb_fuse = false;
+  int* rec = nullptr;
+  unsigned char* d_adj = nullptr;
+  bool adj_stale = true, accepted = false, rb_spec = false;
   ~lorb_ba_devbuild() {
     if (rb_ev) (void)hipEventDestroy(rb_ev);
     if (pinned) (void)hipHostFree(pinned);
@@ -202,11 +205,15 @@
   bw.part_base = total;
   total += (long long)bw.n_sg * bw.part_stride;
 }
-int sg_factor(int n_pblk) {
+__host__ __device__ inline int sg_factor_rule(int n_pblk, int forced) {
+  if (forced >= 1) return n_pblk > 1 ? forced : 1;
+  return n_pblk > 512 ? (n_pblk + 479) / 480 : 1;
+}
+int sg_forced() {
   const char* e = getenv("LORB_SG_F");
-  if (e && atoi(e) >= 1) return n_pblk > 1 ? atoi(e) : 1;
-  return n_pblk > 512 ? (n_pblk + 479) / 480 : 1;
-}
+  return e && atoi(e) >= 1 ? atoi(e) : 0;
+}
+int sg_factor(int n_pblk) { return sg_factor_rule(n_pblk, sg_forced()); }
 int part_budget_check(lorb_ctx* ctx, long long total) {
   if ((size_t)std::max(total, 1ll) * sizeof(double) > kPartBudgetBytes)
     return lorb::set_error(ctx, LORB_E_NOMEM, "point-group partials need %.1f GB (> %.0f GB budget)",
@@ -747,6 +754,7 @@
   int up_words;
   int sgf = 1, nsg = 0;
   int4* sgrp = nullptr;
+  int* gate = nullptr;
 };
 struct DbCams {
   int perm[kPmSpan], gcam[kPmSpan];
@@ -778,12 +786,12 @@
   s0 = __shfl(lo, 0, 64);
   s1 = __shfl(lo, 32, 64);
 }
-__global__ __launch_bounds__(256) void k_db_gather(lorb_ba_window_dev w, BaDev d, int K, const int* __restrict__ key,
-                                                   const int* __restrict__ val, DbFused f, DbCams cams) {
+__device__ __forceinline__ void db_gather_run(const lorb_ba_window_dev& w, const BaDev& d, const int K,
+                                              const int* __restrict__ key, const int* __restrict__ val, const DbFused& f,
+                                              const int* __restrict__ perm, const int* __restrict__ gcam) {
   const int gt = blockIdx.x * 256 + threadIdx.x, gs = gridDim.x * 256;
   for (int i = gt; i < f.up_words; i += gs) f.up_dst[i] = f.up_src[i];
-  const int* __restrict__ perm = cams.perm;
-  const int* __restrict__ gcam = cams.gcam;
+  if (gt == 0 && f.gate) *f.gate = 0;
   {
     const int m = max(max(6 * f.C, 6 * f.F), 3 * f.P);
     for (int i = gt; i < m; i += gs) {
@@ -819,10 +827,115 @@
     const_cast<double2*>(d.obs_uv)[e] = make_double2(w.d_obs_uv[2 * k], w.d_obs_uv[2 * k + 1]);
   }
 }
+__global__ __launch_bounds__(256) void k_db_gather(lorb_ba_window_dev w, BaDev d, int K, const int* __restrict__ key,
+                                                   const int* __restrict__ val, DbFused f, DbCams cams) {
+  db_gather_run(w, d, K, key, val, f, cams.perm, cams.gcam);
+}
+
+enum { kRecK, kRecP, kRecMaxk, kRecS, kRecG, kRecSF, kRecNSG, kRecNbp, kRecPairs, kRecBw, kRecPartLo, kRecPartHi,
+       kRecCertified, kRecGate, kDbRec = 16 };
+
+__global__ __launch_bounds__(256) void k_db_gather_spec(lorb_ba_window_dev w, BaDev d, DbFused f,
+                                                        const int* __restrict__ rec, const int* __restrict__ perm,
+                                                        const int* __restrict__ gcam) {
+  if (!rec[kRecCertified]) return;
+  f.P = rec[kRecP]; f.G = rec[kRecG]; f.S = rec[kRecS]; f.sgf = rec[kRecSF]; f.nsg = rec[kRecNSG];
+  db_gather_run(w, d, rec[kRecK], nullptr, nullptr, f, perm, gcam);
+}
+
+struct DbCert {
+  int C, P_cap, n_bp, pblk_cap, grid_bp, red_prev, had_groups, sg_forced;
+  long long gpart_cap;
+  const int *hdr, *cov, *cam_cnt;
+  const unsigned char* adj;
+  BaWin* win; int* live; const int* perm; int* gcam; BlockPair* bp;
+  int* rec;
+  int* host;
+};
+__global__ __launch_bounds__(1024) void k_db_certify(DbCert a) {
+  __shared__ int s_bad, s_inv[kPmSpan], s_wsum[16];
+  const int t = threadIdx.x, C = a.C, lane = t & 63, wv = t >> 6;
+  const int K = a.hdr[0], maxk = a.hdr[1], err = a.hdr[2], Pn = a.hdr[3];
+  const BaWin W = *a.win;
+  if (t == 0) s_bad = 0;
+  if (t < C) s_inv[a.perm[t]] = t;
+  for (int k = t; k < 8 + C * C + C; k += 1024) a.host[k] = a.hdr[k];
+  auto cov_of = [&](int i, int j) { return a.cov[max(i, j) * C + min(i, j)]; };
+  int bad = 0;
+  for (int k = t; k < C * C; k += 1024) {
+    const int i = k / C, j = k - i * C;
+    const int c = cov_of(i, j), cam = a.cam_cnt[i], ad = a.adj[k];
+    bad |= ad != (int)((i == j && cam > 0) || c > 0);
+  }
+  bool ok = err == 0 && Pn >= 0 && Pn <= a.P_cap && kGB - maxk >= 1;
+  int S = 0, G = 0, SF = 1, NSG = 0;
+  long long part_total = 0;
+  if (ok) {
+    S = kGB - (maxk + 1) + 1;
+    G = Pn > 0 ? (K + Pn - 1) / S + 1 : 0;
+    SF = sg_factor_rule(G, a.sg_forced);
+    NSG = G > 0 ? (G + SF - 1) / SF : 0;
+    part_total = (long long)NSG * W.part_stride;
+    const long long need = part_total > 1 ? part_total : 1;
+    ok = max(G, 1) <= a.pblk_cap && need <= a.gpart_cap && (size_t)need * sizeof(double) <= kPartBudgetBytes && SF == 1 &&
+         (G > 0) == (a.had_groups != 0) && red_threads_rule(1, C, G, W.bw, a.grid_bp) == a.red_prev;
+  }
+  const int nb = a.n_bp, per = (nb + 1023) / 1024, e0 = min(t * per, nb), e1 = min(e0 + per, nb);
+  int ch0 = 0, cl0 = 0;
+  if (e0 < e1) { ch0 = a.bp[e0].ch; cl0 = a.bp[e0].cl; }
+  __syncthreads();
+  if (bad) s_bad = 1;
+  auto cnt_of = [&](int e) {
+    const int ch = e == e0 ? ch0 : a.bp[e].ch, cl = e == e0 ? cl0 : a.bp[e].cl;
+    return ch == cl ? a.cam_cnt[s_inv[ch]] : cov_of(s_inv[ch], s_inv[cl]);
+  };
+  int sum = 0;
+  for (int e = e0; e < e1; ++e) sum += cnt_of(e);
+  int inc = sum;
+#pragma unroll
+  for (int o = 1; o < 64; o <<= 1) {
+    const int v = __shfl_up(inc, o, 64);
+    if (lane >= o) inc += v;
+  }
+  if (lane == 63) s_wsum[wv] = inc;
+  __syncthreads();
+  ok = ok && !s_bad;
+  int off = inc - sum, n_pairs = 0;
+#pragma unroll
+  for (int w = 0; w < 16; ++w) {
+    const int v = s_wsum[w];
+    if (w < wv) off += v;
+    n_pairs += v;
+  }
+  if (ok) {
+    for (int e = e0; e < e1; ++e) {
+      const int cnt = cnt_of(e);
+      a.bp[e].off = off; a.bp[e].cnt = cnt;
+      off += cnt;
+    }
+    if (t < C) a.gcam[t] = a.cam_cnt[t];
+  }
+  if (t == 0) {
+    if (ok) {
+      a.win->n_points = Pn; a.win->n_pblk = G; a.win->n_obs = K; a.win->n_obs_all = K; a.win->n_sg = NSG;
+      a.live[0] = G; a.live[1] = nb; a.live[2] = NSG;
+    }
+    int r[kDbRec] = {};
+    r[kRecK] = K; r[kRecP] = Pn; r[kRecMaxk] = maxk; r[kRecS] = S; r[kRecG] = G; r[kRecSF] = SF; r[kRecNSG] = NSG;
+    r[kRecNbp] = nb; r[kRecPairs] = n_pairs; r[kRecBw] = W.bw;
+    r[kRecPartLo] = (int)(part_total & 0xffffffffll); r[kRecPartHi] = (int)(part_total >> 32);
+    r[kRecCertified] = ok ? 1 : 0; r[kRecGate] = ok ? 0 : 1;
+#pragma unroll
+    for (int i = 0; i < kDbRec; ++i) { a.rec[i] = r[i]; a.host[8 + C * C + C + i] = r[i]; }
+  }
+}
 
 __global__ __launch_bounds__(256) void k_db_result(BaDev d, int C, int P, const int* __restrict__ perm,
                                                    float* __restrict__ pose_out, float* __restrict__ pt_out,
-                                                   float* __restrict__ ring, int R, int t0) {
+                                                   float* __restrict__ ring, int R, int t0,
+                                                   const int* __restrict__ gate) {
+  if (gate && *gate) return;
+  if (P < 0) P = d.win[0].n_points;
   const int i = blockIdx.x * 256 + threadIdx.x;
   const int cur = d.st[0].cur;
   if ((pose_out || ring) && i < 6 * C) {
@@ -876,13 +989,16 @@
     return lorb::set_error(ctx, LORB_E_UNSUPPORTED, "device-built plans hold windows of <= %d cameras (%d)", kPmSpan, b.C);
   LORB_TRY(dalloc(P, K, &b.key_out)); LORB_TRY(dalloc(P, K, &b.val_out));
   {
-    const size_t ints = ((Pn + 1 + 8 + C * C + C) + 1) & ~(size_t)1;
+    const size_t ints = ((Pn + 1 + 8 + C * C + C + kDbRec) + 1) & ~(size_t)1;
     b.scr_bytes = sizeof(int) * ints + sizeof(unsigned long long) * C * (size_t)b.Wd;
     unsigned char* m;
     LORB_TRY(dalloc(P, b.scr_bytes, &m));
     b.scr = reinterpret_cast<int*>(m);
     b.pt_cnt = b.scr; b.hdr = b.pt_cnt + Pn + 1; b.cov = b.hdr + 8; b.cam_cnt = b.cov + C * C;
+    b.rec = b.cam_cnt + C;
     b.bits = reinterpret_cast<unsigned long long*>(b.scr + ints);
+    LORB_TRY(dalloc(P, C * C, &b.d_adj));
+    if (!P->comm) P->gate = b.rec + kRecGate;
   }
   LORB_TRY(dalloc(P, K, &d.obs_pt)); LORB_TRY(dalloc(P, K, &d.obs_cam)); LORB_TRY(dalloc(P, K, &d.obs_fix));
   LORB_TRY(dalloc(P, K, &d.obs_uv)); LORB_TRY(dalloc(P, C, &d.cam_active));
@@ -944,18 +1060,18 @@
   return LORB_OK;
 }
 
-int db_phase1_issue(lorb_ctx* ctx, const lorb_ba_window_dev* w, lorb_ba_plan* P, bool sorted) {
+int db_phase1_issue(lorb_ctx* ctx, const lorb_ba_window_dev* w, lorb_ba_plan* P, bool sorted, const DbCert* cert = nullptr) {
   lorb_ba_devbuild& b = *P->devb;
   hipStream_t s = ctx->stream;
   BaDev& d = P->dev;
   const int C = b.C, F = b.F, Kc = w->max_obs;
   const size_t nrb = 8 + (size_t)C + (size_t)C * C;
   const int nb_obs = lorb::ceil_div(std::max(Kc, 1), 256), nb_pt = lorb::ceil_div(std::max(b.P_cap, 1), 256);
-  if (b.pinned_n < nrb) {
+  if (b.pinned_n < nrb + kDbRec) {
     if (b.pinned) (void)hipHostFree(b.pinned);
     b.pinned = nullptr; b.pinned_n = 0;
-    LORB_HIP(ctx, hipHostMalloc(reinterpret_cast<void**>(&b.pinned), sizeof(int) * nrb));
-    b.pinned_n = nrb;
+    LORB_HIP(ctx, hipHostMalloc(reinterpret_cast<void**>(&b.pinned), sizeof(int) * (nrb + kDbRec)));
+    b.pinned_n = nrb + kDbRec;
   }
   if (!b.rb_ev) LORB_HIP(ctx, hipEventCreateWithFlags(&b.rb_ev, hipEventDisableTiming));
   if (b.dirty) LORB_HIP(ctx, hipMemsetAsync(b.scr, 0, b.scr_bytes, s));
@@ -978,9 +1094,11 @@
   if (C > 0 && !fuse)
     hipLaunchKernelGGL(k_db_cov, dim3(lorb::ceil_div(C * (C + 1) / 2, 4)), dim3(256), 0, s, C, b.Wd, b.bits, b.cov,
                        b.cam_cnt);
+  if (cert) hipLaunchKernelGGL(k_db_certify, dim3(1), dim3(1024), 0, s, *cert);
   LORB_CHECK_LAUNCH(ctx);
-  LORB_HIP(ctx, hipMemcpyAsync(b.pinned, b.hdr, sizeof(int) * nrb, hipMemcpyDeviceToHost, s));
+  if (!cert) LORB_HIP(ctx, hipMemcpyAsync(b.pinned, b.hdr, sizeof(int) * nrb, hipMemcpyDeviceToHost, s));
   LORB_HIP(ctx, hipEventRecord(b.rb_ev, s));
+  b.rb_spec = cert != nullptr;
   b.rb_sorted = sorted;
   b.rb_fuse = fuse;
   b.rb_pending = true;
@@ -1000,6 +1118,7 @@
 
 int dev_build_issue(lorb_ctx* ctx, const lorb_ba_window_dev* w, lorb_ba_plan* P, int* lerr_out) {
   lorb_ba_devbuild& b = *P->devb;
+  b.accepted = false;
   const bool shape_ok = w->n_poses == b.C && w->n_fixed == b.F && w->max_obs <= b.K_cap && w->max_points <= b.P_cap;
   *lerr_out = shape_ok ? 0 : 32;
   if (!shape_ok && !P->comm)
@@ -1094,7 +1213,7 @@
   return LORB_OK;
 }
 
-void db_camera_order(lorb_ba_devbuild& b, const DbBuild& r) {
+bool db_same_adj(const lorb_ba_devbuild& b, const DbBuild& r) {
   const int C = b.C;
   bool same_adj = b.last_adj.size() == (size_t)C * C;
   for (int i = 0; i < C && same_adj; ++i) {
@@ -1103,7 +1222,12 @@
     for (int j = 0; j < C; ++j)
       if (last[j] != (char)((i == j && r.gcam[i] > 0) || row[j] > 0)) { same_adj = false; break; }
   }
-  if (!same_adj) {
+  return same_adj;
+}
+void db_camera_order(lorb_ba_devbuild& b, const DbBuild& r) {
+  const int C = b.C;
+  if (!db_same_adj(b, r)) {
+    b.adj_stale = true;
     std::vector<char> adj((size_t)C * C, 0);
     for (int i = 0; i < C; ++i)
       for (int j = 0; j < C; ++j) adj[(size_t)i * C + j] = (i == j && r.gcam[i] > 0) || r.gcov[(size_t)i * C + j] > 0;
@@ -1187,6 +1311,7 @@
   DbFused f{C, b.F, r.Pn, r.G, r.S, P->env_total, C * b.Wd, b.rb_sorted ? 1 : 0, b.bits, b.hdr, b.cov, C * C + C,
             reinterpret_cast<const int*>(b.up_host_dev), reinterpret_cast<int*>(b.up_dev), up_words};
   f.sgf = r.SF; f.nsg = r.NSG; f.sgrp = const_cast<int4*>(P->dev.sgrp);
+  f.gate = P->gate;
   DbCams cams;
   for (int c = 0; c < C; ++c) { cams.perm[c] = map[c]; cams.gcam[c] = r.gcam[c]; }
   const int NB = lorb::ceil_div(r.K, 256);
@@ -1214,6 +1339,94 @@
   hp.mark(3);
   db_stage_and_gather(ctx, w, P, r, hp);
   LORB_CHECK_LAUNCH(ctx);
+  b.accepted = true;
+  return LORB_OK;
+}
+
+
+int red_of(const lorb_ba_plan* P) { return red_threads_rule(P->W, P->Ctot, P->n_pblk, P->max_bw, P->grid_bp); }
+
+int spec_issue(lorb_ctx* ctx, const lorb_ba_window_dev* w, lorb_ba_plan* P, int obs_bound, bool* armed) {
+  lorb_ba_devbuild& b = *P->devb;
+  *armed = false;
+  const int C = b.C;
+  const bool shape_ok = w->n_poses == b.C && w->n_fixed == b.F && w->max_obs <= b.K_cap && w->max_points <= b.P_cap;
+  const bool chol_in_lds = sizeof(double) * (size_t)P->max_env <= (size_t)kLdsBudget;
+  if (P->comm || !b.accepted || !b.sorted_hint || b.dirty || !shape_ok || C < 1 || P->has_super || !chol_in_lds ||
+      !b.up_dev || P->n_bp < 1 || !P->gate || ctx->ktime)
+    return LORB_OK;
+  const BaWin& hw = P->hwin[0];
+  if (hw.fx != w->fx || hw.fy != w->fy || hw.cx != w->cx || hw.cy != w->cy) return LORB_OK;
+  hipStream_t s = ctx->stream;
+  if (b.adj_stale) {
+    if (b.last_adj.size() != (size_t)C * C) return LORB_OK;
+    LORB_HIP(ctx, hipMemcpyAsync(b.d_adj, b.last_adj.data(), (size_t)C * C, hipMemcpyHostToDevice, s));
+    b.adj_stale = false;
+  }
+  b.accepted = false;
+  DbCert a{};
+  a.C = C; a.P_cap = b.P_cap; a.n_bp = P->n_bp; a.pblk_cap = b.pblk_cap; a.grid_bp = P->grid_bp; a.red_prev = red_of(P);
+  a.had_groups = P->n_pblk > 0; a.sg_forced = sg_forced(); a.gpart_cap = (long long)b.gpart_cap;
+  a.hdr = b.hdr; a.cov = b.cov; a.cam_cnt = b.cam_cnt; a.adj = b.d_adj;
+  a.win = reinterpret_cast<BaWin*>(b.up_dev); a.live = reinterpret_cast<int*>(b.up_dev + b.off_live);
+  a.perm = b.perm; a.gcam = reinterpret_cast<int*>(b.up_dev + b.off_gcam);
+  a.bp = reinterpret_cast<BlockPair*>(b.up_dev + b.off_bp); a.rec = b.rec;
+  LORB_HIP(ctx, hipHostGetDevicePointer(reinterpret_cast<void**>(&a.host), b.pinned, 0));
+  LORB_TRY(db_phase1_issue(ctx, w, P, true, &a));
+  DbFused f{C, b.F, 0, 0, 1, P->env_total, C * b.Wd, 1, b.bits, b.hdr, b.cov, C * C + C, nullptr, nullptr, 0};
+  f.sgrp = const_cast<int4*>(P->dev.sgrp);
+  const int NB = lorb::ceil_div(std::max(std::min(obs_bound, b.K_cap), 1), 256);
+  hipLaunchKernelGGL(k_db_gather_spec, dim3(NB), dim3(256), 0, s, *w, P->dev, f, (const int*)b.rec, (const int*)b.perm,
+                     (const int*)a.gcam);
+  LORB_CHECK_LAUNCH(ctx);
+  *armed = true;
+  return LORB_OK;
+}
+
+int spec_land(lorb_ctx* ctx, const lorb_ba_window_dev* w, lorb_ba_plan* P, bool* certified, bool* mismatch) {
+  lorb_ba_devbuild& b = *P->devb;
+  *certified = *mismatch = false;
+  if (!b.rb_pending || !b.rb_spec) return lorb::set_error(ctx, LORB_E_INVALID, "no certified build was issued");
+  const int C = b.C;
+  const size_t nrb = 8 + (size_t)C + (size_t)C * C;
+  LORB_HIP(ctx, lorb::spin_wait(b.rb_ev));
+  int rec[kDbRec];
+  std::memcpy(rec, b.pinned + nrb, sizeof(rec));
+  auto differ = [&](const char* what, long long host, long long dev) {
+    *mismatch = true;
+    return lorb::set_error(ctx, LORB_E_DEVICE, "certified plan build: the host's %s (%lld) differs from the device's (%lld)",
+                           what, host, dev);
+  };
+  DbBuild r;
+  bool ok = b.pinned[2] == 0 && db_land(ctx, w, P, 0, LORB_OK, r) == LORB_OK;
+  if (ok) {
+    const int S = kGB - (r.maxk + 1) + 1, G = r.Pn > 0 ? (r.K + r.Pn - 1) / S + 1 : 0, SF = sg_factor(G);
+    const int NSG = G > 0 ? (G + SF - 1) / SF : 0;
+    const long long need = std::max((long long)NSG * P->hwin[0].part_stride, 1ll);
+    ok = db_same_adj(b, r) && std::max(G, 1) <= b.pblk_cap && (size_t)need <= b.gpart_cap &&
+         (size_t)need * sizeof(double) <= kPartBudgetBytes && SF == 1 && (G > 0) == (P->n_pblk > 0) &&
+         red_threads_rule(1, C, G, P->hwin[0].bw, P->grid_bp) == red_of(P);
+  }
+  if (ok != (rec[kRecCertified] != 0)) return differ("verdict", ok, rec[kRecCertified]);
+  if (!ok) return dev_build_finish(ctx, w, P, 0);
+  b.rb_pending = false;
+  const lorb_ba_plan::GraphKey key_before = lorb::ba::plan_graph_key(P);
+  db_camera_order(b, r);
+  P->cam_map.assign(1, b.last_map);
+  db_blocks(b, r);
+  if (db_layout(ctx, w, P, r) != LORB_OK) return differ("layout", 0, 1);
+  const long long dev_part = ((long long)rec[kRecPartHi] << 32) | (unsigned)rec[kRecPartLo];
+  const long long hv[] = {r.K, r.Pn, r.maxk, r.S, r.G, r.SF, r.NSG, (long long)r.bps.size(), r.n_pairs, r.bw, r.part_total};
+  const long long dv[] = {rec[kRecK], rec[kRecP], rec[kRecMaxk], rec[kRecS], rec[kRecG], rec[kRecSF], rec[kRecNSG],
+                          rec[kRecNbp], rec[kRecPairs], rec[kRecBw], dev_part};
+  const char* names[] = {"observations", "points", "largest point", "group bound", "point groups", "groups per run", "runs",
+                         "blocks", "pairs", "band", "partials"};
+  for (int i = 0; i < 11; ++i)
+    if (hv[i] != dv[i]) return differ(names[i], hv[i], dv[i]);
+  if (!(lorb::ba::plan_graph_key(P) == key_before)) return differ("launch shape", 1, 0);
+  b.dirty = false;
+  b.accepted = true;
+  *certified = true;
   return LORB_OK;
 }
 
@@ -1289,12 +1502,26 @@
 static dim3 result_grid(const lorb_ba_plan* P) {
   return dim3(lorb::ceil_div(std::max(std::max(6 * P->Ctot, 1), std::min(3 * P->Ptot, 256 * 1024)), 256));
 }
-int ba_plan_result_ring_dev(lorb_ba_plan* P, float* ring, int R, int t0, float* d_point_out) {
+int ba_plan_result_ring_dev(lorb_ba_plan* P, float* ring, int R, int t0, float* d_point_out, int spec_points) {
   if (!P || !P->devb || !ring || R < 1) return LORB_E_INVALID;
-  hipLaunchKernelGGL(k_db_result, result_grid(P), dim3(256), 0, P->ctx->stream, P->dev, P->Ctot, P->Ptot,
-                     P->devb->perm, (float*)nullptr, d_point_out, ring, R, t0);
+  if (spec_points >= 0) {
+    const dim3 grid(lorb::ceil_div(std::max(std::max(6 * P->Ctot, 1), std::min(3 * spec_points, 256 * 1024)), 256));
+    hipLaunchKernelGGL(k_db_result, grid, dim3(256), 0, P->ctx->stream, P->dev, P->Ctot, -1, P->devb->perm,
+                       (float*)nullptr, d_point_out, ring, R, t0, (const int*)P->gate);
+  } else {
+    hipLaunchKernelGGL(k_db_result, result_grid(P), dim3(256), 0, P->ctx->stream, P->dev, P->Ctot, P->Ptot,
+                       P->devb->perm, (float*)nullptr, d_point_out, ring, R, t0, (const int*)nullptr);
+  }
   LORB_CHECK_LAUNCH(P->ctx);
   return LORB_OK;
+}
+int ba_plan_spec_issue(lorb_ba_plan* P, const lorb_ba_window_dev* w, int obs_bound, bool* armed) {
+  if (!P || !w || !armed || !P->devb) return LORB_E_INVALID;
+  return spec_issue(P->ctx, w, P, obs_bound, armed);
+}
+int ba_plan_spec_land(lorb_ba_plan* P, const lorb_ba_window_dev* w, bool* certified, bool* mismatch) {
+  if (!P || !w || !certified || !mismatch || !P->devb) return LORB_E_INVALID;
+  return spec_land(P->ctx, w, P, certified, mismatch);
 }
 
 int ba_plan_result64_dev(lorb_ba_plan* P, double* d_out) {
@@ -1342,7 +1569,7 @@
   const int m = std::max(6 * C, std::min(3 * Pn, 256 * 1024));
   if (m > 0)
     hipLaunchKernelGGL(k_db_result, dim3(lorb::ceil_div(m, 256)), dim3(256), 0, plan->ctx->stream, plan->dev, C, Pn,
-                       plan->devb->perm, d_pose_out, d_point_out, (float*)nullptr, 1, 0);
+                       plan->devb->perm, d_pose_out, d_point_out, (float*)nullptr, 1, 0, (const int*)nullptr);
   LORB_CHECK_LAUNCH(plan->ctx);
   return LORB_OK;
 }
diff --git a/lorb_slam_amd/csrc/lorb_ba_dev.h b/lorb_slam_amd/csrc/lorb_ba_dev.h
--- a/lorb_slam_amd/csrc/lorb_ba_dev.h
+++ b/lorb_slam_amd/csrc/lorb_ba_dev.h
@@ -330,6 +330,13 @@
   return k;
 }
 
+__host__ __device__ inline int red_threads_rule(int W, int ctot, int n_pblk, int max_bw, int grid_bp) {
+  const double Wd = W > 1 ? W : 1, c = (double)ctot / Wd, cams = c > 1.0 ? c : 1.0;
+  const double cand = (double)n_pblk / Wd * ((max_bw + 1) / 6.0) / cams;
+  if (grid_bp <= 256 || cand >= 128.0) return 1024;
+  return grid_bp <= 1024 ? 512 : 256;
+}
+
 
 constexpr int kLdsBudget = 160 * 1024 - 2048;
 struct CholShape { int W, max_env, max_env_w, max_bw; };
diff --git a/lorb_slam_amd/csrc/lorb_ba_plan.h b/lorb_slam_amd/csrc/lorb_ba_plan.h
--- a/lorb_slam_amd/csrc/lorb_ba_plan.h
+++ b/lorb_slam_amd/csrc/lorb_ba_plan.h
@@ -101,6 +101,7 @@
   bool fold = false;
   int pt_launch = 0;
   int* live = nullptr;
+  int* gate = nullptr;
   lorb_comm* comm = nullptr;
   double *x2_send = nullptr, *x2_recv = nullptr;
   size_t fx_n = 0;
@@ -110,3 +111,7 @@
   lorb_ba_devbuild* devb = nullptr;
   ~lorb_ba_plan();
 };
+
+namespace lorb::ba {
+lorb_ba_plan::GraphKey plan_graph_key(const lorb_ba_plan* P);
+}
diff --git a/lorb_slam_amd/csrc/lorb_internal.h b/lorb_slam_amd/csrc/lorb_internal.h
--- a/lorb_slam_amd/csrc/lorb_internal.h
+++ b/lorb_slam_amd/csrc/lorb_internal.h
@@ -92,7 +92,9 @@
   } while (0)
 
 int ba_plan_result64_dev(lorb_ba_plan* P, double* d_out);
-int ba_plan_result_ring_dev(lorb_ba_plan* P, float* ring, int R, int t0, float* d_point_out);
+int ba_plan_result_ring_dev(lorb_ba_plan* P, float* ring, int R, int t0, float* d_point_out, int spec_points = -1);
+int ba_plan_spec_issue(lorb_ba_plan* P, const lorb_ba_window_dev* w, int obs_bound, bool* armed);
+int ba_plan_spec_land(lorb_ba_plan* P, const lorb_ba_window_dev* w, bool* certified, bool* mismatch);
 void ba_plan_sorted_hint(lorb_ba_plan* P, bool sorted);
 int ba_plan_update_dev_issue(lorb_ba_plan* P, const lorb_ba_window_dev* w);
 int ba_plan_update_dev_finish(lorb_ba_plan* P, const lorb_ba_window_dev* w);
diff --git a/lorb_slam_amd/csrc/lorb_map.hip b/lorb_slam_amd/csrc/lorb_map.hip
--- a/lorb_slam_amd/csrc/lorb_map.hip
+++ b/lorb_slam_amd/csrc/lorb_map.hip
@@ -277,6 +277,8 @@
   hipEvent_t ev_built = nullptr, ev_app = nullptr;
   bool built = false;
   int n_overlapped = 0;
+  bool spec_armed = false;
+  int n_certified = 0;
   std::vector<void*> allocs;
   ~lorb_map() {
     if (prof && prof_n)
@@ -479,9 +481,11 @@
 }
 
 int map_prepare(lorb_map* M, const lorb_frame_params* frame, const float pose[6], const float Tcw[16], int32_t n,
-                const uint8_t* d_desc, const float* d_x, const float* d_y, const float* d_depth, bool split = false) {
+                const uint8_t* d_desc, const float* d_x, const float* d_y, const float* d_depth, bool split = false,
+                bool spec = false) {
   if (!M || !frame || !pose || !Tcw || n < 0) return LORB_E_INVALID;
   lorb_ctx* ctx = M->ctx;
+  M->spec_armed = false;
   if (n > M->n_cap) return lorb::set_error(ctx, LORB_E_INVALID, "%d keypoints > the map's max_keypoints %d", n, M->n_cap);
   if (n > 0 && (!d_desc || !d_x || !d_y || !d_depth)) return LORB_E_INVALID;
   if (M->broken) return lorb::set_error(ctx, LORB_E_DEVICE, "the map is unusable after an earlier failed step");
@@ -549,8 +553,43 @@
     if (const int rc = lorb::ba_plan_update_dev_issue(M->plan, &w); rc != LORB_OK) return map_build_fail(M, rc);
     return LORB_OK;
   }
+  if (spec) {
+    if (const int rc = lorb::ba_plan_spec_issue(M->plan, &w, std::min(M->h_K + n, m.K_cap), &M->spec_armed); rc != LORB_OK)
+      return map_build_fail(M, rc);
+    if (M->spec_armed) return LORB_OK;
+  }
   if (const int rc = lorb_ba_plan_update_dev(M->plan, &w); rc != LORB_OK) return map_build_fail(M, rc);
   return map_build_done(M);
+}
+
+int map_finish(lorb_map* M);
+
+int map_spec_finish(lorb_map* M, const lorb_lm_options* opt, int p_bound) {
+  lorb_ctx* ctx = M->ctx;
+  M->spec_armed = false;
+  if (!M->ev_built) LORB_HIP(ctx, hipEventCreateWithFlags(&M->ev_built, hipEventDisableTiming));
+  int rc = hipEventRecord(M->ev_built, ctx->stream) == hipSuccess ? LORB_OK : LORB_E_DEVICE;
+  if (rc == LORB_OK) rc = lorb_ba_plan_solve(M->plan, opt);
+  if (rc == LORB_OK) rc = lorb::ba_plan_result_ring_dev(M->plan, M->m.ring, M->m.R, M->t0, M->m.pos, p_bound);
+  const lorb_ba_window_dev w = window_of(M);
+  bool certified = false, mismatch = false;
+  const int rl = lorb::ba_plan_spec_land(M->plan, &w, &certified, &mismatch);
+  if (mismatch || rc != LORB_OK) {
+    M->broken = true;
+    M->built = false;
+    return rc != LORB_OK ? rc : rl;
+  }
+  if (rl != LORB_OK) return map_build_fail(M, rl);
+  if (certified) {
+    M->plan_ok = true;
+    M->built = true;
+    M->n_certified++;
+    lorb::ba_plan_window_counts(M->plan, &M->h_P, &M->h_K);
+    return LORB_OK;
+  }
+  LORB_TRY(map_build_done(M));
+  LORB_TRY(lorb_ba_plan_solve(M->plan, opt));
+  return map_finish(M);
 }
 
 int map_build_finish(lorb_map* M) {
@@ -584,7 +623,11 @@
                       const uint8_t* d_desc, const float* d_x, const float* d_y, const float* d_depth,
                       const lorb_lm_options* opt) {
   if (!M || !opt) return LORB_E_INVALID;
-  LORB_TRY(map_prepare(M, frame, pose, Tcw, n, d_desc, d_x, d_y, d_depth));
+  const char* ns = getenv("LORB_NO_SPEC");
+  const bool spec = !(ns && ns[0] == '1') && !M->prof && !M->ctx->ktime;
+  const int p_bound = std::min(M->h_P + std::max(n, 0), M->m.P_cap);
+  LORB_TRY(map_prepare(M, frame, pose, Tcw, n, d_desc, d_x, d_y, d_depth, false, spec));
+  if (M->spec_armed) return map_spec_finish(M, opt, p_bound);
   LORB_TRY(lorb_ba_plan_solve(M->plan, opt));
   LORB_TRY(map_mark(M, 5));
   return map_finish(M);
@@ -604,9 +647,9 @@
   lorb_ctx* ctx = M->ctx;
   LORB_HIP(ctx, hipMemcpyAsync(M->pinned, M->m.cnt, sizeof(int) * 8, hipMemcpyDeviceToHost, ctx->stream));
   LORB_HIP(ctx, hipStreamSynchronize(ctx->stream));
-  const int32_t v[9] = {M->pinned[0], M->pinned[1], M->t0, M->last_n, M->pinned[3], M->pinned[4], M->pinned[5], M->m.W,
-                        M->n_overlapped};
-  for (int i = 0; i < n && i < 9; ++i) out[i] = v[i];
+  const int32_t v[10] = {M->pinned[0], M->pinned[1], M->t0, M->last_n, M->pinned[3], M->pinned[4], M->pinned[5], M->m.W,
+                         M->n_overlapped, M->n_certified};
+  for (int i = 0; i < n && i < 10; ++i) out[i] = v[i];
   return LORB_OK;
 }
 
diff --git a/lorb_slam_amd/runtime.py b/lorb_slam_amd/runtime.py
--- a/lorb_slam_amd/runtime.py
+++ b/lorb_slam_amd/runtime.py
@@ -440,7 +440,7 @@
 class LocalMap:
 
     COUNT_KEYS = ("points", "observations", "t0", "keypoints", "new_points", "new_observations", "matches", "window",
-                  "overlapped_steps")
+                  "overlapped_steps", "certified_steps")
 
     def __init__(self, ctx, init, max_points=None, max_obs=None, max_keypoints=4096):
         self.ctx, self._keep = ctx, A.KeepAlive()
@@ -486,8 +486,8 @@
                 a.free()
 
     def counts(self):
-        v = (C.c_int32 * 9)()
-        self.ctx.check(lib().lorb_map_counts(self._p, v, C.c_int32(9)), "lorb_map_counts")
+        v = (C.c_int32 * 10)()
+        self.ctx.check(lib().lorb_map_counts(self._p, v, C.c_int32(10)), "lorb_map_counts")
         return dict(zip(self.COUNT_KEYS, [int(x) for x in v]))
 
     def read(self):
```

Result: faster. 11720 BA iterations/s (median of 5 runs) (+1.6%).
